# flexcompute/tidy3d

Hardware: AMD Instinct MI355X
Metric: Mcells/s on 512^3 Yee grid (higher is better)
Workload: dtype f32; 1 GPU; v0: vacuum, PEC walls, curl stencil only; 512^3 Yee cells, Ez point dipole (GaussianPulse 200 THz), random +-1e-3 initial fields; parallelism=z-slab x1, bytes_per_cell_step=72

## Files before the change

include/fdtd_hip.h:

```cpp
#ifndef FDTD_HIP_H
#define FDTD_HIP_H

#include <stddef.h>
#include <stdint.h>

#ifdef __cplusplus
extern "C" {
#endif

typedef struct FdtdSolver FdtdSolver;

enum { FDTD_BC_PEC = 0, FDTD_BC_PMC = 1, FDTD_BC_PERIODIC = 2, FDTD_BC_NEIGHBOR = 3 };
enum { FDTD_MON_TIME = 0, FDTD_MON_DFT = 1 };
enum { FDTD_VARIANT_AUTO = 0, FDTD_VARIANT_SIMPLE = 1, FDTD_VARIANT_ZMARCH = 2, FDTD_VARIANT_FUSED = 3 };
enum { FDTD_FLAG_TIME_KERNELS = 1 };

typedef struct FdtdConfig {
  int32_t nx, ny, nz;
  int32_t bc[6];
  int32_t device;
  int32_t variant;
  int32_t flags;
  int32_t z_chunk;
  float   ch;
  int32_t reserved[6];
} FdtdConfig;

typedef struct FdtdStats {
  int64_t steps_done;
  int32_t diverged;
  int32_t stopped_early;
  double  field_decay;
  double  run_ms;
  double  h_kernel_ms;
  double  e_kernel_ms;
  int64_t h_kernel_launches;
  int64_t e_kernel_launches;
  int64_t device_bytes;
  double  fused_kernel_ms;
  int64_t fused_kernel_launches;
  int32_t tile_rows;
  int32_t tile_zchunk;
  int32_t tile_order;
  int32_t placement;
  float   placement_ms_first;
  float   placement_ms_kept;
  int32_t stream_overlap;
  int32_t stream_retries;
  int32_t comm_ranks;
  int32_t comm_rank;
  int64_t two_step_pairs;
  int32_t tblock_planes;
  int32_t reserved0;
  int64_t graph_pairs;
  int64_t fused2_pairs;
  int64_t fused2_shape;
  int64_t shell_pairs;
  double  shell_kernel_ms;
  int64_t shell_kernel_launches;
  int64_t shell2_pairs;
  int32_t fused2_off_reason;
  int32_t struct_bytes;
  int64_t disp_pairs;
  int32_t single_step_reason;
  int32_t src_paged_pairs;
  double  seam_kernel_ms;
  int64_t seam_kernel_launches;
} FdtdStats;

enum { FDTD_F2_OFF_NONE = 0,
       FDTD_F2_OFF_DISABLED = 1,
       FDTD_F2_OFF_TOO_SMALL = 2,
       FDTD_F2_OFF_COMM = 3,
       FDTD_F2_OFF_PML = 4,
       FDTD_F2_OFF_ADE = 5,
       FDTD_F2_OFF_TFSF = 6,
       FDTD_F2_OFF_BOUNDARY = 7,
       FDTD_F2_OFF_H_SOURCE_ABSORBER = 8,
       FDTD_F2_OFF_SEAM_SOURCE = 9,
       FDTD_F2_OFF_SOURCES = 10,
       FDTD_F2_OFF_VARIANT = 11,
       FDTD_F2_OFF_SHELL = 12,
       FDTD_F2_OFF_MEMORY = 13 };

typedef int (*FdtdProgressFn)(int64_t step, double time, double field_decay, void* user);

const char* fdtd_last_error(const FdtdSolver* h);
int  fdtd_device_count(void);

int  fdtd_far_field(int device, int n_u, int n_v, const double* u, const double* v, const double* wu, const double* wv,
                    const double* currents, double w0, double k_re, double k_im, int n_dir, const double* r_u,
                    const double* r_v, const double* r_w, double* out);

int  fdtd_create(const FdtdConfig* cfg, FdtdSolver** out);
void fdtd_destroy(FdtdSolver* h);

int fdtd_set_steps(FdtdSolver* h, int axis, const float* inv_primal, const float* inv_dual, int n);

int fdtd_set_media(FdtdSolver* h, const float* ca, const float* cb, int n_media);
int fdtd_set_material(FdtdSolver* h, const uint8_t* mat, size_t bytes);
int fdtd_set_material16(FdtdSolver* h, const uint16_t* mat, size_t count);

int fdtd_set_pml(FdtdSolver* h, int axis, int n_lo, int n_hi,
                 const float* kinv_e, const float* b_e, const float* c_e,
                 const float* kinv_h, const float* b_h, const float* c_h, int n);

int fdtd_set_mirror_plus(FdtdSolver* h, int axis, int wall);

int fdtd_set_absorber(FdtdSolver* h, int axis, int n_lo, int n_hi, const float* fb, const float* fc, int n);

int fdtd_add_ade(FdtdSolver* h, int comp, int64_t n_cells, const uint32_t* cell_index,
                 int n_poles, const float* kap, const float* bet, float cc);

int fdtd_add_aniso(FdtdSolver* h, int comp, int64_t n_nodes, const uint32_t* cell_index, const uint32_t* nbr_index,
                   const float* w_new, const float* w_old);
int fdtd_add_aniso_bloch(FdtdSolver* h, int comp, int64_t n_nodes, const uint32_t* cell_index, const uint32_t* nbr_index,
                         const float* w_new, const float* w_old, const uint8_t* wrap);

int fdtd_add_point_source(FdtdSolver* h, int64_t n_points, const int32_t* comp,
                          const uint32_t* cell_index, const float* w_re, const float* w_im,
                          int64_t n_steps, const float* wave_e, const float* wave_h);

int fdtd_add_tfsf(FdtdSolver* h, int n_aux, const float* ae, const float* be,
                  const float* ah, const float* bh, int src_cell,
                  int64_t n_steps, const float* wave,
                  int64_t n_e, const int32_t* e_comp, const uint32_t* e_index, const float* e_w,
                  const int32_t* e_aux,
                  int64_t n_h, const int32_t* h_comp, const uint32_t* h_index, const float* h_w,
                  const int32_t* h_aux);

int fdtd_add_monitor(FdtdSolver* h, int kind, int n_comps, const int32_t* comps,
                     const int32_t lo[3], const int32_t hi[3],
                     int64_t n_rec, const int64_t* steps,
                     int nf, const float* phase_e, const float* phase_h);
int fdtd_get_monitor(FdtdSolver* h, int monitor_id, void* host, size_t bytes);

int fdtd_set_field(FdtdSolver* h, int comp, const float* host, size_t bytes);
int fdtd_get_field(FdtdSolver* h, int comp, float* host, size_t bytes);

int fdtd_set_shutoff(FdtdSolver* h, int every, double shutoff, int64_t ref_step);

int fdtd_comm_unique_id(char id[128]);
int fdtd_comm_init(FdtdSolver* h, const char id[128], int rank, int n_ranks);

int fdtd_run(FdtdSolver* h, int64_t n_steps, FdtdProgressFn progress, void* user);
int fdtd_run_bloch(FdtdSolver* h_re, FdtdSolver* h_im, int64_t n_steps, const double phase[3], const int n_real[3],
                   FdtdProgressFn progress, void* user);
int fdtd_get_stats(FdtdSolver* h, FdtdStats* out);
enum { FDTD_OPT_FLAGS = 0, FDTD_OPT_VARIANT = 1, FDTD_OPT_ZCHUNK = 2, FDTD_OPT_ROWS = 3, FDTD_OPT_XCD_REMAP = 4 ,
       FDTD_OPT_FUSED_LB = 5,
       FDTD_OPT_PML_FUSED = 6 ,
       FDTD_OPT_BND_PLANES = 7 ,
       FDTD_OPT_AUTOTUNE = 8 ,
       FDTD_OPT_PML_SPLIT = 9 ,
       FDTD_OPT_PLACEMENT_TRIES = 12,
       FDTD_OPT_MEM_HINTS = 11,
       FDTD_OPT_TBLOCK = 13,
       FDTD_OPT_EDGE_ZCHUNK = 14,
       FDTD_OPT_GRAPH = 15,
       FDTD_OPT_TWOSTEP = 16,
       FDTD_OPT_SHELL_PAIRS = 17,
       FDTD_OPT_STRIP = 18,
       FDTD_OPT_SHELL2 = 19,
       FDTD_OPT_SHELL2_SHAPE = 20,
       FDTD_OPT_DEBUG_SYNC = 21,
       FDTD_OPT_TILE_SPLIT = 22,
       FDTD_OPT_DISP = 23,
       FDTD_OPT_SRC_PAGED = 25,
       FDTD_OPT_WHATIF = 24,
       FDTD_OPT_SLAB_BOXES_FIRST = 26,
       FDTD_OPT_LDS_PAD = 10  };
int fdtd_set_option(FdtdSolver* h, int key, int value);
int fdtd_reset(FdtdSolver* h);

#ifdef __cplusplus
}
#endif
#endif
```

tidy3d_amd/csrc/fdtd_capi.hip:

```cpp
#include <hip/hip_runtime.h>
#include <rccl/rccl.h>

#include <array>
#include <cmath>
#include <cstdarg>
#include <cstdio>
#include <cstdlib>
#include <cstring>
#include <deque>
#include <map>
#include <string>
#include <utility>
#include <algorithm>
#include <vector>

#include "../../include/fdtd_hip.h"
#include "fdtd_kernels.hpp"
#include "fdtd_fused2.hpp"
#include "fdtd_strip.hpp"
#include "fdtd_shell2_host.hpp"
#include "fdtd_aniso.hpp"

using namespace fdtd;

// ... 165 lines not shown
  SrcPaged spg;
  std::map<std::array<int, 6>, int> box_paged;
  int spg_on = -1;
  int whatif = 0;
  int disp_on = -1;
  std::vector<AnisoGroup> aniso;
  std::vector<PointSrc> psrc;
  std::vector<Tfsf> tfsf;
  std::vector<Monitor> mons;
  hipStream_t stream = nullptr, comm_stream = nullptr;
  hipEvent_t ev0 = nullptr, ev1 = nullptr;
  std::vector<hipEvent_t> kev;
  std::vector<int> kev_kind;
  double* energy_dev = nullptr;
  int decay_every = 0;
  double shutoff = 0.0;
  long long decay_ref = 0;
  double energy_max = 0.0;
  long long step = 0;
  FdtdStats stats{};
  int zchunk = 2;
  int zchunk_f = 16;
  int last_zc = 0;
  int rows_f = 3;
  int xcd_remap = -1;
  int fused_lb = 0;
  int pml_fused = -1;
  int placement_tries = 6;
  int slab_boxes_first = 3;
  hipStream_t box_stream = nullptr;
  bool box_stream_tried = false;
  int box_stream_attempts = 0;
  hipEvent_t ev_box = nullptr, ev_box_in = nullptr;
  bool placement_done = false;
  float placement_ms[9] = {};
  int placement_tried = 0, placement_kept = 0;
  int mem_hints = 1;
  int lds_pad = 0;
  int pml_split = -1;
  int autotune = 0;
  bool tuned = false, user_geometry = false;
  int bnd_planes = 0;
  int rows = 4;
  PmlP* pml_blk[8][2][2] = {};
  PmlP* pml_blk2[2][2] = {};
  PmlP* pml_blk_hole[2][2][2] = {};
  bool pml_blk_hole_ok = false;
  bool pml_blk_ok[8] = {};
  bool pml_blk2_ok = false;
  int pml_parity = 0;
  int pml_e_parity = 0;
  ncclComm_t comm = nullptr;
  int rank = 0, n_ranks = 1;
  hipEvent_t ev_h_int = nullptr, ev_h_bnd = nullptr, ev_e_int = nullptr, ev_e_bnd = nullptr;
  int stream_overlap = 0, stream_retries = 0;
  bool streams_shared = false;
  int tblock = -1;
  int edge_zchunk = -1;
  int use_graph = -1;
  long long* step_dev = nullptr;
  long long step_dev_value = -1;
  bool step_dev_mode = false;
  long long step_dev_off = 0;
  long long graph_pairs = 0;
  int mirror_wall[3] = {-1, -1, -1};
  int graph_status = 0;
  long long two_step_pairs = 0;
  int tblock_used = 0;
  int twostep_w = -1, twostep_zc = 0;
  int twostep_w_used = 0, twostep_zc_used = 0;
  long long fused2_pairs = 0;
  int shell_on = -1;
  int strip_zc = 4;
  int strip_occ = 3;
  long long shell_pairs = 0;
  int shell2_on = -1;
  int shell2_qw = 0, shell2_ww = 8, shell2_zcw = 0;
  int shell2_ws = 6, shell2_zcs = 0;
  long long shell2_pairs = 0;
  int f2_off_reason = 0;
  int debug_sync = 0;
  hipEvent_t ev_shell_a = nullptr, ev_shell_b = nullptr;
  hipEvent_t ev_rec = nullptr;
  float* seam_buf = nullptr;
  float* inj_val = nullptr;
  float* cap_val = nullptr;
  float* dump_buf = nullptr;
  long long dump_cap = 0;
  std::deque<F2Table> f2_tables;
  size_t inj_sources = 0;
  float* src_tab = nullptr;
  long long src_tab_steps = 0, src_tab_nodes = 0;
  bool src_on_seam = false;
  bool src_h_on_seam = false;
  long long src_nodes = 0;
  int f2_dyn_reason = 0;
  long long src_h_nodes = 0;
  bool src_e_in_damp = false;
};

namespace {

int fail(FdtdSolver* h, const char* fmt, ...) {
  char buf[1024];
  va_list ap;
  va_start(ap, fmt);
  vsnprintf(buf, sizeof(buf), fmt, ap);
  va_end(ap);
  if (h) h->err = buf; else g_create_error = buf;
  return -1;
}

#define HIPCHK(h, call)                                                                   \
  do {                                                                                    \
    hipError_t e_ = (call);                                                               \
    if (e_ != hipSuccess)                                                                 \
      return fail(h, "%s failed: %s (%s:%d)", #call, hipGetErrorString(e_), __FILE__, __LINE__); \
  } while (0)

#define NCCLCHK(h, call)                                                                  \
  do {                                                                                    \
    ncclResult_t r_ = (call);                                                             \
    if (r_ != ncclSuccess)                                                                \
      return fail(h, "%s failed: %s (%s:%d)", #call, ncclGetErrorString(r_), __FILE__, __LINE__); \
  } while (0)

template <typename T>
int dev_alloc(FdtdSolver* h, T** out, size_t count, bool zero_fill = true) {
  void* p = nullptr;
  size_t bytes = count * sizeof(T);
  if (bytes == 0) bytes = sizeof(T);
  HIPCHK(h, hipMalloc(&p, bytes));
  if (zero_fill) {
    HIPCHK(h, hipMemset(p, 0, bytes));
    HIPCHK(h, hipStreamSynchronize(nullptr));
  }
  h->bufs.push_back({p, bytes});
  h->stats.device_bytes += (int64_t)bytes;
  *out = reinterpret_cast<T*>(p);
  return 0;
}

template <typename T>
int dev_upload(FdtdSolver* h, T** out, const T* host, size_t count) {
  if (dev_alloc(h, out, count, false)) return -1;
  if (count) HIPCHK(h, hipMemcpy(*out, host, count * sizeof(T), hipMemcpyHostToDevice));
  return 0;
}

#ifdef FDTD_PLACEMENT_PROBE
inline long env_long(const char* name, long dflt) {
  const char* e = std::getenv(name);
  return e ? std::atol(e) : dflt;
}
int alloc_field_set(FdtdSolver* h, float** base, size_t fcount, int set) {
  const int mode = (int)env_long("FDTD_FIELD_LAYOUT", 0);
  if (mode == 3 || mode == 4) {
    if (set == 1) return 0;
    const size_t s0 = (size_t)env_long("FDTD_FIELD_S0", 0) / 16 * 4;
    const size_t s1 = (size_t)env_long("FDTD_FIELD_S1", 0) / 16 * 4, s2 = (size_t)env_long("FDTD_FIELD_S2", 0) / 16 * 4;
    const size_t stride = fcount + s1;
    float* blk = nullptr;
    if (mode == 4) {
      static float* pool = nullptr;
      const size_t pool_floats = (size_t)env_long("FDTD_FIELD_POOL", 16L << 30) / 4;
      if (!pool) HIPCHK(h, hipMalloc((void**)&pool, pool_floats * 4));
      if (s0 + 12 * stride + s2 > pool_floats) return fail(h, "field pool too small");
// ... 556 lines not shown
  }
  std::stable_sort(ent.begin(), ent.end(), [](const std::array<int, 5>& x, const std::array<int, 5>& y) {
    return x[0] != y[0] ? x[0] < y[0] : (x[3] >= 8) < (y[3] >= 8);
  });
  std::vector<int> start((size_t)g.nz + 2, 0);
  std::vector<int4> e4(std::max<size_t>(1, ent.size()));
  for (size_t q = 0; q < ent.size(); ++q) {
    start[(size_t)ent[q][0] + 1]++;
    e4[q].x = ent[q][1]; e4[q].y = ent[q][2]; e4[q].z = ent[q][3]; e4[q].w = ent[q][4];
  }
  for (int k = 0; k <= g.nz; ++k) start[(size_t)k + 1] += start[(size_t)k];
  if (dev_upload(h, &tb.start, (const int*)start.data(), start.size()) ||
      dev_upload(h, &tb.ent, (const int4*)e4.data(), e4.size())) return nullptr;
  tb.dfts = plan.dfts; tb.dft_when = plan.dft_when;
  if (!plan.dfts.empty()) {
    std::vector<DumpBox> boxes;
    std::vector<std::vector<int>> per_plane((size_t)g.nz + 1);
    long long off = 0;
    for (size_t q = 0; q < plan.dfts.size(); ++q) {
      const Monitor& m = h->mons[(size_t)plan.dfts[q]];
      DumpBox bx{m.box.lo0, m.box.lo1, m.box.lo2, m.box.nx, m.box.ny, m.box.nz, {-1, -1, -1, -1, -1, -1}};
      const int when = plan.dft_when[q];
      for (int c : m.comps) if ((c >= 3 && (when & 1)) || (c < 3 && (when & 2))) { bx.off[c] = (int)off; off += m.cells; }
      tb.dft_off.push_back({bx.off[0], bx.off[1], bx.off[2], bx.off[3], bx.off[4], bx.off[5]});
      bool any = false;
      for (int c = 0; c < 6; ++c) any = any || bx.off[c] >= 0;
      if (!any) continue;
      for (int k = m.box.lo2; k < m.box.lo2 + m.box.nz; ++k) per_plane[(size_t)k].push_back((int)boxes.size());
      boxes.push_back(bx);
    }
    tb.dump_floats = off;
    if (!boxes.empty()) {
      std::vector<int> ds((size_t)g.nz + 2, 0), dl;
      for (int k = 0; k <= g.nz; ++k) { ds[(size_t)k] = (int)dl.size(); if (k < g.nz) for (int b : per_plane[(size_t)k]) dl.push_back(b); }
      ds[(size_t)g.nz + 1] = (int)dl.size();
      if (dl.empty()) dl.push_back(0);
      if (dev_upload(h, &tb.dstart, (const int*)ds.data(), ds.size()) || dev_upload(h, &tb.dlist, (const int*)dl.data(), dl.size()) ||
          dev_upload(h, &tb.dboxes, (const DumpBox*)boxes.data(), boxes.size())) return nullptr;
    }
  }
  h->f2_tables.push_back(tb);
  return &h->f2_tables.back();
}

const FdtdSolver::TileClasses* tile_classes(FdtdSolver* h, int W, int zc, const ClipP& box, int nbx, int nby, int nbz, bool disp = false, bool src = false) {
  const bool mats = h->mat4 && !h->roww_host.empty();
  if ((!mats && !src) || h->tile_split == 0) return nullptr;
  for (const auto& t : h->tile_cls)
    if (t.W == W && t.zc == zc && t.nbx == nbx && t.nby == nby && t.nbz == nbz && t.box.j0 == box.j0 && t.box.j1 == box.j1 &&
        t.box.k0 == box.k0 && t.box.k1 == box.k1 && t.disp == disp && t.src == src) return &t;
  const GridP& g = h->g;
  const int R = W - 3, nbx_all = (g.nx + 255) / 256;
  std::vector<unsigned char> cls((size_t)nbx * nby * nbz, 0);
  long long n_bg = 0;
  for (int tz = 0; tz < nbz; ++tz)
    for (int tx = 0; tx < nbx; ++tx)
      for (int ty = 0; ty < nby; ++ty) {
        const int k0 = box.k0 + tz * zc, k1 = std::min(k0 + zc, box.k1);
        const int j0 = box.j0 + ty * R;
        unsigned char c = 0;
        for (int k = std::max(k0 - 1, 0); mats && k <= std::min(k1, g.nz - 1) && !c; ++k)
          for (int j = std::max(j0 - 2, 0); j <= std::min(j0 + R, g.ny - 1); ++j)
            if (h->roww_host[((size_t)k * g.ny + j) * nbx_all + tx] != kBgWord) { c = 1; break; }
        if (disp && c)
          for (int k = std::max(k0 - 1, 0); k <= std::min(k1, g.nz - 1) && c < 2; ++k)
            for (int j = std::max(j0 - 2, 0); j <= std::min(j0 + R, g.ny - 1); ++j)
              if (h->disp.dseg_host[((size_t)k * g.ny + j) * nbx_all + tx] >= 0) { c = 2; break; }
        n_bg += !c;
        if (src) {
          bool found = false;
          for (int k = std::max(k0 - 1, 0); k <= std::min(k1, g.nz - 1) && !found; ++k)
            for (int j = std::max(j0 - 2, 0); j <= std::min(j0 + R, g.ny - 1); ++j)
              if (h->spg.sseg_host[((size_t)k * g.ny + j) * nbx_all + tx] >= 0) { found = true; break; }
          if (found) c |= 4;
        }
        cls[((size_t)tz * nbx + tx) * nby + ty] = c;
      }
  FdtdSolver::TileClasses e{W, zc, box, nbx, nby, nbz, nullptr, n_bg, (long long)cls.size(), disp, src};
  if (dev_upload(h, &e.dev, (const unsigned char*)cls.data(), cls.size())) return nullptr;
  h->tile_cls.push_back(e);
  return &h->tile_cls.back();
}

int launch_fused2(FdtdSolver* h, long long n, hipStream_t st, const F2Table* tb, bool* sources2_done, bool* damp2_done = nullptr,
                  const ClipP* clip = nullptr, bool use_disp = false, bool e2_clip = false, const SrcP& sr = SrcP{}) {
  const bool inject = tb->with_sources;
  const GridP& g = h->g;
  if (ensure_second_set(h)) return -1;
  int W = 16, zc = 32;
  const ClipP box = clip ? *clip : ClipP{0, g.nx, 0, g.ny, 0, g.nz};
  fused2_shape(h, &W, &zc, (clip && h->comm) ? clip : nullptr);
  if (clip && !h->comm && h->twostep_zc <= 0 && (long long)g.nx * g.ny * g.nz < (1LL << 28)) zc = std::min(zc, 16);
  zc = std::max(2, std::min(zc, box.k1 - box.k0));
  h->twostep_w_used = W; h->twostep_zc_used = zc;
  const int R = W - 3;
  const int nbx = (g.nx + 255) / 256, nby = (box.j1 - box.j0 + R - 1) / R;
  const int nbz = (box.k1 - box.k0 + zc - 1) / zc;
  const int n_seams = nbx - 1 + ((clip && h->cfg.bc[0] == FDTD_BC_PERIODIC) ? 1 : 0);
  if (!h->seam_buf && (nbx > 1 || h->cfg.bc[0] == FDTD_BC_PERIODIC) &&
      dev_alloc(h, &h->seam_buf, (size_t)nbx * kSeamArrays * (size_t)(g.nz + 2) * (size_t)g.ny)) return -1;
  if (!h->inj_val && dev_alloc(h, &h->inj_val, (size_t)kMaxInj)) return -1;
  if (!h->cap_val && dev_alloc(h, &h->cap_val, (size_t)kMaxCap)) return -1;
  InjP inj{};
  *sources2_done = false;
  {
    bool alive = false, alive2 = true;
    for (const PointSrc& s : h->psrc)
      if (inject && (s.n_e || s.n_h)) { alive = alive || n < s.n_steps; alive2 = alive2 && n + 1 < s.n_steps; }
    if (alive && h->src_tab && n + 1 < h->src_tab_steps) {
      inj.val = h->src_tab + n * h->src_tab_nodes;
      if (alive2) {
        inj.val2 = h->src_tab + (n + 1) * h->src_tab_nodes;
        if (!clip || e2_clip) { inj.e2_in_sweep = 1; *sources2_done = true; }
      }
    } else if (alive) {
      int off = 0;
      for (const PointSrc& s : h->psrc) {
        if (s.n_e) launch_inject_values(st, h->inj_val + off, s.wre_e, s.wim_e, s.wave_e, n, (int)s.n_e);
        off += (int)(s.n_e + s.n_h);
      }
      inj.val = h->inj_val;
    }
    inj.n = (alive || !tb->mons.empty()) ? 1 : 0;
    inj.start = tb->start; inj.ent = tb->ent; inj.cap = h->cap_val;
    if (tb->dstart) {
      if (tb->dump_floats > h->dump_cap) {
        if (dev_alloc(h, &h->dump_buf, (size_t)tb->dump_floats, false)) return -1;
        h->dump_cap = tb->dump_floats;
      }
      inj.dstart = tb->dstart; inj.dlist = tb->dlist; inj.dboxes = tb->dboxes; inj.dump = h->dump_buf;
      inj.n = 1;
    }
  }
  DampT dmp{};
  if (h->has_damp) {
    for (int a = 0; a < 3; ++a) { dmp.fb[a] = h->damp_fb[a]; dmp.fc[a] = h->damp_fc[a]; }
    bool post_sources = false;
    for (const PointSrc& s : h->psrc) post_sources = post_sources || (s.n_e && n + 1 < s.n_steps);
    dmp.e2 = (!post_sources || inj.e2_in_sweep || sr.sseg || !h->src_e_in_damp) ? 1 : 0;
    if (damp2_done) *damp2_done = dmp.e2 != 0;
  }
  const int total = nbx * nby * nbz;
  const int remap = h->xcd_remap < 0 ? 32 : h->xcd_remap;
  StepP sp = step_params(h);
  time_begin(h, 2, st);
  const MatP mp = mat_params(h);
  DispP dp{nullptr, nullptr, nullptr};
  if (use_disp) dp = DispP{h->disp.dseg, h->disp.cs, h->disp.e1};
  int opt = (h->mem_hints ? 1 : 0) | (h->mat4 ? 2 : 0) | ((tb->mons.empty() && (!tb->with_sources || h->src_h_nodes == 0) && !tb->dstart) ? 0 : 4) |
            (clip ? 16 : (h->has_damp ? 8 : 0)) | (use_disp ? 32 | 1 : 0);
  if (h->whatif > 0 && h->whatif <= 15 && h->whatif != 9 && opt == 1 && (W == 16 || h->whatif == 13 || h->whatif == 14)) opt |= h->whatif << 8;
  SrcP sr_used = sr;
  if (h->whatif == 9 && !sr.sseg && !(opt & 8) && (!(opt & 32) || (opt & 16))) {
    SrcPaged& S = h->spg;
    const size_t nseg = (size_t)g.nz * g.ny * ((g.nx + 255) / 256);
    if (!S.sseg && S.state != 1) {
      S.sseg_host.assign(nseg, -1);
      SrcT tab{};
      if (dev_upload(h, &S.sseg, (const int*)S.sseg_host.data(), nseg) || dev_upload(h, &S.tab, &tab, 1)) return -1;
    }
    if (S.sseg && S.state != 1) { sr_used.sseg = S.sseg; sr_used.t = S.tab; opt |= 64 | 4 | 1; }
  }
  if (sr.sseg) { opt |= 64 | 4 | 1; *sources2_done = true; h->spg.pairs++; }
  const int blocks = remap ? ((total + 7) / 8) * 8 : total;
  const FdtdSolver::TileClasses* tc = tile_classes(h, W, zc, box, nbx, nby, nbz, use_disp, sr_used.sseg != nullptr);
  const bool split = tc && (use_disp || sr_used.sseg || (tc->n_bg > 0 && (h->tile_split == 1 || 8 * tc->n_bg >= tc->n_all)));
  launch_fused2_step(st, W, opt, blocks, g, h->f, h->f2, sp, mp, zc, nbx, nby, nbz, remap, inj, h->seam_buf, dmp, box,
                     TileClassP{split ? tc->dev : nullptr}, dp, sr_used);
  time_end(h, st);
  if (n_seams > 0) {
    time_begin(h, 4, st);
    launch_seams(st, g, h->f2, sp, mp, h->seam_buf, n_seams, dmp, box, inj, sr);
    time_end(h, st);
  }
  if (use_disp) h->disp.pairs++;
  if (!clip) swap_sets(h);
  return 0;
}

struct ShellGeom { int o0[3], o1[3]; };
bool shell_geometry(const FdtdSolver* h, ShellGeom* G) {
  const int N[3] = {h->g.nx, h->g.ny, h->g.nz};
  for (int a = 0; a < 3; ++a) {
    const PmlAxisDev& P = h->pml[a];
    const int lo = P.ns > 0 ? P.lo : 0, hi0 = P.ns > 0 ? P.hi0 : N[a];
    int o0 = lo > 0 ? lo + 2 : 0, o1 = hi0 < N[a] ? hi0 - 1 : N[a];
    if (a > 0 && h->cfg.bc[2 * a] == FDTD_BC_PERIODIC) { o0 = 2; o1 = N[a] - 2; }
    if (a == 0) { o0 = (o0 + 3) / 4 * 4; o1 = o1 / 4 * 4; }
    if (o1 - o0 < (a == 0 ? 16 : 8)) return false;
    G->o0[a] = o0; G->o1[a] = o1;
  }
  return true;
}

void release_buf(FdtdSolver* h, void* p);
int ensure_third_set(FdtdSolver* h) {
  const GridP& g = h->g;
  if (h->f3.ex) return 0;
  const size_t fcount = (size_t)g.sxy * (g.nz + 2);
  if (!h->fbase3[0] && alloc_field_set(h, h->fbase3, fcount, 2)) {
    for (int c = 0; c < 6; ++c) { if (h->fbase3[c]) release_buf(h, h->fbase3[c]); h->fbase3[c] = nullptr; }
    return -1;
  }
  h->f3.ex = h->fbase3[0] + g.sxy; h->f3.ey = h->fbase3[1] + g.sxy; h->f3.ez = h->fbase3[2] + g.sxy;
  h->f3.hx = h->fbase3[3] + g.sxy; h->f3.hy = h->fbase3[4] + g.sxy; h->f3.hz = h->fbase3[5] + g.sxy;
  return 0;
}

void launch_strip(FdtdSolver* h, const FieldP& src, const FieldP& dst, const PmlP* pm, int ci0, int ci1, int j0, int j1,
                  int k0, int k1, hipStream_t st) {
  if (ci1 <= ci0 || j1 <= j0 || k1 <= k0) return;
  StripP sp;
  sp.q = std::min(kStripMaxQ, (ci1 - ci0) / 4);
  sp.xorg = ci0; sp.ci0 = ci0; sp.ci1 = ci1; sp.j0 = j0; sp.j1 = j1; sp.kbeg = k0; sp.kend = k1;
  sp.zchunk = h->strip_zc;
  const int slots = (64 / sp.q) * kStripWaves;
  sp.nbx = (ci1 - ci0 + 4 * sp.q - 1) / (4 * sp.q);
  sp.nby = (j1 - j0 + slots - 2) / (slots - 1);
  sp.nbz = (k1 - k0 + sp.zchunk - 1) / sp.zchunk;
  const int pmc = h->cfg.bc[4] == FDTD_BC_PMC;
  const dim3 grid((unsigned)(sp.nbx * sp.nby * sp.nbz)), block(64, kStripWaves);
  time_begin(h, 3, st);
  if (h->mat4 && h->strip_occ == 4) hipLaunchKernelGGL((strip_step_kernel<true, 4>), grid, block, 0, st, h->g, src, dst, step_params(h), mat_params(h), pm, sp, pmc);
  else if (h->mat4) hipLaunchKernelGGL((strip_step_kernel<true, 3>), grid, block, 0, st, h->g, src, dst, step_params(h), mat_params(h), pm, sp, pmc);
  else if (h->strip_occ == 4) hipLaunchKernelGGL((strip_step_kernel<false, 4>), grid, block, 0, st, h->g, src, dst, step_params(h), mat_params(h), pm, sp, pmc);
  else hipLaunchKernelGGL((strip_step_kernel<false, 3>), grid, block, 0, st, h->g, src, dst, step_params(h), mat_params(h), pm, sp, pmc);
  time_end(h, st);
}

struct ZPlan {
  int n = 0;
  int a[4] = {}, b[4] = {};
  bool ok = false;
};
bool zplan_build(const FdtdSolver* h, const ShellGeom& G, bool source_holes, ZPlan* P) {
  std::vector<std::pair<int, int>> holes;
  for (const AdeGroup& a : h->ade) if (a.n > 0) holes.push_back({a.k0 - 2, a.k1 + 2});
  if (source_holes) {
    for (const PointSrc& s : h->psrc) {
      if (s.n_e) holes.push_back({s.ke0 - 2, s.ke1 + 2});
      if (s.n_h) holes.push_back({s.kh0 - 2, s.kh1 + 2});
    }
    for (const Tfsf& t : h->tfsf) {
      if (t.e.n_targets) holes.push_back({t.e.k0 - 2, t.e.k1 + 2});
      if (t.h.n_targets) holes.push_back({t.h.k0 - 2, t.h.k1 + 2});
    }
  }
  std::sort(holes.begin(), holes.end());
  P->n = 0;
  int lo = G.o0[2];
  auto close = [&](int hi) {
    if (hi - lo >= 8) {
      if (P->n == 4) return false;
      P->a[P->n] = lo; P->b[P->n] = hi; P->n++;
    }
    return true;
  };
  for (const auto& hz : holes) {
    if (hz.second <= lo) continue;
    if (hz.first >= G.o1[2]) break;
// ... 1622 lines not shown
  return 0;
}
}

int fdtd_add_tfsf(FdtdSolver* h, int n_aux, const float* ae, const float* be, const float* ah, const float* bh,
                  int src_cell, int64_t n_steps, const float* wave, int64_t n_e, const int32_t* e_comp,
                  const uint32_t* e_index, const float* e_w, const int32_t* e_aux, int64_t n_h,
                  const int32_t* h_comp, const uint32_t* h_index, const float* h_w, const int32_t* h_aux) {
  if (!h) return -1;
  if (n_aux < 4 || src_cell < 1 || src_cell >= n_aux) return fail(h, "fdtd_add_tfsf: bad auxiliary grid");
  HIPCHK(h, hipSetDevice(h->cfg.device));
  Tfsf t{};
  t.n_aux = n_aux; t.src_cell = src_cell;
  t.n_steps = n_steps;
  if (dev_upload(h, &t.ae, ae, (size_t)n_aux + 1) || dev_upload(h, &t.be, be, (size_t)n_aux + 1) ||
      dev_upload(h, &t.ah, ah, (size_t)n_aux) || dev_upload(h, &t.bh, bh, (size_t)n_aux) ||
      dev_alloc(h, &t.e1, (size_t)n_aux + 1) || dev_alloc(h, &t.h1, (size_t)n_aux) ||
      dev_alloc(h, &t.e1c, (size_t)n_aux + 1) || dev_alloc(h, &t.h1c, (size_t)n_aux) ||
      dev_upload(h, &t.wave, wave, (size_t)n_steps))
    return -1;
  if (build_tfsf_list(h, t.e, n_e, e_comp, e_index, e_w, e_aux, n_aux - 1) ||
      build_tfsf_list(h, t.h, n_h, h_comp, h_index, h_w, h_aux, n_aux))
    return -1;
  h->tfsf.push_back(t);
  return 0;
}

int fdtd_add_monitor(FdtdSolver* h, int kind, int n_comps, const int32_t* comps, const int32_t lo[3],
                     const int32_t hi[3], int64_t n_rec, const int64_t* steps, int nf, const float* phase_e,
                     const float* phase_h) {
  if (!h) return -1;
  if (kind != FDTD_MON_TIME && kind != FDTD_MON_DFT) return fail(h, "fdtd_add_monitor: bad kind %d", kind);
  const int N[3] = {h->g.nx, h->g.ny, h->g.nz};
  for (int a = 0; a < 3; ++a)
    if (lo[a] < 0 || hi[a] > N[a] || hi[a] <= lo[a]) return fail(h, "fdtd_add_monitor: box [%d,%d) outside axis %d of %d cells", lo[a], hi[a], a, N[a]);
  if (n_comps < 1 || n_comps > 6) return fail(h, "fdtd_add_monitor: n_comps must be 1..6");
  if (kind == FDTD_MON_DFT && nf < 1) return fail(h, "fdtd_add_monitor: a DFT monitor needs frequencies");
  HIPCHK(h, hipSetDevice(h->cfg.device));
  Monitor m;
  m.kind = kind;
  m.comps.assign(comps, comps + n_comps);
  for (int c : m.comps) if (c < 0 || c > 5) return fail(h, "fdtd_add_monitor: bad component %d", c);
  m.box.lo0 = lo[0]; m.box.lo1 = lo[1]; m.box.lo2 = lo[2];
  m.box.nx = hi[0] - lo[0]; m.box.ny = hi[1] - lo[1]; m.box.nz = hi[2] - lo[2];
  m.cells = (long long)m.box.nx * m.box.ny * m.box.nz;
  m.steps.assign(steps, steps + n_rec);
  for (size_t i = 1; i < m.steps.size(); ++i)
    if (m.steps[i] <= m.steps[i - 1]) return fail(h, "fdtd_add_monitor: steps must be strictly increasing");
  m.nf = nf;
  if (kind == FDTD_MON_TIME) {
    m.data_bytes = (size_t)n_rec * n_comps * m.cells * sizeof(float);
    float* d = nullptr;
    if (dev_alloc(h, &d, (size_t)n_rec * n_comps * m.cells)) return -1;
    m.data = d;
  } else {
    m.data_bytes = (size_t)nf * n_comps * m.cells * sizeof(float2);
    float2* d = nullptr;
    if (dev_alloc(h, &d, (size_t)nf * n_comps * m.cells)) return -1;
    m.data = d;
    if (dev_upload(h, &m.phase_e, reinterpret_cast<const float2*>(phase_e), (size_t)n_rec * nf) ||
        dev_upload(h, &m.phase_h, reinterpret_cast<const float2*>(phase_h), (size_t)n_rec * nf))
      return -1;
  }
  h->mons.push_back(m);
  return (int)h->mons.size() - 1;
}

int fdtd_get_monitor(FdtdSolver* h, int id, void* host, size_t bytes) {
  if (!h) return -1;
  if (id < 0 || id >= (int)h->mons.size()) return fail(h, "fdtd_get_monitor: bad id %d", id);
  Monitor& m = h->mons[id];
  if (bytes != m.data_bytes) return fail(h, "fdtd_get_monitor: expected %zu bytes, got %zu", m.data_bytes, bytes);
  HIPCHK(h, hipSetDevice(h->cfg.device));
  HIPCHK(h, hipStreamSynchronize(h->stream));
  HIPCHK(h, hipMemcpy(host, m.data, bytes, hipMemcpyDeviceToHost));
  return 0;
}

int fdtd_set_field(FdtdSolver* h, int comp, const float* host, size_t bytes) {
  if (!h) return -1;
  if (comp < 0 || comp > 5) return fail(h, "fdtd_set_field: bad component");
  if (bytes != (size_t)n_cells(h) * 4) return fail(h, "fdtd_set_field: expected %zu bytes", (size_t)n_cells(h) * 4);
  HIPCHK(h, hipSetDevice(h->cfg.device));
  HIPCHK(h, hipMemcpy(field_ptr(h, comp), host, bytes, hipMemcpyHostToDevice));
  for (AdeGroup& a : h->ade)
    if (a.comp == comp) {
      hipLaunchKernelGGL(ade_gather_kernel, dim3(nblk(a.n)), dim3(256), 0, h->stream, (const float*)field_ptr(h, comp),
                         (const uint32_t*)a.cell, a.e_old, a.n);
      HIPCHK(h, hipStreamSynchronize(h->stream));
    }
  if (h->comm == nullptr) { fill_ghost_h(h, h->stream); fill_ghost_e(h, h->stream); fill_ghost_fused(h, h->stream); HIPCHK(h, hipStreamSynchronize(h->stream)); }
  else if (comp == 0 || comp == 1 || comp == 3 || comp == 4) {
    HIPCHK(h, hipStreamSynchronize(h->stream));
    if (exchange(h, comp < 3, h->comm_stream)) return -1;
    HIPCHK(h, hipStreamSynchronize(h->comm_stream));
  }
  return 0;
}

int fdtd_get_field(FdtdSolver* h, int comp, float* host, size_t bytes) {
  if (!h) return -1;
  if (comp < 0 || comp > 5) return fail(h, "fdtd_get_field: bad component");
  if (bytes != (size_t)n_cells(h) * 4) return fail(h, "fdtd_get_field: expected %zu bytes", (size_t)n_cells(h) * 4);
  HIPCHK(h, hipSetDevice(h->cfg.device));
  HIPCHK(h, hipStreamSynchronize(h->stream));
  HIPCHK(h, hipMemcpy(host, field_ptr(h, comp), bytes, hipMemcpyDeviceToHost));
  return 0;
}

int fdtd_set_shutoff(FdtdSolver* h, int every, double shutoff, int64_t ref_step) {
  if (!h) return -1;
  h->decay_every = every; h->shutoff = shutoff; h->decay_ref = ref_step;
  return 0;
}

int fdtd_comm_unique_id(char id[128]) {
  ncclUniqueId u;
  if (ncclGetUniqueId(&u) != ncclSuccess) return fail(nullptr, "ncclGetUniqueId failed");
  std::memcpy(id, &u, 128);
  return 0;
}

int fdtd_comm_init(FdtdSolver* h, const char id[128], int rank, int n_ranks) {
  if (!h) return -1;
  if (rank < 0 || rank >= n_ranks) return fail(h, "fdtd_comm_init: bad rank %d of %d", rank, n_ranks);
  HIPCHK(h, hipSetDevice(h->cfg.device));
  ncclUniqueId u;
  std::memcpy(&u, id, 128);
  NCCLCHK(h, ncclCommInitRank(&h->comm, n_ranks, u, rank));
  h->rank = rank; h->n_ranks = n_ranks;
  int cnt = 0, ur = -1;
  NCCLCHK(h, ncclCommCount(h->comm, &cnt));
  NCCLCHK(h, ncclCommUserRank(h->comm, &ur));
  h->stats.comm_ranks = cnt; h->stats.comm_rank = ur;
  return 0;
}

int fdtd_reset(FdtdSolver* h) {
  if (!h) return -1;
  HIPCHK(h, hipSetDevice(h->cfg.device));
  HIPCHK(h, hipStreamSynchronize(h->stream));
  for (int c = 0; c < 6; ++c) HIPCHK(h, hipMemset(h->fbase[c], 0, h->field_bytes));
  for (int c = 0; c < 6; ++c) if (h->fbase2[c]) HIPCHK(h, hipMemset(h->fbase2[c], 0, h->field_bytes));
  for (int c = 0; c < 6; ++c) if (h->fbase3[c]) HIPCHK(h, hipMemset(h->fbase3[c], 0, h->field_bytes));
  for (int a = 0; a < 3; ++a) {
    PmlAxisDev& P = h->pml[a];
    if (P.n == 0) continue;
    for (int s = 0; s < 2; ++s) {
      if (P.psi_e[s]) HIPCHK(h, hipMemset(P.psi_e[s], 0, P.psi_count * 4));
      if (P.psi_h[s]) HIPCHK(h, hipMemset(P.psi_h[s], 0, (P.psi_count + P.psi_plane) * 4));
      if (P.psi_h2[s]) HIPCHK(h, hipMemset(P.psi_h2[s], 0, (P.psi_count + P.psi_plane) * 4));
      if (P.psi_e2[s]) HIPCHK(h, hipMemset(P.psi_e2[s], 0, P.psi_count * 4));
      if (P.psi_et[s]) HIPCHK(h, hipMemset(P.psi_et[s], 0, P.psi_count * 4));
      if (P.psi_ht[s]) HIPCHK(h, hipMemset(P.psi_ht[s], 0, (P.psi_count + P.psi_plane) * 4));
    }
  }
  for (AdeGroup& a : h->ade) {
    HIPCHK(h, hipMemset(a.e_old, 0, (size_t)a.n * 4));
    HIPCHK(h, hipMemset(a.q, 0, (size_t)a.n * a.p.n_poles * 8));
  }
  if (h->disp.state == 1) HIPCHK(h, hipMemset(h->disp.cs, 0, (size_t)h->disp.n_blocks * 3 * 256 * sizeof(float)));
  for (Tfsf& t : h->tfsf) {
    HIPCHK(h, hipMemset(t.e1, 0, ((size_t)t.n_aux + 1) * 4));
    HIPCHK(h, hipMemset(t.h1, 0, (size_t)t.n_aux * 4));
  }
  for (Monitor& m : h->mons) { HIPCHK(h, hipMemset(m.data, 0, m.data_bytes)); m.next = 0; }
  h->step = 0; h->energy_max = 0.0;
  h->stats.steps_done = 0; h->stats.diverged = 0; h->stats.stopped_early = 0; h->stats.field_decay = 1.0;
  return 0;
}

}
namespace {
struct GraphRec { const float* set; int parity; hipGraphExec_t exec; };
struct Run {
  FdtdSolver* h;
  int64_t n_steps;
  FdtdProgressFn progress;
  void* user;
  bool multi = false, nb_lo = false, nb_hi = false;
  int nz = 0;
  hipStream_t st = nullptr, cs = nullptr;
  bool fused_ok = false, fused = false, fused_multi = false;
  int b_lo = 0, b_hi = 0;
  bool primed = false;
  int pml_in_m = 0;
  bool psi_ghosts = false;
  int tb_req = 0;
  bool tb_two_streams = false, tb_ok = false;
  std::vector<hipEvent_t> tb_ev;
  bool split_now = false, graph_ok = false;
  std::vector<GraphRec> graphs;
  bool f2_ok = false, f2s_ok = false, s2_ok = false, s2_deep = false, f2m_ok = false;
  bool s2_disp = false;
  bool pair_disp = false;
  bool spg_ok = false;
  bool pair_spg = false;
  bool f2mc_ok = false, f2mc_deep = false;
  ShellGeom sg{}, sgm{};
  ZPlan zp_base, zp_src;
  ZPlan zp_s2, zp_s2h;
  F2Plan f2_plan;
  int64_t done = 0;
  long long n = 0;
  bool rec = false, src_alive = false, pair = false, use_s2 = false;
  int src_why = 0;
  const ZPlan* zp = nullptr;

  void sync_point() { if (h->debug_sync) (void)hipDeviceSynchronize(); }
  int setup() {
    multi = h->comm != nullptr;
    nb_lo = h->cfg.bc[4] == FDTD_BC_NEIGHBOR, nb_hi = h->cfg.bc[5] == FDTD_BC_NEIGHBOR;
    if ((nb_lo || nb_hi) && !multi) return fail(h, "fdtd_run: neighbour faces need fdtd_comm_init");
    if (multi && !h->aniso.empty()) return fail(h, "fdtd_run: fully anisotropic media are not available on z-slabs");
    if (multi && h->mirror_wall[2] >= 0 && (nb_hi || h->mirror_wall[2] != h->g.nz - 2 || h->g.nz < 6))
      return fail(h, "fdtd_run: a PMC plus face along z needs the last z-slab to hold the wall and at least 6 planes");
    nz = h->g.nz;
    if ((multi || any_pml(h) || h->tblock > 4096) && probe_stream_overlap(h)) return -1;
    st = h->stream, cs = h->comm_stream;
    for (hipEvent_t e : h->kev) hipEventDestroy(e);
    h->kev.clear(); h->kev_kind.clear();
    h->stats.stopped_early = 0;
    HIPCHK(h, hipEventRecord(h->ev0, st));
    if (multi && (nb_lo || nb_hi) && nz < 2) return fail(h, "fdtd_run: a z-slab needs at least 2 planes");
// ... 240 lines not shown
  int setup_pairs() {
    if (fused && !tb_ok && !h->ade.empty() && disp_setup(h)) return -1;
    h->disp.pairs = 0;
    s2_disp = false;
    spg_ok = false;
    h->spg.pairs = 0;
    if (fused && !tb_ok && !multi && (!h->tfsf.empty() || !h->psrc.empty())) {
      if (fused2_sources(h)) return -1;
      bool needs = !h->tfsf.empty() || h->src_nodes > kMaxInj || h->src_h_on_seam || (h->src_h_nodes > 0 && !h->src_tab);
      if (!needs) {
        long long len = -1;
        for (const PointSrc& s : h->psrc) if (s.n_e || s.n_h) { if (len >= 0 && s.n_steps != len) needs = true; len = s.n_steps; }
      }
      if (needs && spg_setup(h)) return -1;
      spg_ok = needs && h->spg.state == 1 && !(h->has_damp && h->spg.any_h);
    }
    f2_ok = fused && !tb_ok && fused2_eligible(h);
    sg = ShellGeom{};
    f2s_ok = false;
    h->f2_off_reason = !fused ? FDTD_F2_OFF_VARIANT : (tb_ok ? FDTD_F2_OFF_DISABLED : 0);
    if (fused && !tb_ok && !f2_ok) {
      const bool shell = any_pml(h) || any_periodic(h) || !h->ade.empty();
      h->f2_off_reason = shell ? shell_why_not(h, &sg, &zp_base, &zp_src) : fused2_why_not(h);
      f2s_ok = shell && h->f2_off_reason == 0;
    }
    s2_ok = false, s2_deep = false;
    if (fused && !tb_ok && !f2_ok && any_pml(h)) {
      ShellGeom g2{};
      const int why2 = shell2_why_not(h, &g2);
      if (why2 == 0) {
        const int why_r4 = h->f2_off_reason;
        s2_ok = true; sg = g2;
        s2_deep = shell2_sources_deep(h, sg);
        h->f2_off_reason = 0;
        zp_s2 = ZPlan{};
        s2_disp = !h->ade.empty() && h->disp.state == 1 && h->cfg.bc[2] != FDTD_BC_PERIODIC && h->shell2_on != 2 && h->shell2_on != 3;
        if (h->ade.empty() || s2_disp) { zp_s2.n = 1; zp_s2.a[0] = sg.o0[2]; zp_s2.b[0] = sg.o1[2]; zp_s2.ok = true; }
        else if (zplan_build(h, sg, false, &zp_s2) && zp_s2.a[0] == sg.o0[2] && zp_s2.b[zp_s2.n - 1] == sg.o1[2]) zp_s2.ok = true;
        if (!zp_s2.ok) { s2_ok = false; s2_disp = false; h->f2_off_reason = why_r4; }
        zp_s2h = ZPlan{};
        if (h->shell2_on != 2 && h->shell2_on != 3 && zplan_build(h, sg, true, &zp_s2h) && zp_s2h.n > 1 && zp_s2h.a[0] == sg.o0[2] &&
            zp_s2h.b[zp_s2h.n - 1] == sg.o1[2]) zp_s2h.ok = true;
      }
    }
    h->f2_dyn_reason = 0;
    if (f2_ok || f2s_ok || s2_ok) {
      if (fused2_sources(h)) return -1;
    }
    if (f2s_ok && ensure_third_set(h)) {
      (void)hipGetLastError();
      h->err.clear();
      f2s_ok = false;
      h->f2_off_reason = FDTD_F2_OFF_MEMORY;
    }
    if ((f2s_ok || s2_ok) && probe_stream_overlap(h)) return -1;
    f2m_ok = fused_multi && !any_pml(h) && !h->has_damp && h->shell_on != 0 && nz >= 8 && fused2_why_not(h, true) == 0;
    if (fused_multi) h->f2_off_reason = f2m_ok ? 0 : (any_pml(h) || h->has_damp ? FDTD_F2_OFF_COMM : (fused2_why_not(h, true) ? fused2_why_not(h, true) : FDTD_F2_OFF_COMM));
    if (f2m_ok) {
      if (fused2_sources(h)) return -1;
      if (ensure_third_set(h)) { (void)hipGetLastError(); h->err.clear(); f2m_ok = false; h->f2_off_reason = FDTD_F2_OFF_MEMORY; }
    }
    f2mc_ok = false;
    if (fused_multi && any_pml(h) && pml_in_m != 0 && pml_in_m == pml_in_sweep_mask(h) && !h->has_damp && h->shell_on != 0 &&
        h->shell2_on != 0 && h->shell2_on != 2 && h->shell2_on != 3 &&
        h->ade.empty() && !any_periodic(h) && (long long)h->g.sxy * 4 < (1LL << 32)) {
      int why = fused2_why_not(h, true, true);
      if (!why && !shell_geometry(h, &sgm)) why = FDTD_F2_OFF_PML;
      if (!why) {
        const PmlAxisDev& pz = h->pml[2];
        if (nb_lo) sgm.o0[2] = std::max(sgm.o0[2], 2);
        if (nb_hi) sgm.o1[2] = std::min(sgm.o1[2], nz - 2);
        if (sgm.o1[2] - sgm.o0[2] < 8 || (pz.ns > 0 && ((nb_lo && pz.lo > 0) || (nb_hi && pz.hi0 < nz)))) why = FDTD_F2_OFF_TOO_SMALL;
      }
      if (!why && (fused2_sources(h) || ensure_third_set(h) || ensure_pml_blocks2(h) || ensure_pml_blocks_hole(h))) {
        (void)hipGetLastError();
        h->err.clear();
        why = FDTD_F2_OFF_MEMORY;
      }
      f2mc_ok = why == 0;
      f2mc_deep = f2mc_ok && shell2_sources_deep(h, sgm);
      h->f2_off_reason = why;
    }
    h->fused2_pairs = 0;
    h->shell_pairs = 0;
    h->shell2_pairs = 0;
    done = 0;
    return 0;
  }
  int shell_pair(long long n, const F2Table* tb, const ZPlan& zp) {
    hipStream_t cs = (h->shell_on == 2) ? st : h->comm_stream;
    const int pml_in = 7 & pml_in_sweep_mask(h);
    if (ensure_second_set(h) || ensure_third_set(h) || ensure_pml_blocks(h, pml_in)) return -1;
    if (!h->ev_shell_a) {
      HIPCHK(h, hipEventCreateWithFlags(&h->ev_shell_a, hipEventDisableTiming));
      HIPCHK(h, hipEventCreateWithFlags(&h->ev_shell_b, hipEventDisableTiming));
    }
    const int N[3] = {h->g.nx, h->g.ny, nz};
    int in0[3], in1[3];
    for (int a = 0; a < 3; ++a) {
      in0[a] = sg.o0[a] > 0 ? sg.o0[a] + (a == 0 ? 4 : 1) : 0;
      in1[a] = sg.o1[a] < N[a] ? sg.o1[a] - (a == 0 ? 4 : 1) : N[a];
    }
    launch_sources(h, false, n, 0, nz, st);
    advance_tfsf_aux(h, false, n, st);
    if (h->cfg.bc[4] == FDTD_BC_PERIODIC) fill_ghost_h(h, st);
    HIPCHK(h, hipEventRecord(h->ev_shell_a, st));
    HIPCHK(h, hipStreamWaitEvent(cs, h->ev_shell_a, 0));
    const FieldP A = h->f, B = h->f2, T = h->f3;
    const int par = h->pml_parity;
    bool s2 = false;
    for (int i = 0; i < zp.n; ++i) {
      const ClipP clip{sg.o0[0], sg.o1[0], sg.o0[1], sg.o1[1], zp.a[i], zp.b[i]};
      if (launch_fused2(h, n, st, tb, &s2, nullptr, &clip)) return -1;
    }
    if (launch_shell_step(h, A, T, par, in0, in1, pml_in, cs, zp, 1)) return -1;
    launch_sources(h, true, n, 0, nz, cs, false, &T);
    launch_ade(h, 0, nz, cs, &T);
    advance_tfsf_aux(h, true, n, cs);
    launch_sources(h, false, n + 1, 0, nz, cs, false, &T);
    advance_tfsf_aux(h, false, n + 1, cs);
    fill_ghost_fused(h, cs, &T);
    if (launch_shell_step(h, T, B, par ^ 1, sg.o0, sg.o1, pml_in, cs, zp, 0)) return -1;
    HIPCHK(h, hipEventRecord(h->ev_shell_b, cs));
    HIPCHK(h, hipStreamWaitEvent(st, h->ev_shell_b, 0));
    swap_sets(h);
    pair_record(h, tb, n, st);
    if (rec_at(n + 1)) record_monitors(h, n + 1, true, st);
    launch_sources(h, true, n + 1, 0, nz, st);
    launch_ade(h, 0, nz, st);
    advance_tfsf_aux(h, true, n + 1, st);
    fill_ghost_fused(h, st);
    return 0;
  }
  int shell2_pair(long long n, const F2Table* tb, const ZPlan& zp) {
    hipStream_t cs = (h->shell_on == 2) ? st : h->comm_stream;
    const bool holes = zp.n > 1;
    const bool per_y = h->cfg.bc[2] == FDTD_BC_PERIODIC;
    if (ensure_second_set(h) || ensure_pml_blocks2(h)) return -1;
    if ((holes || per_y) && (ensure_third_set(h) || ensure_pml_blocks_hole(h))) return -1;
    if (!h->ev_shell_a) {
      HIPCHK(h, hipEventCreateWithFlags(&h->ev_shell_a, hipEventDisableTiming));
      HIPCHK(h, hipEventCreateWithFlags(&h->ev_shell_b, hipEventDisableTiming));
    }
    launch_sources(h, false, n, 0, nz, st);
    if (pair_spg) spg_fill(h, n, st);
    else advance_tfsf_aux(h, false, n, st);
    const SrcP sr = pair_spg ? spg_params(h) : SrcP{};
    HIPCHK(h, hipEventRecord(h->ev_shell_a, st));
    HIPCHK(h, hipStreamWaitEvent(cs, h->ev_shell_a, 0));
    const FieldP A = h->f, B = h->f2, T = h->f3;
    const int hp = h->pml_parity, ep = h->pml_e_parity;
    bool s2 = false;
    Shell2Box boxes[kShell2MaxBoxes];
    int nb = 0;
    for (int i = 0; i < zp.n; ++i) {
      const ClipP clip{sg.o0[0], sg.o1[0], sg.o0[1], sg.o1[1], zp.a[i], zp.b[i]};
      if (launch_fused2(h, n, st, tb, &s2, nullptr, &clip, pair_disp, zp.n == 1 && s2_deep, sr)) return -1;
      ShellGeom gi = sg;
      gi.o0[2] = zp.a[i]; gi.o1[2] = zp.b[i];
      Shell2Box bi[kShell2MaxBoxes];
      const int ni = shell2_boxes(h, gi, bi, i == 0 ? 0 : zp.a[i], i == zp.n - 1 ? nz : zp.b[i]);
      for (int q = 0; q < ni && nb < kShell2MaxBoxes; ++q) boxes[nb++] = bi[q];
    }
    bool src_due = false;
    for (const PointSrc& sr : h->psrc) src_due = src_due || (sr.n_e && n + 1 < sr.n_steps);
    const bool ade2_early = pair_disp && (s2 || !src_due) && disp_inside(h, sg.o0, sg.o1, 2);
    if (ade2_early) launch_ade2(h, st, &B);
    launch_shell2_boxes(h, boxes, nb, h->pml_blk2[hp][ep], cs, tb, pair_disp, sr);
    if (holes || per_y) {
      const int pml_in = 7 & pml_in_sweep_mask(h);
      ShellSets s1{A, T, hp, 0, 0, h->pml_blk_hole[0][hp][ep]}, s2h{T, B, hp, 0, 0, h->pml_blk_hole[1][hp][ep]};
      auto wrap_rows = [&](const ShellSets& base, int grow) {
        const int R = h->rows_f, ny = h->g.ny, nby_all = (ny + R - 1) / R;
        const int in0 = 2 + grow, in1 = ny - 2 - grow;
        const int ty_a = std::min(nby_all, (in0 + R - 1) / R), ty_c = std::max(ty_a, in1 / R);
        ShellSets sh = base;
        sh.ex_j0 = in0; sh.ex_j1 = in1;
        for (int i = 0; i < zp.n; ++i) {
          const int lo = i == 0 ? 0 : zp.a[i], hi = i == zp.n - 1 ? nz : zp.b[i];
          if (launch_fused_range(h, lo, hi, cs, pml_in, 0, 0, ty_a + (nby_all - ty_c), ty_a, ty_c - ty_a, true, &sh)) return -1;
        }
        return 0;
      };
      for (int i = 0; i + 1 < zp.n; ++i)
        if (launch_fused_range(h, zp.b[i] - 1, zp.a[i + 1] + 1, cs, pml_in, 0, 0, -1, 0, 0, true, &s1)) return -1;
      if (per_y && wrap_rows(s1, 1)) return -1;
      if (holes) {
        launch_sources(h, true, n, 0, nz, cs, false, &T);
        launch_ade(h, 0, nz, cs, &T);
        advance_tfsf_aux(h, true, n, cs);
        launch_sources(h, false, n + 1, 0, nz, cs, false, &T);
        advance_tfsf_aux(h, false, n + 1, cs);
      }
      for (int i = 0; i + 1 < zp.n; ++i)
        if (launch_fused_range(h, zp.b[i], zp.a[i + 1], cs, pml_in, 0, 0, -1, 0, 0, true, &s2h)) return -1;
      if (per_y && wrap_rows(s2h, 0)) return -1;
    }
    HIPCHK(h, hipEventRecord(h->ev_shell_b, cs));
    HIPCHK(h, hipStreamWaitEvent(st, h->ev_shell_b, 0));
    swap_sets(h);
    swap_psi_h(h, 7);
    swap_psi_e(h);
    pair_record(h, tb, n, st);
    if (rec_at(n + 1)) record_monitors(h, n + 1, true, st);
    if (!holes && !pair_spg) {
      advance_tfsf_aux(h, true, n, st);
      advance_tfsf_aux(h, false, n + 1, st);
    }
    if (!s2) launch_sources(h, true, n + 1, 0, nz, st);
    if (!pair_disp) launch_ade(h, 0, nz, st);
    else if (!ade2_early) launch_ade2(h, st);
    if (!pair_spg) advance_tfsf_aux(h, true, n + 1, st);
    fill_ghost_fused(h, st);
    return 0;
  }
  bool plan_clear_of_holes(const F2Plan& pl, const ZPlan& zp) {
    auto inside = [&](const Monitor& m, bool segment) {
      for (int i = 0; i < zp.n; ++i) {
        const int lo = (segment && i == 0) ? 0 : zp.a[i], hi = (segment && i == zp.n - 1) ? nz : zp.b[i];
        if (m.box.lo2 >= lo && m.box.lo2 + m.box.nz <= hi) return true;
      }
      return false;
    };
    for (int q : pl.mons) if (!inside(h->mons[(size_t)q], false)) return false;
    for (int q : pl.dfts) if (!inside(h->mons[(size_t)q], true)) return false;
    if (h->cfg.bc[2] == FDTD_BC_PERIODIC)
      for (int q : pl.dfts) {
        const Monitor& m = h->mons[(size_t)q];
        if (m.box.lo1 < 2 || m.box.lo1 + m.box.ny > h->g.ny - 2) return false;
      }
    return true;
  }
  bool plan_in_bulk(const F2Plan& pl, const ZPlan& zp) {
    auto inside = [&](const Monitor& m) {
      for (int i = 0; i < zp.n; ++i) if (m.box.lo2 >= zp.a[i] && m.box.lo2 + m.box.nz <= zp.b[i]) return true;
      return false;
    };
    for (int q : pl.mons) if (!inside(h->mons[(size_t)q])) return false;
    for (int q : pl.dfts) if (!inside(h->mons[(size_t)q])) return false;
    return true;
  }
  int begin_step() {
    n = h->step;
    rec = !fused_multi && rec_at(n);
    if (rec && multi) {
      HIPCHK(h, hipStreamWaitEvent(st, h->ev_e_bnd, 0));
      HIPCHK(h, hipStreamWaitEvent(st, h->ev_h_bnd, 0));
    }
    src_alive = false;
    src_why = 0;
    zp = &zp_base;
    pair = fused && (f2_ok || f2s_ok || s2_ok) && done + 2 <= n_steps && !(h->decay_every > 0 && ((n + 1) % h->decay_every) == 0);
    use_s2 = false;
    if (pair) {
      src_why = fused2_sources_why_not(h, n, &src_alive);
      pair_spg = false;
      if (src_why != 0 && spg_ok && (src_why == FDTD_F2_OFF_TFSF || src_why == FDTD_F2_OFF_SOURCES || src_why == FDTD_F2_OFF_SEAM_SOURCE)) {
        const bool s2_form = s2_ok && zp_s2.ok && zp_s2.n == 1 && h->cfg.bc[2] != FDTD_BC_PERIODIC;
        if (s2_form || f2_ok) { pair_spg = true; src_why = 0; src_alive = false; }
      }
      use_s2 = s2_ok && src_why == 0 && (!src_alive || s2_deep || pair_spg);
      if (use_s2) zp = &zp_s2;
      else if (s2_ok && zp_s2h.ok && (src_why != 0 || src_alive)) {
        use_s2 = true; src_why = 0; src_alive = false; zp = &zp_s2h;
      }
      if (!use_s2 && !f2_ok && !f2s_ok) { if (src_why) h->f2_dyn_reason = src_why; pair = false; }
    }
    if (pair && use_s2) {
      pair = fused2_plan(h, n, &f2_plan, sg.o0, sg.o1, true) && plan_clear_of_holes(f2_plan, *zp);
      if (!pair && f2s_ok) { pair = true; use_s2 = false; zp = &zp_base; src_why = fused2_sources_why_not(h, n, &src_alive); }
    }
    if (pair && !use_s2) {
      if (src_why && f2s_ok && zp_src.ok) { src_why = 0; src_alive = false; zp = &zp_src; }
      if (src_why) h->f2_dyn_reason = src_why;
      pair = src_why == 0 && fused2_plan(h, n, &f2_plan, f2s_ok ? sg.o0 : nullptr, f2s_ok ? sg.o1 : nullptr) &&
             (!f2s_ok || plan_in_bulk(f2_plan, *zp));
    }
    pair_disp = pair && !h->ade.empty() && h->disp.state == 1 && (use_s2 ? (s2_disp && zp == &zp_s2) : !f2s_ok);
    pair_spg = pair_spg && pair && (use_s2 ? zp == &zp_s2 : (f2_ok && !f2s_ok));
    if (rec) record_monitors(h, n, false, st, (pair && !h_terms_in_front(h)) ? &f2_plan : nullptr);
    if (rec && multi) {
      if (!h->ev_rec) HIPCHK(h, hipEventCreateWithFlags(&h->ev_rec, hipEventDisableTiming));
      HIPCHK(h, hipEventRecord(h->ev_rec, st));
      HIPCHK(h, hipStreamWaitEvent(cs, h->ev_rec, 0));
    }
    return 0;
  }
  int slab_shell2_pair(const F2Table* tb) {
    const int bl = nb_lo ? 2 : 0, bh = nb_hi ? 2 : 0;
    const FieldP A = h->f, B = h->f2, T = h->f3;
    const int hp = h->pml_parity, ep = h->pml_e_parity;
    ShellSets s1{A, T, hp, 0, 0, h->pml_blk_hole[0][hp][ep]}, s2h{T, B, hp, 0, 0, h->pml_blk_hole[1][hp][ep]};
    HIPCHK(h, hipStreamWaitEvent(cs, h->ev_e_int, 0));
    HIPCHK(h, hipStreamWaitEvent(st, h->ev_e_bnd, 0));
    const ClipP clip{sgm.o0[0], sgm.o1[0], sgm.o0[1], sgm.o1[1], sgm.o0[2], sgm.o1[2]};
    bool s2done = false;
    Shell2Box boxes[kShell2MaxBoxes];
    const int nb = shell2_boxes(h, sgm, boxes, bl, nz - bh);
    bool third = (h->slab_boxes_first == 2 || (h->slab_boxes_first == 3 && nz >= 96)) && nb > 0 && !h->streams_shared && !h->debug_sync;
    if (third && !h->box_stream_tried && make_box_stream(h)) return -1;
    third = third && h->box_stream != nullptr;
    if (third) {
      HIPCHK(h, hipEventRecord(h->ev_box_in, st));
      HIPCHK(h, hipStreamWaitEvent(h->box_stream, h->ev_box_in, 0));
      HIPCHK(h, hipStreamWaitEvent(h->box_stream, h->ev_e_bnd, 0));
      launch_shell2_boxes(h, boxes, nb, h->pml_blk2[hp][ep], h->box_stream, tb);
      HIPCHK(h, hipEventRecord(h->ev_box, h->box_stream));
    } else if (h->slab_boxes_first) launch_shell2_boxes(h, boxes, nb, h->pml_blk2[hp][ep], st, tb);
    if (launch_fused2(h, n, st, tb, &s2done, nullptr, &clip)) return -1;
    if (launch_fused_range(h, 0, bl ? bl + 1 : 0, cs, pml_in_m, bh ? nz - bh - 1 : nz, nz, -1, 0, 0, true, &s1)) return -1;
    HIPCHK(h, hipEventRecord(h->ev_h_bnd, cs));
    if (bl) { launch_sources(h, true, n, 0, bl + 1, cs, false, &T); launch_sources(h, false, n + 1, 0, bl + 1, cs, false, &T); }
    if (bh) { launch_sources(h, true, n, nz - bh - 1, nz, cs, false, &T); launch_sources(h, false, n + 1, nz - bh - 1, nz, cs, false, &T); }
    if (exchange_fused_all(h, cs, psi_ghosts, &T, 1)) return -1;
    if (launch_fused_range(h, 0, bl, cs, pml_in_m, nz - bh, nz, -1, 0, 0, true, &s2h)) return -1;
    if (bl) { launch_sources(h, true, n + 1, 0, bl, cs, false, &B); launch_sources(h, false, n + 2, 0, bl, cs, false, &B); }
    if (bh) { launch_sources(h, true, n + 1, nz - bh, nz, cs, false, &B); launch_sources(h, false, n + 2, nz - bh, nz, cs, false, &B); }
    HIPCHK(h, hipEventRecord(h->ev_e_bnd, cs));
    if (exchange_fused_all(h, cs, psi_ghosts, &B, 2)) return -1;
    if (!h->slab_boxes_first) launch_shell2_boxes(h, boxes, nb, h->pml_blk2[hp][ep], st, tb);
    if (third) HIPCHK(h, hipStreamWaitEvent(st, h->ev_box, 0));
    swap_sets(h);
    swap_psi_h(h, 7);
    swap_psi_e(h);
    launch_sources(h, true, n + 1, bl, nz - bh, st);
    launch_sources(h, false, n + 2, bl, nz - bh, st);
    HIPCHK(h, hipEventRecord(h->ev_e_int, st));
// ... 27 lines not shown
      bool s2done = false;
      if (launch_fused2(h, n, st, tb, &s2done, nullptr, &clip)) return -1;
      if (launch_fused_range(h, 0, bl ? bl + 1 : 0, cs, 0, bh ? nz - bh - 1 : nz, nz, -1, 0, 0, false, &s1)) return -1;
      HIPCHK(h, hipEventRecord(h->ev_h_bnd, cs));
      if (bl) { launch_sources(h, true, n, 0, bl + 1, cs, false, &T); launch_sources(h, false, n + 1, 0, bl + 1, cs, false, &T); }
      if (bh) { launch_sources(h, true, n, nz - bh - 1, nz, cs, false, &T); launch_sources(h, false, n + 1, nz - bh - 1, nz, cs, false, &T); }
      if (exchange_fused_all(h, cs, false, &T)) return -1;
      if (launch_fused_range(h, 0, bl, cs, 0, nz - bh, nz, -1, 0, 0, false, &s2)) return -1;
      if (bl) { launch_sources(h, true, n + 1, 0, bl, cs, false, &B); launch_sources(h, false, n + 2, 0, bl, cs, false, &B); }
      if (bh) { launch_sources(h, true, n + 1, nz - bh, nz, cs, false, &B); launch_sources(h, false, n + 2, nz - bh, nz, cs, false, &B); }
      HIPCHK(h, hipEventRecord(h->ev_e_bnd, cs));
      if (exchange_fused_all(h, cs, false, &B)) return -1;
      swap_sets(h);
      launch_sources(h, true, n + 1, bl, nz - bh, st);
      launch_sources(h, false, n + 2, bl, nz - bh, st);
      HIPCHK(h, hipEventRecord(h->ev_e_int, st));
      h->fused2_pairs++;
      h->step = n + 2;
      return 1;
    }
    const bool decay_step = h->decay_every > 0 && ((n + 1) % h->decay_every) == 0;
    const bool last = (done + 1 == n_steps) || decay_step;
    HIPCHK(h, hipStreamWaitEvent(cs, h->ev_e_int, 0));
    const int pml_b = pml_in_m & 3;
    if (b_lo > 0 && b_hi > 0) { if (launch_fused_range(h, 0, b_lo, cs, pml_b, nz - b_hi, nz)) return -1; }
    else if (b_lo > 0) { if (launch_fused_range(h, 0, b_lo, cs, pml_b)) return -1; }
    else if (b_hi > 0) { if (launch_fused_range(h, nz - b_hi, nz, cs, pml_b)) return -1; }
    HIPCHK(h, hipEventRecord(h->ev_h_bnd, cs));
    HIPCHK(h, hipStreamWaitEvent(st, h->ev_e_bnd, 0));
    if ((pml_in_m & 6) == 0) {
      if (launch_fused_range(h, b_lo, nz - b_hi, st, pml_in_m)) return -1;
    } else {
      const int R = h->rows_f, nby_all = (h->g.ny + R - 1) / R, ki = b_lo, ke = nz - b_hi;
      const PmlAxisDev &py = h->pml[1], &pz = h->pml[2];
      const bool in_y = (pml_in_m & 2) && py.ns > 0, in_z = (pml_in_m & 4) && pz.ns > 0;
      const int za = std::min(ke, std::max(ki, (in_z && pz.lo > 0) ? std::min(nz, pz.lo + 1) : 0));
      const int zc = std::max(za, std::min(ke, (in_z && pz.hi0 < nz) ? pz.hi0 : nz));
      const int ty_a = (in_y && py.lo > 0) ? std::min(nby_all, py.lo / R + 1) : 0;
      const int ty_c = (in_y && py.hi0 < h->g.ny) ? std::max(ty_a, py.hi0 / R) : nby_all;
      if ((za > ki || zc < ke) && launch_fused_range(h, ki, za, st, pml_in_m, zc, ke, -1, 0, 0, true)) return -1;
      if (launch_fused_range(h, za, zc, st, pml_in_m & 3, 0, 0, ty_a + (nby_all - ty_c), ty_a, ty_c - ty_a, true)) return -1;
      if (launch_fused_range(h, za, zc, st, pml_in_m & 1, 0, 0, ty_c - ty_a, 0, ty_a)) return -1;
    }
    swap_sets(h);
    swap_psi_h(h, pml_in_m);
    const bool rec_post = rec_at(n);
    if (rec_post || last || rec_at(n + 1)) {
      HIPCHK(h, hipStreamWaitEvent(st, h->ev_h_bnd, 0));
      if (rec_post) record_monitors(h, n, true, st);
      e_post(n, 0, nz, st, false);
      advance_tfsf_aux(h, true, n, st, false);
      advance_tfsf_aux(h, true, n, st, true);
      primed = false;
      if (!last && prime(n + 1)) return -1;
      if (last) {
        HIPCHK(h, hipEventRecord(h->ev_e_int, st));
        HIPCHK(h, hipStreamWaitEvent(cs, h->ev_e_int, 0));
        HIPCHK(h, hipEventRecord(h->ev_e_bnd, cs));
      }
    } else {
      e_post(n, 0, b_lo, cs, true);
      e_post(n, nz - b_hi, nz, cs, true);
      advance_tfsf_aux(h, true, n, cs, true);
      h_pre(n + 1, 0, b_lo, cs, true);
      h_pre(n + 1, nz - b_hi, nz, cs, true);
      advance_tfsf_aux(h, false, n + 1, cs, true);
      HIPCHK(h, hipEventRecord(h->ev_e_bnd, cs));
      if (exchange_fused_all(h, cs, psi_ghosts)) return -1;
      e_post(n, b_lo, nz - b_hi, st, false);
      advance_tfsf_aux(h, true, n, st, false);
      h_pre(n + 1, b_lo, nz - b_hi, st, false);
      advance_tfsf_aux(h, false, n + 1, st, false);
      HIPCHK(h, hipEventRecord(h->ev_e_int, st));
    }
    h->step = n + 1;
    return 0;
  }
  int plain_pair() {
    const F2Table* tb = fused2_table(h, f2_plan, src_alive);
    if (!tb) return -1;
    bool sources2_done = false, damp2_done = true;
    launch_sources(h, false, n, 0, nz, st);
    if (pair_spg) spg_fill(h, n, st);
    if (launch_fused2(h, n, st, tb, &sources2_done, &damp2_done, nullptr, pair_disp, false, pair_spg ? spg_params(h) : SrcP{})) return -1;
    pair_record(h, tb, n, st);
    if (rec_at(n + 1)) record_monitors(h, n + 1, true, st);
    if (!sources2_done) launch_sources(h, true, n + 1, 0, nz, st);
    if (h->has_damp && !damp2_done) launch_damp(h, true, 0, nz, st);
    if (pair_disp) launch_ade2(h, st);
    fill_ghost_fused(h, st);
    return 0;
  }
  int two_pass_step() {
    const int h_top = (multi && nb_hi) ? nz - 1 : nz;
    const bool mirrors = h->mirror_wall[0] >= 0 || h->mirror_wall[1] >= 0 || h->mirror_wall[2] >= 0;
    if (multi && mirrors) {
      HIPCHK(h, hipStreamWaitEvent(st, h->ev_e_bnd, 0));
      fill_mirror(h, st, 0, nz);
      if (!h->ev_rec) HIPCHK(h, hipEventCreateWithFlags(&h->ev_rec, hipEventDisableTiming));
      HIPCHK(h, hipEventRecord(h->ev_rec, st));
      HIPCHK(h, hipStreamWaitEvent(cs, h->ev_rec, 0));
    }
    if (multi && nb_hi) {
      HIPCHK(h, hipStreamWaitEvent(cs, h->ev_e_int, 0));
      launch_damp(h, false, h_top, nz, cs);
      launch_sources(h, false, n, h_top, nz, cs);
      launch_pml(h, false, h_top, nz, cs);
      launch_h_main(h, h_top, nz, cs);
      HIPCHK(h, hipEventRecord(h->ev_h_bnd, cs));
    }
    if (multi) HIPCHK(h, hipStreamWaitEvent(st, h->ev_e_bnd, 0));
    if (!multi) fill_mirror(h, st, 0, nz);
    launch_damp(h, false, 0, h_top, st);
    launch_sources(h, false, n, 0, h_top, st);
    launch_pml(h, false, 0, h_top, st);
    launch_h_main(h, 0, h_top, st);
    advance_tfsf_aux(h, false, n, st);
    if (multi) {
      HIPCHK(h, hipEventRecord(h->ev_h_int, st));
      if (!nb_hi) HIPCHK(h, hipStreamWaitEvent(cs, h->ev_h_int, 0));
      HIPCHK(h, hipStreamWaitEvent(cs, h->ev_e_int, 0));
      if (exchange(h, false, cs)) return -1;
    }
    if (!multi || !nb_lo) fill_ghost_h(h, st);
    if (rec) {
      if (multi) HIPCHK(h, hipStreamWaitEvent(st, h->ev_h_bnd, 0));
      record_monitors(h, n, true, st);
    }
    const int e_bot = (multi && nb_lo) ? 1 : 0;
    if (multi && nb_lo) {
      HIPCHK(h, hipStreamWaitEvent(cs, h->ev_h_int, 0));
      launch_e_main(h, 0, e_bot, cs);
      launch_pml(h, true, 0, e_bot, cs);
      launch_sources(h, true, n, 0, e_bot, cs);
      launch_damp(h, true, 0, e_bot, cs);
      launch_ade(h, 0, e_bot, cs);
      HIPCHK(h, hipEventRecord(h->ev_e_bnd, cs));
    }
    if (multi && nb_hi) HIPCHK(h, hipStreamWaitEvent(st, h->ev_h_bnd, 0));
    aniso_save(h, st);
    launch_e_main(h, e_bot, nz, st);
    launch_pml(h, true, e_bot, nz, st);
    launch_sources(h, true, n, e_bot, nz, st);
    aniso_apply(h, st);
    launch_damp(h, true, e_bot, nz, st);
    launch_ade(h, e_bot, nz, st);
    advance_tfsf_aux(h, true, n, st);
    if (multi) {
      HIPCHK(h, hipEventRecord(h->ev_e_int, st));
      if (!nb_lo) HIPCHK(h, hipStreamWaitEvent(cs, h->ev_e_int, 0));
      HIPCHK(h, hipStreamWaitEvent(cs, h->ev_h_int, 0));
      if (exchange(h, true, cs)) return -1;
    }
    if (!multi || !nb_hi) fill_ghost_e(h, st);
    h->step = n + 1;
    return 0;
  }
  int decay_check() {
  if (h->decay_every > 0 && (h->step % h->decay_every) == 0) {
    if (multi) HIPCHK(h, hipStreamWaitEvent(st, h->ev_e_bnd, 0));
    double en = 0.0;
    if (eval_energy(h, st, &en)) return -1;
    if (multi) {
      double* tmp = h->energy_dev;
      HIPCHK(h, hipMemcpyAsync(tmp, &en, sizeof(double), hipMemcpyHostToDevice, cs));
      NCCLCHK(h, ncclAllReduce(tmp, tmp, 1, ncclDouble, ncclSum, h->comm, cs));
      HIPCHK(h, hipMemcpyAsync(&en, tmp, sizeof(double), hipMemcpyDeviceToHost, cs));
      HIPCHK(h, hipStreamSynchronize(cs));
    }
    if (!std::isfinite(en)) {
      h->stats.diverged = 1;
      return 1;
    }
    if (en > h->energy_max) h->energy_max = en;
    h->stats.field_decay = h->energy_max > 0 ? en / h->energy_max : 1.0;
    if (progress && progress(h->step, 0.0, h->stats.field_decay, user)) return 1;
    if (h->shutoff > 0 && h->step > h->decay_ref && h->stats.field_decay < h->shutoff) {
      h->stats.stopped_early = 1;
      return 1;
    }
  }
    return 0;
  }
  int finish() {
    if (multi) {
      HIPCHK(h, hipStreamWaitEvent(st, h->ev_e_bnd, 0));
      HIPCHK(h, hipStreamWaitEvent(st, h->ev_h_bnd, 0));
    }
    HIPCHK(h, hipEventRecord(h->ev1, st));
    HIPCHK(h, hipStreamSynchronize(st));
    HIPCHK(h, hipStreamSynchronize(cs));
    for (hipEvent_t e : tb_ev) hipEventDestroy(e);
    for (const GraphRec& r : graphs) hipGraphExecDestroy(r.exec);
    HIPCHK(h, hipGetLastError());
    float ms = 0.f;
    HIPCHK(h, hipEventElapsedTime(&ms, h->ev0, h->ev1));
    h->stats.run_ms = ms;
    h->stats.steps_done = h->step;
    h->stats.h_kernel_ms = h->stats.e_kernel_ms = h->stats.fused_kernel_ms = h->stats.shell_kernel_ms = h->stats.seam_kernel_ms = 0.0;
    h->stats.h_kernel_launches = h->stats.e_kernel_launches = h->stats.fused_kernel_launches = h->stats.shell_kernel_launches = h->stats.seam_kernel_launches = 0;
    for (size_t i = 0; i < h->kev_kind.size(); ++i) {
      float t = 0.f;
      if (hipEventElapsedTime(&t, h->kev[2 * i], h->kev[2 * i + 1]) != hipSuccess) continue;
      if (h->kev_kind[i] == 0) { h->stats.h_kernel_ms += t; h->stats.h_kernel_launches++; }
      else if (h->kev_kind[i] == 1) { h->stats.e_kernel_ms += t; h->stats.e_kernel_launches++; }
      else if (h->kev_kind[i] == 3) { h->stats.shell_kernel_ms += t; h->stats.shell_kernel_launches++; }
      else if (h->kev_kind[i] == 4) { h->stats.seam_kernel_ms += t; h->stats.seam_kernel_launches++; }
      else { h->stats.fused_kernel_ms += t; h->stats.fused_kernel_launches++; }
    }
    return 0;
  }
  int loop() {
    for (; done < n_steps; ++done) {
      if (begin_step()) return -1;
      if (fused_multi) {
        const int rc = slab_rank_step();
        if (rc < 0) return -1;
        if (rc > 0) { ++done; continue; }
      } else if (fused && tb_ok && done + 2 <= n_steps && !rec && !rec_at(n + 1) &&
                 !(h->decay_every > 0 && ((n + 1) % h->decay_every) == 0)) {
        if (tb_pair(n)) return -1;
        h->step = n + 2;
        ++done;
      } else if (pair && use_s2) {
        const F2Table* tb = fused2_table(h, f2_plan, src_alive);
        if (!tb) return -1;
        if (shell2_pair(n, tb, *zp)) return -1;
        h->fused2_pairs++;
        h->shell_pairs++;
        h->shell2_pairs++;
        h->step = n + 2;
        ++done;
      } else if (pair && f2s_ok) {
        const F2Table* tb = fused2_table(h, f2_plan, src_alive);
        if (!tb) return -1;
        if (shell_pair(n, tb, *zp)) return -1;
        h->fused2_pairs++;
        h->shell_pairs++;
        h->step = n + 2;
        ++done;
      } else if (pair) {
        if (plain_pair()) return -1;
        h->fused2_pairs++;
        h->step = n + 2;
        ++done;
      } else if (fused && graph_ok && done + 2 <= n_steps && !rec && !rec_at(n + 1) &&
                 !(h->decay_every > 0 && ((n + 1) % h->decay_every) == 0) && sources_alive(n + 1)) {
        const int grc = graph_pair(n);
        if (grc < 0) return -1;
        if (grc == 0) {
          h->step = n + 2;
          ++done;
        } else {
          if (fused_one(n, rec)) return -1;
          h->step = n + 1;
        }
      } else if (fused) {
        if (fused_one(n, rec)) return -1;
        h->step = n + 1;
      } else {
        if (two_pass_step()) return -1;
      }
      sync_point();
      const int dc = decay_check();
      if (dc < 0) return -1;
      if (dc > 0) { ++done; break; }
    }
    return 0;
  }
};
}
extern "C" {

int fdtd_run(FdtdSolver* h, int64_t n_steps, FdtdProgressFn progress, void* user) {
  if (!h) return -1;
  HIPCHK(h, hipSetDevice(h->cfg.device));
  Run r{h, n_steps, progress, user};
  if (r.setup() || r.setup_schedules() || r.setup_pairs()) return -1;
  if (r.loop()) return -1;
  return r.finish();
}
int fdtd_run_bloch(FdtdSolver* hr, FdtdSolver* hi, int64_t n_steps, const double phase[3], const int n_real[3],
                   FdtdProgressFn progress, void* user) {
  if (!hr || !hi) return -1;
  if (hi->comm) return fail(hr, "fdtd_run_bloch: the communicator of a z-slab belongs to the first (real-part) handle");
  const bool aniso = !hr->aniso.empty();
  if (hi->aniso.size() != hr->aniso.size())
    return fail(hr, "fdtd_run_bloch: the two solvers must carry the same fully anisotropic lists");
  for (size_t k = 0; k < hr->aniso.size(); ++k)
    if (hi->aniso[k].comp != hr->aniso[k].comp || hi->aniso[k].n != hr->aniso[k].n)
      return fail(hr, "fdtd_run_bloch: the two solvers must carry the same fully anisotropic lists");
  for (int a = 0; a < 3; ++a)
    if (hr->mirror_wall[a] >= 0 || hi->mirror_wall[a] >= 0) return fail(hr, "fdtd_run_bloch: PMC on a plus face is not available together with Bloch boundaries");
  const bool multi = hr->comm != nullptr;
  const bool nb_lo = hr->cfg.bc[4] == FDTD_BC_NEIGHBOR, nb_hi = hr->cfg.bc[5] == FDTD_BC_NEIGHBOR;
  if ((nb_lo || nb_hi) && !multi) return fail(hr, "fdtd_run_bloch: neighbour faces need fdtd_comm_init on the first handle");
  if (multi && aniso) return fail(hr, "fdtd_run_bloch: fully anisotropic media are not available on z-slabs");
  if (hi->cfg.bc[4] != hr->cfg.bc[4] || hi->cfg.bc[5] != hr->cfg.bc[5])
    return fail(hr, "fdtd_run_bloch: the two solvers must have the same z faces");
  if (hr->g.nx != hi->g.nx || hr->g.ny != hi->g.ny || hr->g.nz != hi->g.nz || hr->cfg.device != hi->cfg.device ||
      hr->mons.size() != hi->mons.size() || hr->step != hi->step)
    return fail(hr, "fdtd_run_bloch: the two solvers must describe the same simulation");
  const GridP& g = hr->g;
  const int nz = g.nz;
  const int N[3] = {g.nx, g.ny, nz};
  for (int a = 0; a < 2; ++a)
    if (n_real[a] < 0 || (n_real[a] > 0 && n_real[a] + 2 > N[a]))
      return fail(hr, "fdtd_run_bloch: axis %d has %d cells, cannot hold %d real cells + 2 ghost cells", a, N[a], n_real[a]);
  HIPCHK(hr, hipSetDevice(hr->cfg.device));
  hipStream_t st = hr->stream;
  HIPCHK(hr, hipStreamSynchronize(hi->stream));
  FdtdSolver* both[2] = {hr, hi};
  for (FdtdSolver* h : both) {
    for (hipEvent_t e : h->kev) hipEventDestroy(e);
    h->kev.clear(); h->kev_kind.clear();
    h->stats.stopped_early = 0;
  }
  HIPCHK(hr, hipEventRecord(hr->ev0, st));
  const bool per_z = hr->cfg.bc[4] == FDTD_BC_PERIODIC;
  const bool fused = !multi && !hr->mat4b && (g.nx % 4 == 0) && hr->rows_f <= 15 &&
                     (hr->cfg.variant == FDTD_VARIANT_FUSED || hr->cfg.variant == FDTD_VARIANT_AUTO);
  if (fused) for (FdtdSolver* h : both) if (ensure_second_set(h)) return -1;
  if (fused && !hr->tuned && !hr->user_geometry && !hi->user_geometry &&
      (n_cells(hr) >= (1LL << 20) || hr->autotune == 2)) {
    const long long wgs = (long long)((g.nx + 255) / 256) * ((g.ny + hr->rows_f - 1) / hr->rows_f) *
                          ((nz + hr->zchunk_f - 1) / hr->zchunk_f);
    if (wgs < 768 || hr->autotune) {
      if (autotune_fused(hr, st)) return -1;
      hi->rows_f = hr->rows_f; hi->zchunk_f = hr->zchunk_f; hi->tuned = true;
    }
  }
  float cph[3], sph[3];
  for (int a = 0; a < 3; ++a) { cph[a] = (float)std::cos(phase[a]); sph[a] = (float)std::sin(phase[a]); }
  AnisoPhaseTab wrap_tab{};
  if (aniso) {
    const double ph[3] = {n_real[0] > 0 ? phase[0] : 0.0, n_real[1] > 0 ? phase[1] : 0.0, per_z ? phase[2] : 0.0};
    for (int c = 0; c < kWrapCodes; ++c) {
      double p = 0.0;
      for (int a = 0; a < 3; ++a) {
        const int w = (c >> (2 * a)) & 3;
        p += w == 1 ? ph[a] : (w == 2 ? -ph[a] : 0.0);
      }
      wrap_tab.r[c] = make_float2((float)std::cos(p), (float)std::sin(p));
    }
  }
  auto e_tail = [&](long long n) {
    if (!aniso) {
      for (FdtdSolver* h : both) {
        launch_pml(h, true, 0, nz, st);
        launch_sources(h, true, n, 0, nz, st);
        launch_damp(h, true, 0, nz, st);
        launch_ade(h, 0, nz, st);
      }
      return;
    }
    for (FdtdSolver* h : both) {
      launch_pml(h, true, 0, nz, st);
      launch_sources(h, true, n, 0, nz, st);
    }
    aniso_apply_bloch(hr, hi, wrap_tab, st);
    for (FdtdSolver* h : both) {
      launch_damp(h, true, 0, nz, st);
// ... 81 lines not shown
      if (!per_z && !nb_hi) for (FdtdSolver* h : both) fill_ghost_e(h, st);
    }
    hr->step = hi->step = n + 1;
    if (hr->decay_every > 0 && (hr->step % hr->decay_every) == 0) {
      double en = 0.0;
      for (FdtdSolver* h : both) {
        double part = 0.0;
        if (eval_energy(h, st, &part)) { hr->err = h->err; return -1; }
        en += part;
      }
      if (multi) {
        double* tmp = hr->energy_dev;
        HIPCHK(hr, hipMemcpyAsync(tmp, &en, sizeof(double), hipMemcpyHostToDevice, st));
        NCCLCHK(hr, ncclAllReduce(tmp, tmp, 1, ncclDouble, ncclSum, hr->comm, st));
        HIPCHK(hr, hipMemcpyAsync(&en, tmp, sizeof(double), hipMemcpyDeviceToHost, st));
        HIPCHK(hr, hipStreamSynchronize(st));
      }
      if (!std::isfinite(en)) {
        hr->stats.diverged = hi->stats.diverged = 1;
        ++done;
        break;
      }
      if (en > hr->energy_max) hr->energy_max = hi->energy_max = en;
      hr->stats.field_decay = hi->stats.field_decay = hr->energy_max > 0 ? en / hr->energy_max : 1.0;
      if (progress && progress(hr->step, 0.0, hr->stats.field_decay, user)) { ++done; break; }
      if (hr->shutoff > 0 && hr->step > hr->decay_ref && hr->stats.field_decay < hr->shutoff) {
        hr->stats.stopped_early = hi->stats.stopped_early = 1;
        ++done;
        break;
      }
    }
  }
  fill_xy();
  HIPCHK(hr, hipEventRecord(hr->ev1, st));
  HIPCHK(hr, hipStreamSynchronize(st));
  HIPCHK(hr, hipGetLastError());
  float ms = 0.f;
  HIPCHK(hr, hipEventElapsedTime(&ms, hr->ev0, hr->ev1));
  for (FdtdSolver* h : both) {
    h->stats.run_ms = ms;
    h->stats.steps_done = h->step;
    h->stats.h_kernel_ms = h->stats.e_kernel_ms = h->stats.fused_kernel_ms = 0.0;
    h->stats.h_kernel_launches = h->stats.e_kernel_launches = h->stats.fused_kernel_launches = 0;
  }
  return 0;
}

int fdtd_set_option(FdtdSolver* h, int key, int value) {
  if (!h) return -1;
  switch (key) {
    case FDTD_OPT_FLAGS: h->cfg.flags = value; return 0;
    case FDTD_OPT_VARIANT: h->cfg.variant = value; return 0;
    case FDTD_OPT_ZCHUNK: if (value < 1) break; h->zchunk = value; h->zchunk_f = value; h->user_geometry = true; return 0;
    case FDTD_OPT_ROWS: if (value < 1 || value > 15) break; h->rows = value > 8 ? 8 : value; h->rows_f = value; h->user_geometry = true; return 0;
    case FDTD_OPT_XCD_REMAP: if (value > 1024) break; h->xcd_remap = value < 0 ? -1 : value; return 0;
    case FDTD_OPT_PML_FUSED: h->pml_fused = value < 0 ? -1 : (value & 7); for (bool& ok : h->pml_blk_ok) ok = false; h->pml_blk2_ok = false; h->pml_blk_hole_ok = false; return 0;
    case FDTD_OPT_BND_PLANES: h->bnd_planes = value > 0 ? value : 0; return 0;
    case FDTD_OPT_AUTOTUNE: h->autotune = value < 0 ? 0 : (value > 2 ? 1 : value); if (value) h->tuned = false; return 0;
    case FDTD_OPT_MEM_HINTS: h->mem_hints = value != 0; return 0;
    case FDTD_OPT_PLACEMENT_TRIES: if (value < 0 || (value % 100) > 8) break; h->placement_tries = value; h->placement_done = false; return 0;
    case FDTD_OPT_LDS_PAD: if (value < 0 || value > 120000) break; h->lds_pad = value; return 0;
    case FDTD_OPT_TBLOCK: h->tblock = value < 0 ? -1 : value; return 0;
    case FDTD_OPT_EDGE_ZCHUNK: h->edge_zchunk = value < 0 ? -1 : value; return 0;
    case FDTD_OPT_GRAPH: h->use_graph = value < 0 ? -1 : (value != 0); return 0;
    case FDTD_OPT_TWOSTEP: {
      if (value <= 0) { h->twostep_w = value < 0 ? -1 : 0; h->twostep_zc = 0; return 0; }
      const int w = value % 64, zc = (value / 64) % 1024;
      if (w < 4 || w > 16) return fail(h, "FDTD_OPT_TWOSTEP: %d waves per workgroup (4 ... 16)", w);
      h->twostep_w = w;
      h->twostep_zc = zc;
      return 0;
    }
    case FDTD_OPT_PML_SPLIT: h->pml_split = value < 0 ? -1 : (value != 0); return 0;
    case FDTD_OPT_SHELL_PAIRS: h->shell_on = value < 0 ? -1 : value; return 0;
    case FDTD_OPT_STRIP: if (value % 64 < 1 || (value / 64 != 3 && value / 64 != 4)) break; h->strip_zc = value % 64; h->strip_occ = value / 64; return 0;
    case FDTD_OPT_SHELL2: h->shell2_on = value < 0 ? -1 : (value > 3 ? 1 : value); return 0;
    case FDTD_OPT_DEBUG_SYNC: h->debug_sync = value != 0; return 0;
    case FDTD_OPT_TILE_SPLIT: h->tile_split = value < 0 ? -1 : (value != 0); return 0;
    case FDTD_OPT_SRC_PAGED:
      h->spg_on = value < 0 ? -1 : (value != 0);
      if (h->spg.state == -1 && value != 0) h->spg.state = 0;
      return 0;
    case FDTD_OPT_SLAB_BOXES_FIRST: if (value < 0 || value > 3) break; h->slab_boxes_first = value; return 0;
    case FDTD_OPT_WHATIF: if (value < 0 || value > 15) break; h->whatif = value; return 0;
    case FDTD_OPT_DISP:
      if (h->disp.state == 1 && value == 0) break;
      h->disp_on = value < 0 ? -1 : (value != 0);
      if (h->disp.state == -1 && value != 0) h->disp.state = 0;
      return 0;
    case FDTD_OPT_SHELL2_SHAPE: {
      if (value <= 0) { h->shell2_qw = 0; h->shell2_ww = 8; h->shell2_zcw = 0; h->shell2_ws = 6; h->shell2_zcs = 0; return 0; }
      const int qw = value % 128, ww = (value >> 7) % 8 + ((value >> 7) % 8 == 0 ? 8 : 0), zcw = (value >> 10) % 128;
      const int ws = (value >> 17) % 16, zcs = (value >> 21) % 128;
      if ((qw != 0 && qw < 3) || qw > 64 || ws > 8) break;
      h->shell2_qw = qw; h->shell2_ww = ww; h->shell2_zcw = zcw;
      h->shell2_ws = ws > 0 ? ws : 6; h->shell2_zcs = zcs;
      return 0;
    }
    case FDTD_OPT_FUSED_LB: if (value != 0 && value != 256 && value != 512 && value != 1024) break; h->fused_lb = value; return 0;
    default: break;
  }
  return fail(h, "fdtd_set_option: bad key/value %d/%d", key, value);
}

int fdtd_get_stats(FdtdSolver* h, FdtdStats* out) {
  if (!h || !out) return -1;
  *out = h->stats;
  out->tile_rows = h->rows_f;
  out->tile_zchunk = h->last_zc > 0 ? h->last_zc : h->zchunk_f;
  out->tile_order = h->xcd_remap < 0 ? kTileRun : h->xcd_remap;
  out->placement = (h->placement_tried << 8) | h->placement_kept;
  out->placement_ms_first = h->placement_ms[0];
  out->placement_ms_kept = h->placement_ms[h->placement_kept];
  out->stream_overlap = h->stream_overlap;
  out->stream_retries = h->stream_retries;
  out->two_step_pairs = h->two_step_pairs;
  out->tblock_planes = h->tblock_used;
  out->graph_pairs = h->graph_pairs;
  out->reserved0 = h->graph_status;
  out->fused2_pairs = h->fused2_pairs;
  out->fused2_shape = h->fused2_pairs ? (h->twostep_w_used | (h->twostep_zc_used << 6)) : 0;
  out->shell_pairs = h->shell_pairs;
  out->shell2_pairs = h->shell2_pairs;
  out->fused2_off_reason = h->fused2_pairs ? 0 : (h->f2_off_reason ? h->f2_off_reason : h->f2_dyn_reason);
  out->disp_pairs = h->disp.pairs;
  out->single_step_reason = h->f2_dyn_reason;
  out->src_paged_pairs = (int32_t)std::min<long long>(h->spg.pairs, 0x7fffffff);
  out->struct_bytes = (int32_t)sizeof(FdtdStats);
  return 0;
}

}
```

tidy3d_amd/csrc/fdtd_fused2.hip:

```cpp
#include <hip/hip_runtime.h>
#undef __global__
#if defined(__HIPCC__)
#define __global__ static __attribute__((global))
#else
#define __global__ static
#endif
#include "fdtd_kernels2.hpp"

namespace fdtd {

void launch_inject_values(hipStream_t st, float* val, const float* w_re, const float* w_im, const float2* wave,
                          long long step, int n) {
  hipLaunchKernelGGL(inject_values_kernel, dim3(1), dim3(256), 0, st, val, w_re, w_im, wave, step, n);
}

void launch_fused2_step(hipStream_t st, int waves, int opt, int grid_blocks, const GridP& g, const FieldP& a,
                        const FieldP& b, const StepP& s, const MatP& m, int zchunk, int nbx, int nby, int nbz,
                        int xcd_remap, const InjP& inj, float* seam, const DampT& dmp, const ClipP& clip, const TileClassP& tcl, const DispP& dp, const SrcP& sr) {
  if (opt & 64) {
    launch_fused2_step_src(st, waves, opt, grid_blocks, g, a, b, s, m, zchunk, nbx, nby, nbz, xcd_remap, inj, seam, dmp, clip, tcl, dp, sr);
    return;
  }
  if (opt >> 8) {
    launch_fused2_step_whatif(st, waves, opt, grid_blocks, g, a, b, s, m, zchunk, nbx, nby, nbz, xcd_remap, inj, seam, dmp, clip);
    return;
  }
  if (opt & 32) {
    launch_fused2_step_disp(st, waves, opt, grid_blocks, g, a, b, s, m, zchunk, nbx, nby, nbz, xcd_remap, inj, seam, dmp, clip, tcl, dp);
    return;
  }
  if (opt & 16) {
    launch_fused2_step_clip(st, waves, opt, grid_blocks, g, a, b, s, m, zchunk, nbx, nby, nbz, xcd_remap, inj, seam, dmp, clip, tcl);
    return;
  }
  const dim3 grid(grid_blocks, 1, 1), block(64, waves, 1);
#define FDTD_F2_O(LBV, OV)                                                                                             \
  hipLaunchKernelGGL((fused2_step_kernel<LBV, OV>), grid, block, fused2_lds_bytes(LBV, OV, waves), st, g, a, b, s, m, zchunk, nbx, nby, nbz,     \
                     xcd_remap, inj, seam, dmp, clip, tcl, dp, sr)
#define FDTD_F2(LBV)                                                                                                   \
  do {                                                                                                                 \
    switch (opt & 15) {                                                                                                \
      case 0: FDTD_F2_O(LBV, 0); break; case 1: FDTD_F2_O(LBV, 1); break; case 2: FDTD_F2_O(LBV, 2); break;            \
      case 3: FDTD_F2_O(LBV, 3); break; case 4: FDTD_F2_O(LBV, 4); break; case 5: FDTD_F2_O(LBV, 5); break;            \
      case 6: FDTD_F2_O(LBV, 6); break; case 7: FDTD_F2_O(LBV, 7); break; case 8: FDTD_F2_O(LBV, 8); break;            \
      case 9: FDTD_F2_O(LBV, 9); break; case 10: FDTD_F2_O(LBV, 10); break; case 11: FDTD_F2_O(LBV, 11); break;        \
      case 12: FDTD_F2_O(LBV, 12); break; case 13: FDTD_F2_O(LBV, 13); break; case 14: FDTD_F2_O(LBV, 14); break;      \
      default: FDTD_F2_O(LBV, 15); break;                                                                              \
    }                                                                                                                  \
  } while (0)
  if (waves <= 8) FDTD_F2(512);
  else if (waves <= 12) FDTD_F2(768);
  else FDTD_F2(1024);
#undef FDTD_F2
#undef FDTD_F2_O
}

void launch_inject_table(hipStream_t st, float* tab, long long stride, long long off, const float* w_re, const float* w_im,
                         const float2* wave, long long n_steps, int n) {
  const unsigned blocks = (unsigned)((n_steps * n + 255) / 256);
  hipLaunchKernelGGL(inject_table_kernel, dim3(blocks), dim3(256), 0, st, tab, stride, off, w_re, w_im, wave, n_steps, n);
}

void launch_pair_record(hipStream_t st, const PairRecP& r, long long max_cells, const GridP& g, const FieldP& a, const FieldP& b,
                        const float* cap) {
  const dim3 grid((unsigned)((max_cells + 255) / 256), (unsigned)(r.n_mon * 6));
  hipLaunchKernelGGL(pair_record_kernel, grid, dim3(256), 0, st, r, g, a, b, cap);
}

void launch_dft_record_dump(hipStream_t st, const DftDumpP& r, const float* dump, float2* acc, long long cells, long long fstride,
                            const float2* phase, int nf) {
  const dim3 grid((unsigned)((cells + 255) / 256), (unsigned)r.n);
  hipLaunchKernelGGL(dft_record_dump_kernel, grid, dim3(256), 0, st, r, dump, acc, cells, fstride, phase, nf);
}

void launch_seams(hipStream_t st, const GridP& g, const FieldP& b, const StepP& s, const MatP& m, const float* seam,
                  int n_seams, const DampT& dmp, const ClipP& clip, const InjP& inj, const SrcP& sr) {
  const long long nt = (long long)n_seams * (clip.j1 - clip.j0) * (clip.k1 - clip.k0);
  if (nt <= 0) return;
  const unsigned blocks = (unsigned)((nt + 255) / 256);
  hipLaunchKernelGGL(seam_kernel, dim3(blocks), dim3(256), 0, st, g, b, s, m, seam, n_seams, dmp, clip, inj, sr);
}

}
```

tidy3d_amd/csrc/fdtd_fused2.hpp:

```cpp
#pragma once
#include "fdtd_kernels.hpp"

namespace fdtd {

constexpr int kMaxInj = 256;
struct InjP {
  int n;
  const int* start;
  const int4* ent;
  const float* val;
  const float* val2;
  int e2_in_sweep;
  float* cap;
  const int* dstart;
  const int* dlist;
  const struct DumpBox* dboxes;
  float* dump;
};
struct DumpBox {
  int lo0, lo1, lo2, nx, ny, nz;
  int off[6];
};
constexpr int kMaxDumps = 8;
struct DampT {
  const float* fb[3];
  const float* fc[3];
  int e2;
};
struct ClipP { int i0, i1, j0, j1, k0, k1; };
struct TileClassP { const unsigned char* cls; };
struct DispP {
  const int* dseg;
  const float* cs;
  float* e1;
};
struct SrcT {
  const float* e1;
  const float* h2;
  const float* e2;
  int use_h2, use_e2;
  const float* e1b;
  const float* h2b;
  const float* e2b;
};
struct SrcP {
  const int* sseg = nullptr;
  const SrcT* t = nullptr;
};
#if !defined(FDTD_NO_EXJ)
#define FDTD_NO_EXJ 0
#endif
constexpr bool fused2_exj(int lb, int opt) { return !FDTD_NO_EXJ && (opt & 8) == 0 && !(lb == 512 && (opt & 2) != 0); }
constexpr int fused2_xch_arrays(int lb, int opt) { return fused2_exj(lb, opt) ? 9 : 8; }
constexpr size_t fused2_lds_bytes(int lb, int opt, int waves) {
  return ((size_t)fused2_xch_arrays(lb, opt) * waves * 64 + ((opt & 8) ? 2 * 64 : 0)) * sizeof(float4) + ((opt & 2) ? (size_t)kMaxMedia * sizeof(float2) : 0);
}
static_assert(fused2_lds_bytes(1024, 1 | 2 | 4 | 16 | 32 | 64, 16) <= 160 * 1024 && fused2_lds_bytes(1024, 2 | 8, 16) <= 160 * 1024 &&
              2 * fused2_lds_bytes(512, 1, 8) <= 160 * 1024 && 2 * fused2_lds_bytes(512, 2 | 8, 8) <= 160 * 1024,
              "fused2_step_kernel: LDS of a workgroup (two per CU for eight waves)");
constexpr int kMaxCap = 1024;
constexpr int kSeamArrays = 13;

void launch_inject_values(hipStream_t st, float* val, const float* w_re, const float* w_im, const float2* wave,
                          long long step, int n);
void launch_fused2_step(hipStream_t st, int waves, int opt, int grid_blocks, const GridP& g, const FieldP& a,
                        const FieldP& b, const StepP& s, const MatP& m, int zchunk, int nbx, int nby, int nbz,
                        int xcd_remap, const InjP& inj, float* seam, const DampT& dmp, const ClipP& clip, const TileClassP& tcl = TileClassP{nullptr},
                        const DispP& dp = DispP{nullptr, nullptr, nullptr}, const SrcP& sr = SrcP{});
void launch_fused2_step_src(hipStream_t st, int waves, int opt, int grid_blocks, const GridP& g, const FieldP& a,
                            const FieldP& b, const StepP& s, const MatP& m, int zchunk, int nbx, int nby, int nbz,
                            int xcd_remap, const InjP& inj, float* seam, const DampT& dmp, const ClipP& clip, const TileClassP& tcl, const DispP& dp, const SrcP& sr);
void launch_fused2_step_whatif(hipStream_t st, int waves, int opt, int grid_blocks, const GridP& g, const FieldP& a,
                               const FieldP& b, const StepP& s, const MatP& m, int zchunk, int nbx, int nby, int nbz,
                               int xcd_remap, const InjP& inj, float* seam, const DampT& dmp, const ClipP& clip);
void launch_fused2_step_disp(hipStream_t st, int waves, int opt, int grid_blocks, const GridP& g, const FieldP& a,
                             const FieldP& b, const StepP& s, const MatP& m, int zchunk, int nbx, int nby, int nbz,
                             int xcd_remap, const InjP& inj, float* seam, const DampT& dmp, const ClipP& clip, const TileClassP& tcl, const DispP& dp);
void launch_fused2_step_clip(hipStream_t st, int waves, int opt, int grid_blocks, const GridP& g, const FieldP& a,
                             const FieldP& b, const StepP& s, const MatP& m, int zchunk, int nbx, int nby, int nbz,
                             int xcd_remap, const InjP& inj, float* seam, const DampT& dmp, const ClipP& clip, const TileClassP& tcl = TileClassP{nullptr});
void launch_inject_table(hipStream_t st, float* tab, long long stride, long long off, const float* w_re, const float* w_im,
                         const float2* wave, long long n_steps, int n);
constexpr int kPairMons = 4;
struct PairRecP {
  int n_mon;
  int pre_done;
  BoxP box[kPairMons];
  int nc[kPairMons];
  int comp[kPairMons][6];
  int cap_off[kPairMons];
  float* out_n[kPairMons];
  float* out_m[kPairMons];
};
void launch_pair_record(hipStream_t st, const PairRecP& r, long long max_cells, const GridP& g, const FieldP& a, const FieldP& b,
                        const float* cap);
struct DftDumpP { int n; int slot[3]; int off[3]; };
void launch_dft_record_dump(hipStream_t st, const DftDumpP& r, const float* dump, float2* acc, long long cells, long long fstride,
                            const float2* phase, int nf);
void launch_seams(hipStream_t st, const GridP& g, const FieldP& b, const StepP& s, const MatP& m, const float* seam,
                  int n_seams, const DampT& dmp, const ClipP& clip, const InjP& inj, const SrcP& sr = SrcP{});

}
```

tidy3d_amd/csrc/fdtd_fused2w.hip:

```cpp
#include <hip/hip_runtime.h>
#undef __global__
#if defined(__HIPCC__)
#define __global__ static __attribute__((global))
#else
#define __global__ static
#endif
#include "fdtd_kernels2.hpp"

namespace fdtd {

void launch_fused2_step_whatif(hipStream_t st, int waves, int opt, int grid_blocks, const GridP& g, const FieldP& a,
                               const FieldP& b, const StepP& s, const MatP& m, int zchunk, int nbx, int nby, int nbz,
                               int xcd_remap, const InjP& inj, float* seam, const DampT& dmp, const ClipP& clip) {
  const dim3 grid(grid_blocks, 1, 1), block(64, waves, 1);
  const int wv = opt >> 8;
  const size_t shmem = ((size_t)(wv == 13 ? 9 : ((wv >= 10 && wv <= 12) ? 6 + (wv == 11 ? 2 : 3) : 8)) * waves * 64) * sizeof(float4);
  const TileClassP tcl{nullptr};
  const DispP dp{nullptr, nullptr, nullptr};
#define FDTD_F2_W(WV)                                                                                                  \
  case WV: hipLaunchKernelGGL((fused2_step_kernel<1024, 1 | (WV << 8)>), grid, block, shmem, st, g, a, b, s, m, zchunk, nbx, nby,  \
                              nbz, xcd_remap, inj, seam, dmp, clip, tcl, dp, SrcP{}); break
  switch (opt >> 8) {
    FDTD_F2_W(1); FDTD_F2_W(2); FDTD_F2_W(3); FDTD_F2_W(4); FDTD_F2_W(5); FDTD_F2_W(6); FDTD_F2_W(7); FDTD_F2_W(8);
    FDTD_F2_W(10); FDTD_F2_W(11); FDTD_F2_W(12); FDTD_F2_W(13); FDTD_F2_W(14); FDTD_F2_W(15);
    default: break;
  }
#undef FDTD_F2_W
}

}
```

tidy3d_amd/csrc/fdtd_kernels2.hpp:

```cpp
#pragma once
#include "fdtd_fused2.hpp"

namespace fdtd {

__global__ __launch_bounds__(256) void pair_record_kernel(PairRecP r, GridP g, FieldP a, FieldP b, const float* cap) {
  const int mi = blockIdx.y / 6, ic = blockIdx.y % 6;
  if (mi >= r.n_mon || ic >= r.nc[mi]) return;
  const BoxP bx = r.box[mi];
  const long long cells = (long long)bx.nx * bx.ny * bx.nz;
  const long long t = (long long)blockIdx.x * blockDim.x + threadIdx.x;
  if (t >= cells) return;
  const int c = r.comp[mi][ic];
  const int lx = (int)(t % bx.nx), ly = (int)((t / bx.nx) % bx.ny), lz = (int)(t / ((long long)bx.nx * bx.ny));
  const long long p = (long long)(bx.lo2 + lz) * g.sxy + (long long)(bx.lo1 + ly) * g.nx + bx.lo0 + lx;
  const long long idx = (long long)ic * cells + t;
  const float* fa = c == 0 ? a.ex : (c == 1 ? a.ey : (c == 2 ? a.ez : (c == 3 ? a.hx : (c == 4 ? a.hy : a.hz))));
  const float* fb = c == 0 ? b.ex : (c == 1 ? b.ey : (c == 2 ? b.ez : (c == 3 ? b.hx : (c == 4 ? b.hy : b.hz))));
  const float mid = cap[r.cap_off[mi] + idx];
  float* on = r.out_n[mi];
  float* om = r.out_m[mi];
  if (c < 3) {
    if (on && !r.pre_done) on[idx] = 1.0f * fa[p];
    if (om) om[idx] = 1.0f * mid;
  } else {
    if (on) { float o = on[idx]; if (!r.pre_done) o = o + 0.5f * fa[p]; o = o + 0.5f * mid; on[idx] = o; }
    if (om) { float o = om[idx]; o = o + 0.5f * mid; o = o + 0.5f * fb[p]; om[idx] = o; }
  }
}

__global__ __launch_bounds__(256) void dft_record_dump_kernel(DftDumpP r, const float* dump, float2* acc, long long cells,
                                                              long long fstride, const float2* phase, int nf) {
  const int q = blockIdx.y;
  const long long t = (long long)blockIdx.x * blockDim.x + threadIdx.x;
  if (t >= cells || q >= r.n) return;
  const float v = dump[r.off[q] + t];
  float2* a0 = acc + (long long)r.slot[q] * cells;
  for (int k = 0; k < nf; ++k) {
    const float2 ph = phase[k];
    float2 a = a0[(long long)k * fstride + t];
    a.x += v * ph.x;
    a.y += v * ph.y;
    a0[(long long)k * fstride + t] = a;
  }
}

__global__ __launch_bounds__(256) void inject_table_kernel(float* tab, long long stride, long long off, const float* w_re,
                                                           const float* w_im, const float2* wave, long long n_steps, int n) {
  const long long g = (long long)blockIdx.x * blockDim.x + threadIdx.x;
  if (g >= n_steps * n) return;
  const long long step = g / n;
  const int t = (int)(g % n);
  const float2 a = wave[step];
  tab[step * stride + off + t] = w_re[t] * a.x - w_im[t] * a.y;
}

__global__ __launch_bounds__(256) void inject_values_kernel(float* val, const float* w_re, const float* w_im,
                                                            const float2* wave, long long step, int n) {
  const int t = threadIdx.x;
  if (t >= n) return;
  const float2 a = wave[step];
  val[t] = w_re[t] * a.x - w_im[t] * a.y;
}

__device__ __forceinline__ long long seam_at(const GridP& g, int seam, int arr, int j, int k) {
  return (((long long)seam * kSeamArrays + arr) * (g.nz + 2) + (k + 1)) * g.ny + j;
}

__device__ __forceinline__ float lane_next(float v) {
#if defined(__HIP_DEVICE_COMPILE__)
  const int x = __builtin_bit_cast(int, v);
  return __builtin_bit_cast(float, __builtin_amdgcn_update_dpp(x, x, 0x130, 0xf, 0xf, false));
#else
  return __shfl_down(v, 1);
#endif
}
__device__ __forceinline__ float lane_prev(float v) {
#if defined(__HIP_DEVICE_COMPILE__)
  const int x = __builtin_bit_cast(int, v);
  return __builtin_bit_cast(float, __builtin_amdgcn_update_dpp(x, x, 0x138, 0xf, 0xf, false));
#else
  return __shfl_up(v, 1);
#endif
}

__device__ __forceinline__ void lds_dma16(const float* base, unsigned off, float4* dst, int lane) {
#if defined(__HIP_DEVICE_COMPILE__)
  const unsigned lds_addr = __builtin_amdgcn_readfirstlane((unsigned)(size_t)dst);
  unsigned keep;
  asm volatile("s_mov_b32 %0, m0\n\ts_mov_b32 m0, %2\n\ts_nop 0\n\tglobal_load_lds_dwordx4 %1, %3\n\ts_mov_b32 m0, %0"
               : "=&s"(keep) : "v"(off), "s"(lds_addr), "s"(base) : "memory");
#else
  dst[lane] = *reinterpret_cast<const float4*>(reinterpret_cast<const char*>(base) + off);
#endif
}
__device__ __forceinline__ void lds_dma_wait() {
#if defined(__HIP_DEVICE_COMPILE__)
  asm volatile("s_waitcnt vmcnt(0)" ::: "memory");
#endif
}
__device__ __forceinline__ void lds_dma_fence() {
#if defined(__HIP_DEVICE_COMPILE__)
  asm volatile("s_waitcnt lgkmcnt(0)" ::: "memory");
#endif
}

__device__ __forceinline__ int opaque_lane(int v) {
#if defined(__HIP_DEVICE_COMPILE__)
  asm volatile("" : "+v"(v));
#endif
  return v;
}

__device__ __forceinline__ int lane_value(int v, int l) {
#if defined(__HIP_DEVICE_COMPILE__)
  return __builtin_amdgcn_readlane(v, l);
#else
  return __shfl(v, l);
#endif
}

template <int LB, int OPT>
__device__ __forceinline__ void fused2_step_tile(const GridP& g, const FieldP& a, const FieldP& b, const StepP& s, const MatP& m,
                                                 int zchunk, int nbx, int nby, int nbz, const InjP& inj,
                                                 float* __restrict__ seam, const DampT& dmp, const ClipP& clip, int t,
                                                 const DispP& dp, const SrcP& sr) {
  constexpr int V = 4;
  constexpr bool SRC = (OPT & 64) != 0;
  constexpr bool NT = (OPT & 1) != 0, MAT = (OPT & 2) != 0, MON = (OPT & 4) != 0;
  constexpr bool DISP = (OPT & 32) != 0;
  constexpr int WHATIF = (OPT >> 8) & 15;
  constexpr int PF = (WHATIF >= 10 && WHATIF <= 12) ? WHATIF : 0;
  constexpr bool EZL = WHATIF == 15;
  constexpr bool EXJ = (WHATIF == 0 && (OPT & 4096) == 0) || WHATIF == 13 || EZL;
  constexpr bool E1S = PF != 0 || EZL;
  constexpr int XE = E1S ? 6 : 8, XZ = 7;
  [[maybe_unused]] constexpr int NPF = PF == 11 ? 2 : (PF ? 3 : 0);
  constexpr int NXCH = E1S ? 6 : 8;
  static_assert((!PF && !EZL) || (OPT & 0xfe) == 0, "prefetch instantiations: the vacuum sweep only");
  constexpr bool DAMP = (OPT & 8) != 0;
  constexpr bool CLIP = (OPT & 16) != 0;
  const bool per_x = CLIP && g.bcx0 == BC_PERIODIC;
  const int tile_y = t % nby;
  const int tile_x = (t / nby) % nbx;
  const int tile_z = t / (nby * nbx);
  HIP_DYNAMIC_SHARED(float4, xch)
  const int tx = threadIdx.x;
  const int ty = __builtin_amdgcn_readfirstlane((int)threadIdx.y);
  const int W = blockDim.y, R = W - 3;
  const int slot = W * 64;
  const int me = ty * 64 + tx;
  {
    const float4 z4 = {0.f, 0.f, 0.f, 0.f};
#pragma unroll
    for (int q = 0; q < NXCH; ++q) xch[q * slot + me] = z4;
  }
  [[maybe_unused]] float4* xdm = xch + (EXJ ? 9 : 8) * slot;
  [[maybe_unused]] float2* lut_s = reinterpret_cast<float2*>(xdm + (DAMP ? 2 * 64 : 0));
  if constexpr (MAT) {
    for (int q = me; q < m.n_media; q += slot) lut_s[q] = m.lut[q];
  }
  if constexpr (DAMP) {
    if (ty == 0) {
      const int ii = (tile_x * 64 + tx) * V;
      float4 b4 = {1.f, 1.f, 1.f, 1.f}, c4 = {1.f, 1.f, 1.f, 1.f};
      if (ii < g.nx) { b4 = *reinterpret_cast<const float4*>(dmp.fb[0] + ii); c4 = *reinterpret_cast<const float4*>(dmp.fc[0] + ii); }
      xdm[tx] = b4; xdm[64 + tx] = c4;
    }
  }
  __syncthreads();
  const float ca = m.ca1, cb = m.cb1;
  const int k0 = (CLIP ? clip.k0 : 0) + tile_z * zchunk;
  const int k1 = min(k0 + zchunk, CLIP ? clip.k1 : g.nz);
  const int kA = k0 > 0 ? k0 - 1 : 0;
  int j = (CLIP ? clip.j0 : 0) + tile_y * R + ty - 2;
  const bool row_ok = (j >= 0) && (j < g.ny);
  if (!row_ok) {
    if constexpr (WHATIF != 6 && WHATIF != 7 && WHATIF != 8)
      for (int k = kA; k <= k1; ++k) { __syncthreads(); if constexpr (WHATIF != 2) __syncthreads(); }
    return;
  }
  const int i0 = (tile_x * 64 + tx) * V;
  const unsigned ux = (unsigned)i0;
  const unsigned ub = ux * 4u;
  const unsigned ubc = (i0 < g.nx) ? ub : 0u;
  const bool act = (i0 < g.nx);
  const bool do_e1 = ty >= 1;
  const bool do_h2 = ty >= 1 && ty <= W - 2;
  const bool own = ty >= 2 && ty <= W - 2 && (!CLIP || j < clip.j1);
  const float ch = g.ch;
  const bool last_x = (i0 + V >= g.nx);
  const bool first_x = (i0 == 0);
  const bool use_jp = (j + 1 < g.ny);
  const long long rowb = (long long)j * g.nx;
  const long long rowpb = use_jp ? rowb + g.nx : 0;
  const bool xh = act && (tx == 0) && (!first_x || per_x);
  const int im = first_x ? (per_x ? g.nx - 1 : 0) : i0 - 1;
  const bool pmc_x0 = g.bcx0 == BC_PMC, pmc_y0 = g.bcy0 == BC_PMC, pmc_z0 = !g.pec_z0;
  const bool wall_y = (j == 0) && !pmc_y0;

  [[maybe_unused]] float byv = 1.f, cyv = 1.f, bxm = 1.f, cxm = 1.f, bz_m = 1.f, cz_m = 1.f;
  if constexpr (DAMP) { byv = dmp.fb[1][j]; cyv = dmp.fc[1][j]; }
  float ipx[V], idx[V];
  zero<V>(ipx); zero<V>(idx);
  float ipx_m = 0.f;
  if (act) {
    ldv<V>(ipx, at(uni(s.ipx), ub));
    ldv<V>(idx, at(uni(s.idx), ub));
    ipx_m = s.ipx[im];
    if constexpr (DAMP) { bxm = dmp.fb[0][im]; cxm = dmp.fc[0][im]; }
  }
  const float ipy = s.ipy[j], idy = s.idy[j];

  float exk[V], eyk[V];
  float h1x[V], h1y[V], h1z[V];
  float e1x[V], e1y[V], e1z[V];
  float h2xm[V], h2ym[V];
  zero<V>(h1x); zero<V>(h1y); zero<V>(h1z); zero<V>(e1x); zero<V>(e1y); zero<V>(e1z); zero<V>(h2xm); zero<V>(h2ym);
  float exk_m = 0.f;
  float ipz_m = 0.f, idz_m = 0.f;
  int qm0 = 0, qm1 = 0;
  [[maybe_unused]] uint32_t rw_m = kBgWord;
  [[maybe_unused]] int ss_m = -1;
  {
    const long long p0 = (long long)kA * g.sxy + rowb;
    ldf<V, true>(exk, uni(a.ex + p0), ubc);
    ldf<V, true>(eyk, uni(a.ey + p0), ubc);
    if (xh) exk_m = a.ex[p0 + im];
  }
  if (kA > 0 && do_e1) {
    const long long pb = (long long)(kA - 1) * g.sxy + rowb;
    float ezm[V], ezj[V], exm[V], eym[V], ho[V], hoy[V];
    zero<V>(ezj);
    ldf<V, true>(ezm, uni(a.ez + pb), ubc);
    ldf<V, true>(exm, uni(a.ex + pb), ubc);
    ldf<V, true>(eym, uni(a.ey + pb), ubc);
    if (use_jp) ldf<V, true>(ezj, uni(a.ez + (long long)(kA - 1) * g.sxy + rowpb), ubc);
    float ezx = lane_next(ezm[0]);
    if (act && (tx == 63 || last_x)) ezx = last_x ? (per_x ? a.ez[pb] : 0.f) : a.ez[pb + ux + V];
    const float ipz = s.ipz[kA - 1];
    ldf<V, true>(ho, uni(a.hx + pb), ubc);
    ldf<V, true>(hoy, uni(a.hy + pb), ubc);
    if constexpr (DAMP) {
      const float czp = dmp.fc[2][kA - 1];
      const float4 b4 = xdm[tx], c4 = xdm[64 + tx];
      const float bx[V] = {b4.x, b4.y, b4.z, b4.w}, cx[V] = {c4.x, c4.y, c4.z, c4.w};
#pragma unroll
      for (int e = 0; e < V; ++e) { ho[e] *= bx[e] * cyv * czp; hoy[e] *= cx[e] * byv * czp; }
    }
#pragma unroll
    for (int e = 0; e < V; ++e) h1x[e] = upd_h(ho[e], ch, ezj[e] - ezm[e], ipy, eyk[e] - eym[e], ipz);
#pragma unroll
    for (int e = 0; e < V; ++e) {
      const float ez_ip = (e + 1 < V) ? ezm[(e + 1) % V] : ezx;
      h1y[e] = upd_h(hoy[e], ch, exk[e] - exm[e], ipz, ez_ip - ezm[e], ipx[e]);
    }
  }
  int cur = 0;
  const long long seam_arr = (long long)(g.nz + 2) * g.ny;
  const long long seam_row = seam_at(g, tile_x, 0, j, 0);
  struct Ld {
    float exn[V], eyn[V], ezk[V], exj[V], ezj[V], hxn[V], hyn[V], hzn[V];
    float eyx_g, ezx_g;
    float exn_m, ez_mm, ey_mm, ex_jm, hy_o, hz_o;
  };
  [[maybe_unused]] float4* pfb = xch + NXCH * slot;
  [[maybe_unused]] auto pf_issue = [&](int k) __attribute__((always_inline)) {
    if constexpr (PF != 0) {
      const long long pb = (long long)k * g.sxy + rowb;
      const long long up = (k < g.nz) ? g.sxy : 0;
      lds_dma_fence();
      if constexpr (PF == 10) {
        lds_dma16(uni(a.hx + pb), ubc, pfb + 0 * slot + ty * 64, tx);
        lds_dma16(uni(a.hy + pb), ubc, pfb + 1 * slot + ty * 64, tx);
        lds_dma16(uni(a.hz + pb), ubc, pfb + 2 * slot + ty * 64, tx);
      } else if constexpr (PF == 11) {
        lds_dma16(uni(a.ey + pb + up), ubc, pfb + 0 * slot + ty * 64, tx);
        lds_dma16(uni(a.hy + pb), ubc, pfb + 1 * slot + ty * 64, tx);
      } else {
        lds_dma16(uni(a.ex + pb + up), ubc, pfb + 0 * slot + ty * 64, tx);
        lds_dma16(uni(a.ey + pb + up), ubc, pfb + 1 * slot + ty * 64, tx);
        lds_dma16(uni(a.ez + pb), ubc, pfb + 2 * slot + ty * 64, tx);
      }
    }
  };
  [[maybe_unused]] auto pf_take = [&](int q, float (&o)[V]) __attribute__((always_inline)) {
    const float4 t4 = pfb[q * slot + me];
    o[0] = t4.x; o[1] = t4.y; o[2] = t4.z; o[3] = t4.w;
  };
  auto issue = [&](int k, Ld& L) __attribute__((always_inline)) {
    if constexpr (WHATIF == 3) {
      if (ty < 2 || ty == W - 1) {
        zero<V>(L.exn); zero<V>(L.eyn); zero<V>(L.ezk); zero<V>(L.exj); zero<V>(L.ezj); zero<V>(L.hxn); zero<V>(L.hyn); zero<V>(L.hzn);
        L.eyx_g = L.ezx_g = L.exn_m = L.ez_mm = L.ey_mm = L.ex_jm = L.hy_o = L.hz_o = 0.f;
        return;
      }
    }
    const int txo = (MAT || DAMP) ? tx : opaque_lane(tx);
    const int i0o = (tile_x * 64 + txo) * V;
    const bool act = i0o < g.nx, last_x = i0o + V >= g.nx, first_x = i0o == 0;
    const bool xh = act && txo == 0 && (!first_x || per_x);
    [[maybe_unused]] const bool wall_x0 = first_x && !pmc_x0 && !per_x;
    const long long pb = WHATIF == 4 ? (long long)(k & 1) * g.sxy : (long long)k * g.sxy + rowb;
    const long long pjb = WHATIF == 4 ? (long long)(k & 1) * g.sxy + g.nx : (long long)k * g.sxy + rowpb;
    const long long up = WHATIF == 4 ? 0 : ((k < g.nz) ? g.sxy : 0);
    if constexpr (PF != 12) ldf<V, true>(L.exn, uni(a.ex + pb + up), ubc);
    if constexpr (WHATIF == 1) zero<V>(L.eyn);
    else if constexpr (PF != 11 && PF != 12) ldf<V, true>(L.eyn, uni(a.ey + pb + up), ubc);
    if constexpr (EZL) {
      if (k == kA) ldf<V, true>(L.ezk, uni(a.ez + pb), ubc);
      else { const float4 t4 = xch[XZ * slot + me]; L.ezk[0] = t4.x; L.ezk[1] = t4.y; L.ezk[2] = t4.z; L.ezk[3] = t4.w; }
    } else if constexpr (PF != 12) ldf<V, true>(L.ezk, uni(a.ez + pb), ubc);
    if (use_jp) {
      if constexpr (EXJ) {
        if (ty == W - 1 || k == kA) ldf<V, true>(L.exj, uni(a.ex + pjb), ubc);
        else { const float4 t4 = xch[XE * slot + me + 64]; L.exj[0] = t4.x; L.exj[1] = t4.y; L.exj[2] = t4.z; L.exj[3] = t4.w; }
      } else {
        ldf<V, true>(L.exj, uni(a.ex + pjb), ubc);
      }
      if constexpr (EZL) {
        if (ty == W - 1 || k == kA) ldf<V, true>(L.ezj, uni(a.ez + pjb), ubc);
        else { const float4 t4 = xch[XZ * slot + me + 64]; L.ezj[0] = t4.x; L.ezj[1] = t4.y; L.ezj[2] = t4.z; L.ezj[3] = t4.w; }
      } else {
        ldf<V, true>(L.ezj, uni(a.ez + pjb), ubc);
      }
    } else {
      zero<V>(L.exj); zero<V>(L.ezj);
    }
    if constexpr (PF != 10) ldf<V, true>(L.hxn, uni(a.hx + pb), ubc);
    if constexpr (WHATIF == 1) zero<V>(L.hyn);
    else if constexpr (PF != 10 && PF != 11) ldf<V, true>(L.hyn, uni(a.hy + pb), ubc);
    if constexpr (PF != 10) ldf<V, true>(L.hzn, uni(a.hz + pb), ubc);
    L.eyx_g = 0.f; L.ezx_g = 0.f;
    if (act && txo == 63 && !last_x) { L.eyx_g = a.ey[pb + ux + V]; L.ezx_g = a.ez[pb + ux + V]; }
    if (per_x && act && last_x) { L.eyx_g = a.ey[pb]; L.ezx_g = a.ez[pb]; }
    L.exn_m = 0.f; L.ez_mm = 0.f; L.ey_mm = 0.f; L.ex_jm = 0.f; L.hy_o = 0.f; L.hz_o = 0.f;
    if (xh && do_e1) {
      const long long pm = pb + im;
      L.exn_m = a.ex[pm + up];
      L.ez_mm = a.ez[pm]; L.ey_mm = a.ey[pm];
      L.ex_jm = use_jp ? a.ex[pjb + im] : 0.f;
      L.hy_o = a.hy[pm]; L.hz_o = a.hz[pm];
    }
    if constexpr (PF != 0) {
      lds_dma_wait();
      if constexpr (PF == 10) { pf_take(0, L.hxn); pf_take(1, L.hyn); pf_take(2, L.hzn); }
      else if constexpr (PF == 11) { pf_take(0, L.eyn); pf_take(1, L.hyn); }
      else { pf_take(0, L.exn); pf_take(1, L.eyn); pf_take(2, L.ezk); }
    }
  };
  Ld LA, LB2;
  auto body = [&](int k, Ld& L) __attribute__((always_inline)) {
    const int txo = (MAT || DAMP) ? tx : opaque_lane(tx);
    const int i0o = (tile_x * 64 + txo) * V;
    const bool act = i0o < g.nx, last_x = i0o + V >= g.nx, first_x = i0o == 0;
    const bool xh = act && txo == 0 && (!first_x || per_x);
    [[maybe_unused]] const bool wall_x0 = first_x && !pmc_x0 && !per_x;
    const bool seam_l = (txo == 63 && !last_x) || (per_x && last_x), seam_r = txo == 0 && (tile_x > 0 || per_x);
    const long long seam_back = (tile_x > 0 ? -1 : (long long)(nbx - 1)) * kSeamArrays * seam_arr;
    const long long pb = (long long)k * g.sxy + rowb;
    const float ipz = s.ipz[k], idz = s.idz[k];
    [[maybe_unused]] float bzk = 1.f, czk = 1.f;
    if constexpr (DAMP) { bzk = dmp.fb[2][min(k, g.nz - 1)]; czk = dmp.fc[2][min(k, g.nz - 1)]; }
    int q0 = 0, q1 = 0;
    if (inj.n > 0) { q0 = inj.start[k]; q1 = inj.start[k + 1]; }
    [[maybe_unused]] int d0 = 0, d1 = 0;
    if constexpr (MON) { if (inj.dstart) { d0 = inj.dstart[k]; d1 = inj.dstart[k + 1]; } }
    float hy_m = 0.f, hz_m = 0.f;
    float (&exn)[V] = L.exn, (&eyn)[V] = L.eyn, (&ezk)[V] = L.ezk, (&exj)[V] = L.exj, (&ezj)[V] = L.ezj;
    float (&hxn)[V] = L.hxn, (&hyn)[V] = L.hyn, (&hzn)[V] = L.hzn;
    [[maybe_unused]] uint32_t rw = kBgWord;
    if constexpr (MAT) {
      if (do_e1) rw = m.roww[((long long)min(k, g.nz - 1) * g.ny + j) * nbx + tile_x];
    }
    [[maybe_unused]] int ss = -1;
    if constexpr (SRC) {
      if (do_e1 && k < g.nz) ss = sr.sseg[((long long)k * g.ny + j) * nbx + tile_x];
    }
    [[maybe_unused]] int ds = -1;
    if constexpr (DISP) {
      if (do_e1 && k < g.nz) ds = dp.dseg[((long long)k * g.ny + j) * nbx + tile_x];
    }
    if constexpr (WHATIF == 7) {
      issue(k, L);
      if (own && k > k0 && act) {
        const long long po = pb - g.sxy + i0;
        float o0[V], o1[V], o2[V];
#pragma unroll
        for (int e = 0; e < V; ++e) { o0[e] = L.exn[e] + L.exj[e]; o1[e] = L.ezk[e] + L.ezj[e]; o2[e] = L.eyn[e]; }
        stv_h<V, NT>(b.ex + po, o0); stv_h<V, NT>(b.ey + po, o2); stv_h<V, NT>(b.ez + po, o1);
        stv_h<V, NT>(b.hx + po, L.hxn); stv_h<V, NT>(b.hy + po, L.hyn); stv_h<V, NT>(b.hz + po, L.hzn);
      }
      return;
    }
    {
      issue(k, L);
      float eyx = lane_next(eyk[0]);
      float ezx = lane_next(ezk[0]);
      if (act && (txo == 63 || last_x)) {
        if (!last_x || per_x) { eyx = L.eyx_g; ezx = L.ezx_g; }
        else { eyx = 0.f; ezx = 0.f; }
      }
      if constexpr (DAMP) {
        {
          const float4 b4 = xdm[tx];
          const float bx[V] = {b4.x, b4.y, b4.z, b4.w};
#pragma unroll
          for (int e = 0; e < V; ++e) hxn[e] *= bx[e] * cyv * czk;
        }
        {
          const float4 c4 = xdm[64 + tx];
          const float cx[V] = {c4.x, c4.y, c4.z, c4.w};
#pragma unroll
          for (int e = 0; e < V; ++e) { hyn[e] *= cx[e] * byv * czk; hzn[e] *= cx[e] * cyv * bzk; }
        }
        L.hy_o *= cxm * byv * czk;
        L.hz_o *= cxm * cyv * bzk;
      }
#pragma unroll
      for (int e = 0; e < V; ++e) {
        const float ey_ip = (e + 1 < V) ? eyk[(e + 1) % V] : eyx;
        const float ez_ip = (e + 1 < V) ? ezk[(e + 1) % V] : ezx;
        hxn[e] = upd_h(hxn[e], ch, ezj[e] - ezk[e], ipy, eyn[e] - eyk[e], ipz);
        hyn[e] = upd_h(hyn[e], ch, exn[e] - exk[e], ipz, ez_ip - ezk[e], ipx[e]);
        hzn[e] = upd_h(hzn[e], ch, ey_ip - eyk[e], ipx[e], exj[e] - exk[e], ipy);
// ... 112 lines not shown
            } else if (MON && en.z >= (DISP ? 11 : 8) && own && k >= k0 && k < k1) {
              const int c = en.z - 8;
#pragma unroll
              for (int e = 0; e < V; ++e) {
                if (d == e) {
                  float mid = c == 0 ? e1xn[e] : (c == 1 ? e1yn[e] : (c == 2 ? e1zn[e] : (c == 3 ? hxn[e] : (c == 4 ? hyn[e] : hzn[e]))));
                  if constexpr (DAMP) {
                    const float4 b4 = xdm[tx], c4 = xdm[64 + tx];
                    const float bx[V] = {b4.x, b4.y, b4.z, b4.w}, cx[V] = {c4.x, c4.y, c4.z, c4.w};
                    if (c == 0) mid *= cx[e] * byv * bzk; else if (c == 1) mid *= bx[e] * cyv * bzk; else if (c == 2) mid *= bx[e] * byv * czk;
                  }
                  inj.cap[en.w] = mid;
                }
              }
            }
          }
        }
        if constexpr (DAMP) {
          {
            const float4 c4 = xdm[64 + tx];
            const float cx[V] = {c4.x, c4.y, c4.z, c4.w};
#pragma unroll
            for (int e = 0; e < V; ++e) e1xn[e] *= cx[e] * byv * bzk;
          }
          {
            const float4 b4 = xdm[tx];
            const float bx[V] = {b4.x, b4.y, b4.z, b4.w};
#pragma unroll
            for (int e = 0; e < V; ++e) { e1yn[e] *= bx[e] * cyv * bzk; e1zn[e] *= bx[e] * byv * czk; }
          }
        }
        if constexpr (DISP) {
          if (ds >= 0 && act) {
            const long long qb = ((long long)ds * 3) * 256 + tx * V;
            float cx[V], cy[V], cz[V];
            ldv<V>(cx, dp.cs + qb); ldv<V>(cy, dp.cs + qb + 256); ldv<V>(cz, dp.cs + qb + 512);
#pragma unroll
            for (int e = 0; e < V; ++e) { e1xn[e] = e1xn[e] - cx[e]; e1yn[e] = e1yn[e] - cy[e]; e1zn[e] = e1zn[e] - cz[e]; }
            if (own && k >= k0 && k < k1 && (!CLIP || (i0o >= clip.i0 && i0o < clip.i1))) {
              stv<V>(dp.e1 + qb, e1xn); stv<V>(dp.e1 + qb + 256, e1yn); stv<V>(dp.e1 + qb + 512, e1zn);
            }
          }
          if constexpr (MON) {
            if (own && k >= k0 && k < k1) {
              for (int qb = q0; qb < q1; qb += 64) {
                int4 ev = {0, -1, 0, 0};
                if (qb + tx < q1) ev = inj.ent[qb + tx];
                unsigned long long hit = __ballot(ev.y == j && ev.z >= 8 && ev.z < 11);
                while (hit) {
                  const int l = __ffsll(hit) - 1;
                  hit &= hit - 1;
                  const int d = lane_value(ev.x, l) - i0, c = lane_value(ev.z, l) - 8, w = lane_value(ev.w, l);
#pragma unroll
                  for (int e = 0; e < V; ++e)
                    if (d == e) inj.cap[w] = c == 0 ? e1xn[e] : (c == 1 ? e1yn[e] : e1zn[e]);
                }
              }
            }
          }
        }
        if constexpr (MON) {
          if (own && k >= k0 && k < k1) {
            for (int q = d0; q < d1; ++q) {
              const DumpBox bx = inj.dboxes[inj.dlist[q]];
              const int ly = j - bx.lo1, lz = k - bx.lo2;
              if (ly >= 0 && ly < bx.ny) {
                const long long rowo = ((long long)lz * bx.ny + ly) * bx.nx;
#pragma unroll
                for (int e = 0; e < V; ++e) {
                  const int lx = i0o + e - bx.lo0;
                  if (lx >= 0 && lx < bx.nx && act && (!CLIP || (i0o + e >= clip.i0 && i0o + e < clip.i1))) {
                    if (bx.off[0] >= 0) inj.dump[bx.off[0] + rowo + lx] = e1xn[e];
                    if (bx.off[1] >= 0) inj.dump[bx.off[1] + rowo + lx] = e1yn[e];
                    if (bx.off[2] >= 0) inj.dump[bx.off[2] + rowo + lx] = e1zn[e];
                    if (bx.off[3] >= 0) inj.dump[bx.off[3] + rowo + lx] = hxn[e];
                    if (bx.off[4] >= 0) inj.dump[bx.off[4] + rowo + lx] = hyn[e];
                    if (bx.off[5] >= 0) inj.dump[bx.off[5] + rowo + lx] = hzn[e];
                  }
                }
              }
            }
          }
        }
        if ((CLIP || (own && k >= k0 && k < k1)) && act) {
          float* sp = seam + seam_row + (long long)k * g.ny;
          if (seam_l) {
            sp[0] = hyn[V - 1];
            sp[seam_arr] = hzn[V - 1];
            sp[2 * seam_arr] = e1xn[V - 1];
            sp[3 * seam_arr] = e1yn[V - 1];
            sp[4 * seam_arr] = e1zn[V - 1];
          }
          if (seam_r) {
            sp[5 * seam_arr + seam_back] = e1yn[0];
            sp[6 * seam_arr + seam_back] = e1zn[0];
          }
        }
      }
    }
    float h2x[V], h2y[V], h2z[V];
    unspecified<V>(h2x); unspecified<V>(h2y); unspecified<V>(h2z);
    if (do_h2 && k > kA) {
      if constexpr (DAMP) {
        {
          const float4 b4 = xdm[tx];
          const float bx[V] = {b4.x, b4.y, b4.z, b4.w};
#pragma unroll
          for (int e = 0; e < V; ++e) h1x[e] *= bx[e] * cyv * cz_m;
        }
        {
          const float4 c4 = xdm[64 + tx];
          const float cx[V] = {c4.x, c4.y, c4.z, c4.w};
#pragma unroll
          for (int e = 0; e < V; ++e) { h1y[e] *= cx[e] * byv * cz_m; h1z[e] *= cx[e] * cyv * bz_m; }
        }
      }
      if constexpr (SRC) {
        if (ss_m >= 0 && act && sr.t->use_h2) {
          const long long qs = ((long long)ss_m * 3) * 256 + tx * V;
          float tx_[V], ty_[V], tz_[V];
          ldv<V>(tx_, sr.t->h2 + qs); ldv<V>(ty_, sr.t->h2 + qs + 256); ldv<V>(tz_, sr.t->h2 + qs + 512);
#pragma unroll
          for (int e = 0; e < V; ++e) { h1x[e] = h1x[e] + tx_[e]; h1y[e] = h1y[e] + ty_[e]; h1z[e] = h1z[e] + tz_[e]; }
          if (sr.t->h2b) {
            ldv<V>(tx_, sr.t->h2b + qs); ldv<V>(ty_, sr.t->h2b + qs + 256); ldv<V>(tz_, sr.t->h2b + qs + 512);
#pragma unroll
            for (int e = 0; e < V; ++e) { h1x[e] = h1x[e] + tx_[e]; h1y[e] = h1y[e] + ty_[e]; h1z[e] = h1z[e] + tz_[e]; }
          }
        }
      }
      if constexpr (MON) {
        if (inj.val2) {
          for (int qb = qm0; qb < qm1; qb += 64) {
            int4 ev = {0, -1, 8, 0};
            if (qb + tx < qm1) ev = inj.ent[qb + tx];
            unsigned long long hit = __ballot(ev.y == j && ev.z >= 3 && ev.z < 8);
            while (hit) {
              const int l = __ffsll(hit) - 1;
              hit &= hit - 1;
              const int d = lane_value(ev.x, l) - i0o, code = lane_value(ev.z, l);
              const float v = inj.val2[lane_value(ev.w, l)];
#pragma unroll
              for (int e = 0; e < V; ++e) {
                const bool mine = d == e;
                h1x[e] = (mine && code == 3) ? h1x[e] + v : h1x[e];
                h1y[e] = (mine && code == 4) ? h1y[e] + v : h1y[e];
                h1z[e] = (mine && code == 5) ? h1z[e] + v : h1z[e];
              }
            }
          }
        }
      }
      float eyx = lane_next(e1y[0]);
      float ezx = lane_next(e1z[0]);
      if (txo == 63 || last_x) { eyx = 0.f; ezx = 0.f; }
      float4 t0, t1;
      if constexpr (WHATIF == 6) {
        t0 = make_float4(e1x[0], e1x[1], e1x[2], e1x[3]); t1 = make_float4(e1z[0], e1z[1], e1z[2], e1z[3]);
      } else {
        t0 = xch[(4 + (E1S ? 0 : (cur ^ 1) * 2) + 0) * slot + me + 64];
        t1 = xch[(4 + (E1S ? 0 : (cur ^ 1) * 2) + 1) * slot + me + 64];
      }
      const float exj1[V] = {t0.x, t0.y, t0.z, t0.w}, ezj1[V] = {t1.x, t1.y, t1.z, t1.w};
#pragma unroll
      for (int e = 0; e < V; ++e) {
        const float ey_ip = (e + 1 < V) ? e1y[(e + 1) % V] : eyx;
        const float ez_ip = (e + 1 < V) ? e1z[(e + 1) % V] : ezx;
// ... 77 lines not shown
      const bool wall_z = (k - 1 == 0) && !pmc_z0;
      float ex[V], ey[V], ez[V];
      auto s4 = [&](auto coef) __attribute__((always_inline)) {
#pragma unroll
        for (int e = 0; e < V; ++e) {
          const float hy_im = (e > 0) ? h2y[(e + V - 1) % V] : hyx;
          const float hz_im = (e > 0) ? h2z[(e + V - 1) % V] : hzx;
          float nex = upd_e(e1x[e], coef(0, e).x, coef(0, e).y, h2z[e] - hzj[e], idy, h2y[e] - h2ym[e], idz_m);
          float ney = upd_e(e1y[e], coef(1, e).x, coef(1, e).y, h2x[e] - h2xm[e], idz_m, h2z[e] - hz_im, idx[e]);
          float nez = upd_e(e1z[e], coef(2, e).x, coef(2, e).y, h2y[e] - hy_im, idx[e], h2x[e] - hxj[e], idy);
          const bool wx = wall_x0 && (e == 0);
          if (wall_y || wall_z) nex = 0.f;
          if (wx || wall_z) ney = 0.f;
          if (wx || wall_y) nez = 0.f;
          ex[e] = nex; ey[e] = ney; ez[e] = nez;
        }
      };
      if constexpr (MAT) {
        if (rw_m != kMixedWord) {
          const float2 c0 = lut_s[rw_m & 1023u], c1 = lut_s[(rw_m >> 10) & 1023u], c2 = lut_s[(rw_m >> 20) & 1023u];
          s4([&](int c, int) { return c == 0 ? c0 : (c == 1 ? c1 : c2); });
        } else {
          uint32_t mw_m[V] = {kBgWord, kBgWord, kBgWord, kBgWord};
          if (act) ldm<V>(mw_m, at(uni(m.m4 + pb - g.sxy), ub));
          s4([&](int c, int e) { return lut_s[(mw_m[e] >> (10 * c)) & 1023u]; });
        }
      } else {
        const float2 c1 = make_float2(ca, cb);
        s4([&](int, int) { return c1; });
      }
      if constexpr (SRC) {
        if (ss_m >= 0 && act && sr.t->use_e2) {
          const long long qs = ((long long)ss_m * 3) * 256 + tx * V;
          float tx_[V], ty_[V], tz_[V];
          ldv<V>(tx_, sr.t->e2 + qs); ldv<V>(ty_, sr.t->e2 + qs + 256); ldv<V>(tz_, sr.t->e2 + qs + 512);
#pragma unroll
          for (int e = 0; e < V; ++e) { ex[e] = ex[e] + tx_[e]; ey[e] = ey[e] + ty_[e]; ez[e] = ez[e] + tz_[e]; }
          if (sr.t->e2b) {
            ldv<V>(tx_, sr.t->e2b + qs); ldv<V>(ty_, sr.t->e2b + qs + 256); ldv<V>(tz_, sr.t->e2b + qs + 512);
#pragma unroll
            for (int e = 0; e < V; ++e) { ex[e] = ex[e] + tx_[e]; ey[e] = ey[e] + ty_[e]; ez[e] = ez[e] + tz_[e]; }
          }
        }
      }
      if (inj.val2 && inj.e2_in_sweep) {
        for (int qb = qm0; qb < qm1; qb += 64) {
          int4 ev = {0, -1, 8, 0};
          if (qb + tx < qm1) ev = inj.ent[qb + tx];
          unsigned long long hit = __ballot(ev.y == j && ev.z < 3);
          while (hit) {
            const int l = __ffsll(hit) - 1;
            hit &= hit - 1;
            const int d = lane_value(ev.x, l) - i0, code = lane_value(ev.z, l);
            const float v = inj.val2[lane_value(ev.w, l)];
#pragma unroll
            for (int e = 0; e < V; ++e) {
              if (d == e) {
                if (code == 0) ex[e] += v;
                else if (code == 1) ey[e] += v;
                else ez[e] += v;
              }
            }
          }
        }
      }
      if constexpr (DAMP) {
        if (dmp.e2) {
          {
            const float4 c4 = xdm[64 + tx];
            const float cx[V] = {c4.x, c4.y, c4.z, c4.w};
#pragma unroll
            for (int e = 0; e < V; ++e) ex[e] *= cx[e] * byv * bz_m;
          }
          {
            const float4 b4 = xdm[tx];
            const float bx[V] = {b4.x, b4.y, b4.z, b4.w};
#pragma unroll
            for (int e = 0; e < V; ++e) { ey[e] *= bx[e] * cyv * bz_m; ez[e] *= bx[e] * byv * cz_m; }
          }
        }
      }
      if (act && (!CLIP || (i0o >= clip.i0 && i0o < clip.i1))) {
        float* sq = seam + seam_row + (long long)(k - 1) * g.ny;
        if (!CLIP && txo == 63 && !last_x) {
          sq[7 * seam_arr] = h2x[V - 1];
          sq[8 * seam_arr] = h2y[V - 2];
          sq[9 * seam_arr] = h2z[V - 2];
        }
        if (!CLIP && txo == 0 && tile_x > 0) {
          sq[10 * seam_arr - kSeamArrays * seam_arr] = h2x[0];
          sq[11 * seam_arr - kSeamArrays * seam_arr] = h2y[0];
          sq[12 * seam_arr - kSeamArrays * seam_arr] = h2z[0];
        }
        const long long po = pb - g.sxy + i0;
        if (WHATIF != 5 || ex[0] == 3.0e38f) {
          stv_h<V, NT>(b.hx + po, h2x);
          stv_h<V, NT>(b.hy + po, h2y);
          stv_h<V, NT>(b.hz + po, h2z);
          stv_h<V, NT>(b.ex + po, ex);
          stv_h<V, NT>(b.ey + po, ey);
          stv_h<V, NT>(b.ez + po, ez);
        }
      }
    }
#pragma unroll
    for (int e = 0; e < V; ++e) {
      h2xm[e] = h2x[e]; h2ym[e] = h2y[e];
      h1x[e] = hxn[e]; h1y[e] = hyn[e]; h1z[e] = hzn[e];
      e1x[e] = e1xn[e]; e1y[e] = e1yn[e]; e1z[e] = e1zn[e];
      exk[e] = exn[e]; eyk[e] = eyn[e];
    }
    exk_m = L.exn_m;
    ipz_m = ipz; idz_m = idz;
    qm0 = q0; qm1 = q1;
    if constexpr (DAMP) { bz_m = bzk; cz_m = czk; }
    if constexpr (MAT) rw_m = rw;
    if constexpr (SRC) ss_m = ss;
    cur ^= 1;
  };
  if constexpr (PF != 0) pf_issue(kA);
  for (int k = kA; k <= k1; k += 2) {
    body(k, LA);
    if (k + 1 <= k1) body(k + 1, LB2);
  }
}

template <int LB, int OPT>
__device__ __forceinline__ void fused2_tile_by_class(const GridP& g, const FieldP& a, const FieldP& b, const StepP& s, const MatP& m,
                                                     int zchunk, int nbx, int nby, int nbz, const InjP& inj, float* __restrict__ seam,
                                                     const DampT& dmp, const ClipP& clip, int t, const DispP& dp, const SrcP& sr, const TileClassP& tcl) {
  if constexpr ((OPT & 2) != 0) {
    if (tcl.cls) {
      const int cl = tcl.cls[t] & 3;
      if (cl == 0) {
        fused2_step_tile<LB, (OPT & ~(2 | 32))>(g, a, b, s, m, zchunk, nbx, nby, nbz, inj, seam, dmp, clip, t, dp, sr);
        return;
      }
      if constexpr ((OPT & 32) != 0) {
        if (cl == 1) {
          fused2_step_tile<LB, (OPT & ~32)>(g, a, b, s, m, zchunk, nbx, nby, nbz, inj, seam, dmp, clip, t, dp, sr);
          return;
        }
      }
    }
  }
  fused2_step_tile<LB, OPT>(g, a, b, s, m, zchunk, nbx, nby, nbz, inj, seam, dmp, clip, t, dp, sr);
}

template <int LB, int OPT>
__global__ __launch_bounds__(LB, (LB == 512 ? 4 : 1)) void fused2_step_kernel(GridP g, FieldP a, FieldP b, StepP s, MatP m,
                                                         int zchunk, int nbx, int nby, int nbz, int xcd_remap,
                                                         InjP inj, float* __restrict__ seam, DampT dmp, ClipP clip, TileClassP tcl, DispP dp, SrcP sr) {
  const int total = nbx * nby * nbz;
  int t = blockIdx.x;
  if (xcd_remap == 1) {
    const int per = (total + 7) >> 3;
    t = (t & 7) * per + (t >> 3);
    if (t >= total) return;
  } else if (xcd_remap > 1) {
    const int G = xcd_remap, full = total / (8 * G) * (8 * G);
    if (t < full) {
      const int x = t & 7, mloc = t >> 3;
      t = ((mloc / G) * 8 + x) * G + mloc % G;
    }
    if (t >= total) return;
  }
  constexpr int OPTK = OPT | (fused2_exj(LB, OPT) ? 0 : 4096);
  if constexpr ((OPT & 64) != 0) {
    if (tcl.cls && !(tcl.cls[t] & 4)) {
      fused2_tile_by_class<LB, (OPTK & ~64)>(g, a, b, s, m, zchunk, nbx, nby, nbz, inj, seam, dmp, clip, t, dp, sr, tcl);
      return;
    }
  }
  fused2_tile_by_class<LB, OPTK>(g, a, b, s, m, zchunk, nbx, nby, nbz, inj, seam, dmp, clip, t, dp, sr, tcl);
}

__global__ __launch_bounds__(256) void seam_kernel(GridP g, FieldP b, StepP s, MatP m,
                                                   const float* __restrict__ seam, int n_seams, DampT dmp, ClipP clip, InjP inj, SrcP sr) {
  const long long t = (long long)blockIdx.x * blockDim.x + threadIdx.x;
  const int nj = clip.j1 - clip.j0;
  const long long per = (long long)nj * (clip.k1 - clip.k0);
  if (t >= per * n_seams) return;
  const int sm = (int)(t / per);
  const int k = clip.k0 + (int)((t % per) / nj), j = clip.j0 + (int)(t % nj);
  const bool wrap = g.bcx0 == BC_PERIODIC && sm == n_seams - 1;
  const int c = wrap ? g.nx : (sm + 1) * 256;
  const int cc = wrap ? 0 : c;
  const bool wl = c - 1 >= clip.i0 && c - 1 < clip.i1, wr = cc >= clip.i0 && cc < clip.i1;
  if (!wl && !wr) return;
  const float ch = g.ch;
  const float ipx = s.ipx[c - 1];
  auto A = [&](int a, int jj, int kk) { return seam[seam_at(g, sm, a, jj, kk)]; };
  auto h2 = [&](int jj, int kk, float& hy, float& hz) {
    const float e1x = A(2, jj, kk), e1y = A(3, jj, kk), e1z = A(4, jj, kk);
    const float e1x_jp = (jj + 1 < g.ny) ? A(2, jj + 1, kk) : 0.f;
    float h1y = A(0, jj, kk), h1z = A(1, jj, kk);
    if (dmp.fb[0]) {
      const float cxv = dmp.fc[0][c - 1];
      h1y *= cxv * dmp.fb[1][jj] * dmp.fc[2][kk];
      h1z *= cxv * dmp.fc[1][jj] * dmp.fb[2][kk];
    }
    if (sr.sseg && sr.t->use_h2) {
      const int blk = sr.sseg[((long long)kk * g.ny + jj) * ((g.nx + 255) >> 8) + ((c - 1) >> 8)];
      if (blk >= 0) {
        const long long qs = ((long long)blk * 3) * 256 + ((c - 1) & 255);
        h1y = h1y + sr.t->h2[qs + 256];
        h1z = h1z + sr.t->h2[qs + 512];
        if (sr.t->h2b) { h1y = h1y + sr.t->h2b[qs + 256]; h1z = h1z + sr.t->h2b[qs + 512]; }
      }
    }
    hy = upd_h(h1y, ch, A(2, jj, kk + 1) - e1x, s.ipz[kk], A(6, jj, kk) - e1z, ipx);
    hz = upd_h(h1z, ch, A(5, jj, kk) - e1y, ipx, e1x_jp - e1x, s.ipy[jj]);
  };
  float hy_m, hz_m;
  h2(j, k, hy_m, hz_m);
  const bool pmc_y0 = g.bcy0 == BC_PMC, pmc_z0 = !g.pec_z0;
  const bool wall_y = (j == 0) && !pmc_y0, wall_z = (k == 0) && !pmc_z0;
  const bool mir_y = (j == 0) && pmc_y0, mir_z = (k == 0) && pmc_z0;
  const long long pr = (long long)k * g.sxy + (long long)j * g.nx;
  const long long p = pr + cc, pl = pr + c - 1;
  if (wl) { b.hy[pl] = hy_m; b.hz[pl] = hz_m; }
  const float idy = s.idy[j], idz = s.idz[k], idx_m = s.idx[c - 1], idx_c = s.idx[cc];
  const float hx_m = A(7, j, k), hy_mm = A(8, j, k), hz_mm = A(9, j, k);
  const float hx_c = A(10, j, k), hy_c = A(11, j, k), hz_c = A(12, j, k);
  auto coef = [&](long long cell, int c) {
    return m.m4 ? m.lut[(m.m4[cell] >> (10 * c)) & 1023u] : make_float2(m.ca1, m.cb1);
  };
  float ex_m = 0.f, ey_m = 0.f, ez_m = 0.f, ey_c = 0.f, ez_c = 0.f;
  float hy_k = 0.f, hz_j = 0.f, dum;
  if (mir_z) hy_k = -hy_m; else if (!wall_z) h2(j, k - 1, hy_k, dum);
  if (mir_y) hz_j = -hz_m; else if (!wall_y) h2(j - 1, k, dum, hz_j);
  const float hxm_k = wall_z ? 0.f : (mir_z ? -hx_m : A(7, j, k - 1)), hxc_k = wall_z ? 0.f : (mir_z ? -hx_c : A(10, j, k - 1));
  const float hxm_j = wall_y ? 0.f : (mir_y ? -hx_m : A(7, j - 1, k)), hxc_j = wall_y ? 0.f : (mir_y ? -hx_c : A(10, j - 1, k));
  if (!wall_y && !wall_z) { const float2 q = coef(pl, 0); ex_m = upd_e(A(2, j, k), q.x, q.y, hz_m - hz_j, idy, hy_m - hy_k, idz); }
  if (!wall_z) {
    const float2 qm = coef(pl, 1), qc = coef(p, 1);
    ey_m = upd_e(A(3, j, k), qm.x, qm.y, hx_m - hxm_k, idz, hz_m - hz_mm, idx_m);
    ey_c = upd_e(A(5, j, k), qc.x, qc.y, hx_c - hxc_k, idz, hz_c - hz_m, idx_c);
  }
  if (!wall_y) {
    const float2 qm = coef(pl, 2), qc = coef(p, 2);
    ez_m = upd_e(A(4, j, k), qm.x, qm.y, hy_m - hy_mm, idx_m, hx_m - hxm_j, idy);
    ez_c = upd_e(A(6, j, k), qc.x, qc.y, hy_c - hy_m, idx_c, hx_c - hxc_j, idy);
  }
  if (sr.sseg && sr.t->use_e2) {
    const int nbxg = (g.nx + 255) >> 8;
    const int bl = sr.sseg[((long long)k * g.ny + j) * nbxg + ((c - 1) >> 8)], br = sr.sseg[((long long)k * g.ny + j) * nbxg + (cc >> 8)];
    if (bl >= 0) {
      const long long qs = ((long long)bl * 3) * 256 + ((c - 1) & 255);
      ex_m = ex_m + sr.t->e2[qs]; ey_m = ey_m + sr.t->e2[qs + 256]; ez_m = ez_m + sr.t->e2[qs + 512];
      if (sr.t->e2b) { ex_m = ex_m + sr.t->e2b[qs]; ey_m = ey_m + sr.t->e2b[qs + 256]; ez_m = ez_m + sr.t->e2b[qs + 512]; }
    }
    if (br >= 0) {
      const long long qs = ((long long)br * 3) * 256 + (cc & 255);
      ey_c = ey_c + sr.t->e2[qs + 256]; ez_c = ez_c + sr.t->e2[qs + 512];
      if (sr.t->e2b) { ey_c = ey_c + sr.t->e2b[qs + 256]; ez_c = ez_c + sr.t->e2b[qs + 512]; }
    }
  }
  if (inj.val2 && inj.e2_in_sweep) {
    const int q0 = inj.start[k], q1 = inj.start[k + 1];
    for (int q = q0; q < q1; ++q) {
      const int4 en = inj.ent[q];
      if (en.y != j || en.z >= 3) continue;
      const float v = inj.val2[en.w];
      if (en.x == c - 1) { if (en.z == 0) ex_m += v; else if (en.z == 1) ey_m += v; else ez_m += v; }
      else if (en.x == cc) { if (en.z == 1) ey_c += v; else if (en.z == 2) ez_c += v; }
    }
  }
  if (dmp.fb[0] && dmp.e2) {
    const float bxm = dmp.fb[0][c - 1], cxm = dmp.fc[0][c - 1], bxc = dmp.fb[0][cc];
    const float byv = dmp.fb[1][j], cyv = dmp.fc[1][j], bzv = dmp.fb[2][k], czv = dmp.fc[2][k];
    ex_m *= cxm * byv * bzv; ey_m *= bxm * cyv * bzv; ez_m *= bxm * byv * czv;
    ey_c *= bxc * cyv * bzv; ez_c *= bxc * byv * czv;
  }
  if (wl) { b.ex[pl] = ex_m; b.ey[pl] = ey_m; b.ez[pl] = ez_m; }
  if (wr) { b.ey[p] = ey_c; b.ez[p] = ez_c; }
}

}
```

tidy3d_amd/engine.py:

```python
from __future__ import annotations

import ctypes as C
from typing import Callable, Dict, List, Optional, Tuple

import numpy as np

from . import lib as L
from .coeffs import damping_tables, h_coeff, inv_steps, material_table, pml_axis
from .exceptions import SetupError, SolverLibraryError
from .spec import BC_PERIODIC, MonitorSpec, SolverSpec


def _f32(a) -> np.ndarray:
    return np.ascontiguousarray(np.asarray(a, dtype=np.float32))


def _ptr(a: np.ndarray):
    return a.ctypes.data_as(C.c_void_p)


def _cplx_f32(a) -> np.ndarray:
    a = np.asarray(a, dtype=np.complex128)
    out = np.empty(a.shape + (2,), dtype=np.float32)
    out[..., 0] = a.real
# ... 463 lines not shown
            wre, wim = _f32(s.w_re[keep]), _f32(s.w_im[keep])
            we, wh = _cplx_f32(s.wave_e), _cplx_f32(s.wave_h)
            self._chk(d.fdtd_add_point_source(h, len(cell), _ptr(comp), _ptr(cell), _ptr(wre),
                                              _ptr(wim), len(s.wave_e), _ptr(we), _ptr(wh)),
                      "fdtd_add_point_source")
        for t in spec.tfsf:
            def loc(ijk, *arrs):
                k = ijk[:, 2]
                keep = (k >= z0) & (k < z1)
                ij = ijk[keep]
                cell = ((ij[:, 2] - z0).astype(np.int64) * sxy + ij[:, 1].astype(np.int64) * nx
                        + ij[:, 0]).astype(np.uint32)
                return [cell] + [np.ascontiguousarray(a[keep]) for a in arrs]
            ecell, ecomp, ew, eaux = loc(t.e_corr_ijk, t.e_corr_comp.astype(np.int32),
                                         t.e_corr_w.astype(np.float32), t.e_corr_aux.astype(np.int32))
            hcell, hcomp, hw, haux = loc(t.h_corr_ijk, t.h_corr_comp.astype(np.int32),
                                         t.h_corr_w.astype(np.float32), t.h_corr_aux.astype(np.int32))
            ae, be, ah, bh, wave = _f32(t.ae), _f32(t.be), _f32(t.ah), _f32(t.bh), _f32(t.wave)
            self._chk(d.fdtd_add_tfsf(h, t.n_aux, _ptr(ae), _ptr(be), _ptr(ah), _ptr(bh),
                                      int(t.src_cell), len(wave),
                                      _ptr(wave), len(ecell), _ptr(ecomp), _ptr(ecell), _ptr(ew),
                                      _ptr(eaux), len(hcell), _ptr(hcomp), _ptr(hcell), _ptr(hw),
                                      _ptr(haux)), "fdtd_add_tfsf")
        self.mon_ids: List[Tuple[MonitorSpec, int, Tuple[int, int]]] = []
        for m in spec.monitors:
            lo2, hi2 = max(m.lo[2], z0), min(m.hi[2], z1)
            if hi2 <= lo2:
                self.mon_ids.append((m, -1, (0, 0)))
                continue
            comps = np.asarray(m.comps, dtype=np.int32)
            lo = np.asarray([m.lo[0], m.lo[1], lo2 - z0], dtype=np.int32)
            hi = np.asarray([m.hi[0], m.hi[1], hi2 - z0], dtype=np.int32)
            steps = np.ascontiguousarray(m.steps, dtype=np.int64)
            if m.kind == "dft":
                pe, ph = _cplx_f32(m.phase_e), _cplx_f32(m.phase_h)
                mid = d.fdtd_add_monitor(h, L.MON_DFT, len(comps), _ptr(comps), _ptr(lo), _ptr(hi),
                                         len(steps), _ptr(steps), len(m.freqs), _ptr(pe), _ptr(ph))
            else:
                mid = d.fdtd_add_monitor(h, L.MON_TIME, len(comps), _ptr(comps), _ptr(lo), _ptr(hi),
                                         len(steps), _ptr(steps), 0, None, None)
            self._chk(mid, "fdtd_add_monitor")
            self.mon_ids.append((m, mid, (lo2, hi2)))
        self._chk(d.fdtd_set_shutoff(h, int(spec.decay_every), float(spec.shutoff),
                                     int(spec.decay_ref_step)), "fdtd_set_shutoff")

    def unique_id(self) -> bytes:
        buf = C.create_string_buffer(128)
        self.lib.check(self.lib.dll.fdtd_comm_unique_id(buf), None, "fdtd_comm_unique_id")
        return buf.raw

    def comm_init(self, uid: bytes):
        buf = C.create_string_buffer(uid, 128)
        self._chk(self.lib.dll.fdtd_comm_init(self.handle, buf, self.rank, self.n_ranks),
                  "fdtd_comm_init")

    def run(self, n_steps: Optional[int] = None,
            progress: Optional[Callable[[int, float, float], bool]] = None) -> L.FdtdStats:
        n_steps = self.spec.n_steps if n_steps is None else n_steps
        dt = self.spec.dt

        def _cb(step, _t, decay, _user):
            try:
                return 1 if (progress and progress(int(step), step * dt, float(decay))) else 0
            except KeyboardInterrupt:
                return 1
        cb = L.PROGRESS_FN(_cb) if progress else C.cast(None, L.PROGRESS_FN)
        if self.twin is not None:
            ph = (C.c_double * 3)(*[float(v) for v in self.spec.bloch])
            nr = (C.c_int * 3)(*[int(v) for v in self.n_real])
            self._chk(self.lib.dll.fdtd_run_bloch(self.handle, self.twin.handle, int(n_steps), ph, nr, cb, None),
                      "fdtd_run_bloch")
        else:
            self._chk(self.lib.dll.fdtd_run(self.handle, int(n_steps), cb, None), "fdtd_run")
        return self.stats()

    def stats(self) -> L.FdtdStats:
        st = L.FdtdStats()
        self._chk(self.lib.dll.fdtd_get_stats(self.handle, C.byref(st)), "fdtd_get_stats")
        if int(st.struct_bytes) != C.sizeof(L.FdtdStats):
            raise SolverLibraryError(f"'{self.lib.path}' fills an FdtdStats of {int(st.struct_bytes)} bytes, this binding expects "
                                     f"{C.sizeof(L.FdtdStats)}: rebuild the library (python -m tidy3d_amd.build)")
        return st

    def set_option(self, key: int, value: int):
        self._chk(self.lib.dll.fdtd_set_option(self.handle, key, value), "fdtd_set_option")

    def reset(self):
        self._chk(self.lib.dll.fdtd_reset(self.handle), "fdtd_reset")
        if self.twin is not None:
            self.twin.reset()

    def _dev_comp(self, comp: int) -> int:
        return (comp % 3 - self.axis_shift) % 3 + 3 * (comp // 3)

    def get_field(self, comp: int) -> np.ndarray:
        dc = self._dev_comp(comp)
        a = self._get_field_real(dc)
        if self.twin is not None:
            a = a + 1j * self.twin._get_field_real(dc)
        return unpermute_array(a, self.axis_shift)

    def _get_field_real(self, comp: int) -> np.ndarray:
        nx, ny, _ = self.spec.shape
        out = np.empty((self.nzl, ny, self.nxp), dtype=np.float32)
        self._chk(self.lib.dll.fdtd_get_field(self.handle, comp, _ptr(out), out.nbytes),
                  "fdtd_get_field")
        if any(self.ghost):
            gx, gy = self.ghost[0], self.ghost[1]
            ux, uy = self.user_shape[0], self.user_shape[1]
            return np.ascontiguousarray(out[:, gy:gy + uy, gx:gx + ux])
        return np.ascontiguousarray(out[..., :nx]) if self.pad_x else out

    def set_field(self, comp: int, arr: np.ndarray):
        if self.axis_shift:
            sig = [(a + self.axis_shift) % 3 for a in range(3)]
            arr = np.transpose(np.asarray(arr), tuple(2 - sig[2 - q] for q in range(3)))
            comp = self._dev_comp(comp)
            shift, self.axis_shift = self.axis_shift, 0
            try:
                return self.set_field(comp, arr)
            finally:
                self.axis_shift = shift
        if self.twin is not None:
            self.twin.set_field(comp, np.imag(arr))
            arr = np.real(arr)
        a = _f32(arr)
        if any(self.ghost):
            gx, gy = self.ghost[0], self.ghost[1]
            a = _f32(np.pad(a, ((0, 0), (gy, gy), (gx, gx))))
        if self.pad_x:
            a = _f32(np.pad(a, ((0, 0), (0, 0), (0, self.pad_x))))
        self._chk(self.lib.dll.fdtd_set_field(self.handle, comp, _ptr(a), a.nbytes),
                  "fdtd_set_field")

    def monitor_data(self) -> Dict[str, Tuple[np.ndarray, Tuple[int, int]]]:
        out = {}
        for m, mid, (lo2, hi2) in self.mon_ids:
            if mid < 0:
                continue
            bz, by, bx = hi2 - lo2, m.hi[1] - m.lo[1], m.hi[0] - m.lo[0]
            if m.kind == "dft":
                arr = np.empty((len(m.freqs), len(m.comps), bz, by, bx), dtype=np.complex64)
            else:
                arr = np.empty((len(m.steps), len(m.comps), bz, by, bx), dtype=np.float32)
            self._chk(self.lib.dll.fdtd_get_monitor(self.handle, mid, _ptr(arr), arr.nbytes),
                      "fdtd_get_monitor")
            out[m.name] = (arr, (lo2, hi2))
        if self.twin is not None:
            im = self.twin.monitor_data()
            for m, mid, _ in self.mon_ids:
                if mid >= 0:
                    out[m.name] = (out[m.name][0] + 1j * im[m.name][0], out[m.name][1])
        if self.axis_shift:
            out = {k: (unpermute_array(v[0], self.axis_shift), self.user_zrange[k]) for k, v in out.items()}
        return out

    def results(self) -> Dict[str, np.ndarray]:
        return {k: v[0] for k, v in self.monitor_data().items()}

    def close(self):
        if getattr(self, "twin", None) is not None:
            self.twin.close()
            self.twin = None
        if getattr(self, "handle", None) and self.handle.value:
            self.lib.dll.fdtd_destroy(self.handle)
            self.handle = C.c_void_p()
# ... 14 lines not shown
```

tidy3d_amd/lib.py:

```python
from __future__ import annotations

import ctypes as C
import os
from typing import Optional

from .exceptions import SolverLibraryError

_HERE = os.path.dirname(os.path.abspath(__file__))
DEFAULT_LIB = os.path.join(_HERE, "libfdtd_hip.so")



def _prefer_hw_queues() -> None:
    os.environ.setdefault("GPU_MAX_HW_QUEUES", "8")


SYMBOLS = (
    "fdtd_last_error", "fdtd_device_count", "fdtd_create", "fdtd_destroy", "fdtd_set_steps",
    "fdtd_set_media", "fdtd_set_material", "fdtd_set_material16", "fdtd_set_pml", "fdtd_set_absorber", "fdtd_add_ade",
    "fdtd_add_point_source", "fdtd_add_tfsf", "fdtd_add_monitor", "fdtd_get_monitor",
    "fdtd_set_field", "fdtd_get_field", "fdtd_set_shutoff", "fdtd_comm_unique_id",
    "fdtd_comm_init", "fdtd_run", "fdtd_run_bloch", "fdtd_get_stats", "fdtd_reset", "fdtd_set_option",
    "fdtd_far_field", "fdtd_set_mirror_plus", "fdtd_add_aniso", "fdtd_add_aniso_bloch",
)

BC_PEC, BC_PMC, BC_PERIODIC, BC_NEIGHBOR = 0, 1, 2, 3
MON_TIME, MON_DFT = 0, 1
VARIANT_AUTO, VARIANT_SIMPLE, VARIANT_ZMARCH, VARIANT_FUSED = 0, 1, 2, 3
FLAG_TIME_KERNELS = 1
OPT_FLAGS, OPT_VARIANT, OPT_ZCHUNK, OPT_ROWS, OPT_XCD_REMAP, OPT_FUSED_LB, OPT_PML_FUSED, OPT_BND_PLANES, OPT_AUTOTUNE, OPT_PML_SPLIT, OPT_LDS_PAD, OPT_MEM_HINTS, OPT_PLACEMENT_TRIES, OPT_TBLOCK, OPT_EDGE_ZCHUNK, OPT_GRAPH, OPT_TWOSTEP, OPT_SHELL_PAIRS, OPT_STRIP, OPT_SHELL2, OPT_SHELL2_SHAPE, OPT_DEBUG_SYNC, OPT_TILE_SPLIT, OPT_DISP, OPT_WHATIF, OPT_SRC_PAGED, OPT_SLAB_BOXES_FIRST = 0, 1, 2, 3, 4, 5, 6, 7, 8, 9, 10, 11, 12, 13, 14, 15, 16, 17, 18, 19, 20, 21, 22, 23, 24, 25, 26
F2_OFF_REASONS = {0: "", 1: "switched off", 2: "grid too small", 3: "z-slab rank", 4: "CPML (shell pairs not possible)",
                  5: "dispersive media not confined to a few planes along z", 6: "TFSF box while it injects", 7: "Bloch / PMC-plus faces (or rows not a multiple of 4 cells)", 8: "magnetic sources with absorber layers",
                  9: "magnetic source node on a tile seam", 10: "too many source nodes", 11: "two-pass kernels",
                  12: "CPML shell too large a part of the grid", 13: "no device memory for the third field set"}


class FdtdConfig(C.Structure):
    _fields_ = [("nx", C.c_int32), ("ny", C.c_int32), ("nz", C.c_int32),
                ("bc", C.c_int32 * 6), ("device", C.c_int32), ("variant", C.c_int32),
                ("flags", C.c_int32), ("z_chunk", C.c_int32), ("ch", C.c_float),
                ("reserved", C.c_int32 * 6)]


class FdtdStats(C.Structure):
    _fields_ = [("steps_done", C.c_int64), ("diverged", C.c_int32), ("stopped_early", C.c_int32),
                ("field_decay", C.c_double), ("run_ms", C.c_double), ("h_kernel_ms", C.c_double),
                ("e_kernel_ms", C.c_double), ("h_kernel_launches", C.c_int64),
                ("e_kernel_launches", C.c_int64), ("device_bytes", C.c_int64),
                ("fused_kernel_ms", C.c_double), ("fused_kernel_launches", C.c_int64),
                ("tile_rows", C.c_int32), ("tile_zchunk", C.c_int32),
                ("tile_order", C.c_int32), ("placement", C.c_int32),
                ("placement_ms_first", C.c_float), ("placement_ms_kept", C.c_float),
                ("stream_overlap", C.c_int32), ("stream_retries", C.c_int32),
                ("comm_ranks", C.c_int32), ("comm_rank", C.c_int32),
                ("two_step_pairs", C.c_int64), ("tblock_planes", C.c_int32), ("reserved0", C.c_int32),
                ("graph_pairs", C.c_int64), ("fused2_pairs", C.c_int64), ("fused2_shape", C.c_int64),
                ("shell_pairs", C.c_int64), ("shell_kernel_ms", C.c_double), ("shell_kernel_launches", C.c_int64),
                ("shell2_pairs", C.c_int64),
                ("fused2_off_reason", C.c_int32), ("struct_bytes", C.c_int32), ("disp_pairs", C.c_int64),
                ("single_step_reason", C.c_int32), ("src_paged_pairs", C.c_int32),
                ("seam_kernel_ms", C.c_double), ("seam_kernel_launches", C.c_int64)]


PROGRESS_FN = C.CFUNCTYPE(C.c_int, C.c_int64, C.c_double, C.c_double, C.c_void_p)


class FdtdLib:
    def __init__(self, path: str):
        self.path = path
        try:
            self.dll = C.CDLL(path)
        except OSError as e:
            raise SolverLibraryError(f"cannot load the HIP solver library '{path}': {e}") from e
        missing = [s for s in SYMBOLS if not hasattr(self.dll, s)]
        if missing:
            raise SolverLibraryError(f"'{path}' does not export: {', '.join(missing)}")
        d = self.dll
        vp, i32, i64, f32 = C.c_void_p, C.c_int32, C.c_int64, C.c_float
        d.fdtd_last_error.restype = C.c_char_p
        d.fdtd_last_error.argtypes = [vp]
        d.fdtd_device_count.restype = C.c_int
        d.fdtd_create.argtypes = [C.POINTER(FdtdConfig), C.POINTER(vp)]
        d.fdtd_destroy.argtypes = [vp]
        d.fdtd_destroy.restype = None
        d.fdtd_set_steps.argtypes = [vp, C.c_int, vp, vp, C.c_int]
        d.fdtd_set_media.argtypes = [vp, vp, vp, C.c_int]
        d.fdtd_set_material.argtypes = [vp, vp, C.c_size_t]
        d.fdtd_set_material16.argtypes = [vp, vp, C.c_size_t]
        d.fdtd_set_pml.argtypes = [vp, C.c_int, C.c_int, C.c_int, vp, vp, vp, vp, vp, vp, C.c_int]
        d.fdtd_set_absorber.argtypes = [vp, C.c_int, C.c_int, C.c_int, vp, vp, C.c_int]
        d.fdtd_set_mirror_plus.argtypes = [vp, C.c_int, C.c_int]
        d.fdtd_add_ade.argtypes = [vp, C.c_int, i64, vp, C.c_int, vp, vp, f32]
        d.fdtd_add_aniso.argtypes = [vp, C.c_int, i64, vp, vp, vp, vp]
        d.fdtd_add_aniso_bloch.argtypes = [vp, C.c_int, i64, vp, vp, vp, vp, vp]
        d.fdtd_add_point_source.argtypes = [vp, i64, vp, vp, vp, vp, i64, vp, vp]
        d.fdtd_add_tfsf.argtypes = [vp, C.c_int, vp, vp, vp, vp, C.c_int, i64, vp,
                                    i64, vp, vp, vp, vp, i64, vp, vp, vp, vp]
        d.fdtd_add_monitor.argtypes = [vp, C.c_int, C.c_int, vp, vp, vp, i64, vp, C.c_int, vp, vp]
        d.fdtd_get_monitor.argtypes = [vp, C.c_int, vp, C.c_size_t]
        d.fdtd_set_field.argtypes = [vp, C.c_int, vp, C.c_size_t]
        d.fdtd_get_field.argtypes = [vp, C.c_int, vp, C.c_size_t]
        d.fdtd_set_shutoff.argtypes = [vp, C.c_int, C.c_double, i64]
        d.fdtd_comm_unique_id.argtypes = [vp]
        d.fdtd_comm_init.argtypes = [vp, vp, C.c_int, C.c_int]
        d.fdtd_run.argtypes = [vp, i64, PROGRESS_FN, vp]
        d.fdtd_run_bloch.argtypes = [vp, vp, i64, vp, vp, PROGRESS_FN, vp]
        d.fdtd_get_stats.argtypes = [vp, C.POINTER(FdtdStats)]
        d.fdtd_reset.argtypes = [vp]
        d.fdtd_set_option.argtypes = [vp, C.c_int, C.c_int]
        f64 = C.c_double
        d.fdtd_far_field.argtypes = [C.c_int, C.c_int, C.c_int, vp, vp, vp, vp, vp, f64, f64, f64, C.c_int, vp, vp, vp, vp]

    def far_field(self, u, v, wu, wv, currents, w0: float, k: complex, r_u, r_v, r_w, device: int = 0):
        import numpy as np
        u, v, wu, wv = (np.ascontiguousarray(a, dtype=np.float64) for a in (u, v, wu, wv))
        cur = np.ascontiguousarray(currents, dtype=np.complex128)
        assert cur.shape == (4, u.size, v.size), cur.shape
        r_u, r_v, r_w = (np.ascontiguousarray(a, dtype=np.float64) for a in (r_u, r_v, r_w))
        out = np.empty((r_u.size, 4), dtype=np.complex128)
        p = lambda a: a.ctypes.data_as(C.c_void_p)
        self.check(self.dll.fdtd_far_field(int(device), int(u.size), int(v.size), p(u), p(v), p(wu), p(wv), p(cur), float(w0),
                                           float(np.real(k)), float(np.imag(k)), int(r_u.size), p(r_u), p(r_v), p(r_w), p(out)),
                   None, "fdtd_far_field")
        return out

    def error(self, handle) -> str:
        msg = self.dll.fdtd_last_error(handle)
        return msg.decode("utf-8", "replace") if msg else ""

    def check(self, status: int, handle=None, what: str = ""):
        if status < 0:
            raise SolverLibraryError(f"{what or 'libfdtd_hip'} failed: {self.error(handle)}")
        return status


_cached: Optional[FdtdLib] = None


def load_library(path: Optional[str] = None) -> FdtdLib:
    global _cached
    if path is None and os.environ.get("TIDY3D_AMD_LIBRARY"):
        path = os.environ["TIDY3D_AMD_LIBRARY"]
        if _cached is not None and getattr(_cached, "_path", None) == path:
            return _cached
        _prefer_hw_queues()
        _cached = FdtdLib(path)
        _cached._path = path
        import sys
        print(f"tidy3d_amd: solver library overridden by $TIDY3D_AMD_LIBRARY: {path}", file=sys.stderr)
        return _cached
    if path is None:
        if _cached is not None:
            return _cached
        if not os.path.exists(DEFAULT_LIB):
            raise SolverLibraryError(
                f"{DEFAULT_LIB} not found: build it with `python -m tidy3d_amd.build` "
                "(hipcc --offload-arch=gfx950); there is no CPU fallback.")
        _prefer_hw_queues()
        _cached = FdtdLib(DEFAULT_LIB)
        return _cached
    return FdtdLib(path)
```

Before: 200,800 Mcells/s.

## Defer seam write-back into next fused sweep via a replacement buffer

The seam kernel that fixes tile-boundary cells no longer writes its corrected values into the field arrays. It stores them in a compact replacement buffer, and the next fused two-step sweep reads them from that buffer instead of from the field arrays. A flush kernel writes the pending values back before monitors, decay checks, field reads, run end or any path that cannot consume them. The goal is to remove scattered field-array stores and reloads at seams on every pair. The cost is extra kernel instantiations, more seam buffer memory, and intricate bookkeeping of the pending state that could go stale if a path misses a flush.

```diff
diff --git a/include/fdtd_hip.h b/include/fdtd_hip.h
--- a/include/fdtd_hip.h
+++ b/include/fdtd_hip.h
@@ -67,6 +67,14 @@
   double  seam_kernel_ms;
   int64_t seam_kernel_launches;
 } FdtdStats;
+
+typedef struct FdtdSeamStats {
+  int64_t seam_deferred_pairs;
+  int64_t seam_flushes;
+  int32_t seam_pending;
+  int32_t reserved;
+  double  seam_flush_ms;
+} FdtdSeamStats;
 
 enum { FDTD_F2_OFF_NONE = 0,
        FDTD_F2_OFF_DISABLED = 1,
@@ -169,8 +177,10 @@
        FDTD_OPT_SRC_PAGED = 25,
        FDTD_OPT_WHATIF = 24,
        FDTD_OPT_SLAB_BOXES_FIRST = 26,
+       FDTD_OPT_SEAM_DEFER = 27,
        FDTD_OPT_LDS_PAD = 10  };
 int fdtd_set_option(FdtdSolver* h, int key, int value);
+int fdtd_get_seam_stats(FdtdSolver* h, FdtdSeamStats* out);
 int fdtd_reset(FdtdSolver* h);
 
 #ifdef __cplusplus
diff --git a/tidy3d_amd/csrc/fdtd_capi.hip b/tidy3d_amd/csrc/fdtd_capi.hip
--- a/tidy3d_amd/csrc/fdtd_capi.hip
+++ b/tidy3d_amd/csrc/fdtd_capi.hip
@@ -271,7 +271,11 @@
   int debug_sync = 0;
   hipEvent_t ev_shell_a = nullptr, ev_shell_b = nullptr;
   hipEvent_t ev_rec = nullptr;
+  long long seam_deferred_pairs = 0, seam_flushes = 0;
+  double seam_flush_ms = 0.0;
   float* seam_buf = nullptr;
+  int seam_defer = -1;
+  bool seam_pending = false;
   float* inj_val = nullptr;
   float* cap_val = nullptr;
   float* dump_buf = nullptr;
@@ -994,8 +998,9 @@
   return &h->tile_cls.back();
 }
 
+void flush_seams(FdtdSolver* h, hipStream_t st);
 int launch_fused2(FdtdSolver* h, long long n, hipStream_t st, const F2Table* tb, bool* sources2_done, bool* damp2_done = nullptr,
-                  const ClipP* clip = nullptr, bool use_disp = false, bool e2_clip = false, const SrcP& sr = SrcP{}) {
+                  const ClipP* clip = nullptr, bool use_disp = false, bool e2_clip = false, const SrcP& sr = SrcP{}, bool defer_ok = false) {
   const bool inject = tb->with_sources;
   const GridP& g = h->g;
   if (ensure_second_set(h)) return -1;
@@ -1010,7 +1015,7 @@
   const int nbz = (box.k1 - box.k0 + zc - 1) / zc;
   const int n_seams = nbx - 1 + ((clip && h->cfg.bc[0] == FDTD_BC_PERIODIC) ? 1 : 0);
   if (!h->seam_buf && (nbx > 1 || h->cfg.bc[0] == FDTD_BC_PERIODIC) &&
-      dev_alloc(h, &h->seam_buf, (size_t)nbx * kSeamArrays * (size_t)(g.nz + 2) * (size_t)g.ny)) return -1;
+      dev_alloc(h, &h->seam_buf, seam_scratch_floats(g, nbx) + seam_rep_floats(g, nbx))) return -1;
   if (!h->inj_val && dev_alloc(h, &h->inj_val, (size_t)kMaxInj)) return -1;
   if (!h->cap_val && dev_alloc(h, &h->cap_val, (size_t)kMaxCap)) return -1;
   InjP inj{};
@@ -1061,6 +1066,7 @@
   if (use_disp) dp = DispP{h->disp.dseg, h->disp.cs, h->disp.e1};
   int opt = (h->mem_hints ? 1 : 0) | (h->mat4 ? 2 : 0) | ((tb->mons.empty() && (!tb->with_sources || h->src_h_nodes == 0) && !tb->dstart) ? 0 : 4) |
             (clip ? 16 : (h->has_damp ? 8 : 0)) | (use_disp ? 32 | 1 : 0);
+  if (h->whatif == 19 && opt == 1 && W == 16) opt |= 9 << 8;
   if (h->whatif > 0 && h->whatif <= 15 && h->whatif != 9 && opt == 1 && (W == 16 || h->whatif == 13 || h->whatif == 14)) opt |= h->whatif << 8;
   SrcP sr_used = sr;
   if (h->whatif == 9 && !sr.sseg && !(opt & 8) && (!(opt & 32) || (opt & 16))) {
@@ -1074,20 +1080,41 @@
     if (S.sseg && S.state != 1) { sr_used.sseg = S.sseg; sr_used.t = S.tab; opt |= 64 | 4 | 1; }
   }
   if (sr.sseg) { opt |= 64 | 4 | 1; *sources2_done = true; h->spg.pairs++; }
+  const bool rep_capable = n_seams > 0 && !clip && (W == 16 || h->seam_defer == 2) && (opt & ~(1 | 2 | 8)) == 0;
+  float* const rep_arr = h->seam_buf ? h->seam_buf + seam_scratch_floats(g, nbx) : nullptr;
+  if (h->seam_pending && !rep_capable) flush_seams(h, st);
+  if (h->seam_pending || (h->whatif == 17 && rep_capable)) opt |= 8192;
+  h->seam_pending = false;
+  bool defer = defer_ok && rep_capable && h->seam_defer != 0 && h->whatif == 0;
+  if (defer) {
+    bool e_post = false;
+    for (const PointSrc& s : h->psrc) e_post = e_post || (s.n_e && n + 1 < s.n_steps);
+    if ((e_post && !*sources2_done) || (h->has_damp && !dmp.e2)) defer = false;
+  }
   const int blocks = remap ? ((total + 7) / 8) * 8 : total;
   const FdtdSolver::TileClasses* tc = tile_classes(h, W, zc, box, nbx, nby, nbz, use_disp, sr_used.sseg != nullptr);
   const bool split = tc && (use_disp || sr_used.sseg || (tc->n_bg > 0 && (h->tile_split == 1 || 8 * tc->n_bg >= tc->n_all)));
   launch_fused2_step(st, W, opt, blocks, g, h->f, h->f2, sp, mp, zc, nbx, nby, nbz, remap, inj, h->seam_buf, dmp, box,
                      TileClassP{split ? tc->dev : nullptr}, dp, sr_used);
   time_end(h, st);
-  if (n_seams > 0) {
+  if (n_seams > 0 && !(rep_capable && (h->whatif == 16 || h->whatif == 17))) {
     time_begin(h, 4, st);
-    launch_seams(st, g, h->f2, sp, mp, h->seam_buf, n_seams, dmp, box, inj, sr);
+    launch_seams(st, g, h->f2, sp, mp, h->seam_buf, n_seams, dmp, box, inj, sr, (defer || (h->whatif == 18 && rep_capable)) ? rep_arr : nullptr);
     time_end(h, st);
   }
   if (use_disp) h->disp.pairs++;
   if (!clip) swap_sets(h);
-  return 0;
+  if (defer) { h->seam_pending = true; h->seam_deferred_pairs++; }
+  return 0;
+}
+void flush_seams(FdtdSolver* h, hipStream_t st) {
+  if (!h->seam_pending) return;
+  const int nbx = (h->g.nx + 255) / 256;
+  time_begin(h, 5, st);
+  launch_seam_flush(st, h->g, h->f, h->seam_buf + seam_scratch_floats(h->g, nbx), nbx - 1);
+  time_end(h, st);
+  h->seam_pending = false;
+  h->seam_flushes++;
 }
 
 struct ShellGeom { int o0[3], o1[3]; };
@@ -2876,6 +2903,7 @@
   if (comp < 0 || comp > 5) return fail(h, "fdtd_set_field: bad component");
   if (bytes != (size_t)n_cells(h) * 4) return fail(h, "fdtd_set_field: expected %zu bytes", (size_t)n_cells(h) * 4);
   HIPCHK(h, hipSetDevice(h->cfg.device));
+  if (h->seam_pending) { flush_seams(h, h->stream); HIPCHK(h, hipStreamSynchronize(h->stream)); }
   HIPCHK(h, hipMemcpy(field_ptr(h, comp), host, bytes, hipMemcpyHostToDevice));
   for (AdeGroup& a : h->ade)
     if (a.comp == comp) {
@@ -2897,6 +2925,7 @@
   if (comp < 0 || comp > 5) return fail(h, "fdtd_get_field: bad component");
   if (bytes != (size_t)n_cells(h) * 4) return fail(h, "fdtd_get_field: expected %zu bytes", (size_t)n_cells(h) * 4);
   HIPCHK(h, hipSetDevice(h->cfg.device));
+  flush_seams(h, h->stream);
   HIPCHK(h, hipStreamSynchronize(h->stream));
   HIPCHK(h, hipMemcpy(host, field_ptr(h, comp), bytes, hipMemcpyDeviceToHost));
   return 0;
@@ -2934,6 +2963,7 @@
   if (!h) return -1;
   HIPCHK(h, hipSetDevice(h->cfg.device));
   HIPCHK(h, hipStreamSynchronize(h->stream));
+  h->seam_pending = false;
   for (int c = 0; c < 6; ++c) HIPCHK(h, hipMemset(h->fbase[c], 0, h->field_bytes));
   for (int c = 0; c < 6; ++c) if (h->fbase2[c]) HIPCHK(h, hipMemset(h->fbase2[c], 0, h->field_bytes));
   for (int c = 0; c < 6; ++c) if (h->fbase3[c]) HIPCHK(h, hipMemset(h->fbase3[c], 0, h->field_bytes));
@@ -3340,6 +3370,7 @@
       h->f2_off_reason = why;
     }
     h->fused2_pairs = 0;
+    h->seam_deferred_pairs = h->seam_flushes = 0;
     h->shell_pairs = 0;
     h->shell2_pairs = 0;
     done = 0;
@@ -3501,6 +3532,7 @@
   int begin_step() {
     n = h->step;
     rec = !fused_multi && rec_at(n);
+    if (rec) flush_seams(h, st);
     if (rec && multi) {
       HIPCHK(h, hipStreamWaitEvent(st, h->ev_e_bnd, 0));
       HIPCHK(h, hipStreamWaitEvent(st, h->ev_h_bnd, 0));
@@ -3694,7 +3726,11 @@
     bool sources2_done = false, damp2_done = true;
     launch_sources(h, false, n, 0, nz, st);
     if (pair_spg) spg_fill(h, n, st);
-    if (launch_fused2(h, n, st, tb, &sources2_done, &damp2_done, nullptr, pair_disp, false, pair_spg ? spg_params(h) : SrcP{})) return -1;
+    const auto decay_at = [&](long long m) { return h->decay_every > 0 && (m % h->decay_every) == 0; };
+    const bool defer_ok = done + 4 <= n_steps && !decay_at(n + 2) && !decay_at(n + 3) && !rec_at(n + 1) && !rec_at(n + 2) && !rec_at(n + 3) &&
+                          !pair_disp && !pair_spg && h->tfsf.empty() && h->src_h_nodes == 0 && h->cfg.bc[4] != FDTD_BC_PERIODIC && !multi &&
+                          !h->step_dev_mode && !h->debug_sync;
+    if (launch_fused2(h, n, st, tb, &sources2_done, &damp2_done, nullptr, pair_disp, false, pair_spg ? spg_params(h) : SrcP{}, defer_ok)) return -1;
     pair_record(h, tb, n, st);
     if (rec_at(n + 1)) record_monitors(h, n + 1, true, st);
     if (!sources2_done) launch_sources(h, true, n + 1, 0, nz, st);
@@ -3795,6 +3831,7 @@
     return 0;
   }
   int finish() {
+    flush_seams(h, st);
     if (multi) {
       HIPCHK(h, hipStreamWaitEvent(st, h->ev_e_bnd, 0));
       HIPCHK(h, hipStreamWaitEvent(st, h->ev_h_bnd, 0));
@@ -3809,7 +3846,7 @@
     HIPCHK(h, hipEventElapsedTime(&ms, h->ev0, h->ev1));
     h->stats.run_ms = ms;
     h->stats.steps_done = h->step;
-    h->stats.h_kernel_ms = h->stats.e_kernel_ms = h->stats.fused_kernel_ms = h->stats.shell_kernel_ms = h->stats.seam_kernel_ms = 0.0;
+    h->stats.h_kernel_ms = h->stats.e_kernel_ms = h->stats.fused_kernel_ms = h->stats.shell_kernel_ms = h->stats.seam_kernel_ms = h->seam_flush_ms = 0.0;
     h->stats.h_kernel_launches = h->stats.e_kernel_launches = h->stats.fused_kernel_launches = h->stats.shell_kernel_launches = h->stats.seam_kernel_launches = 0;
     for (size_t i = 0; i < h->kev_kind.size(); ++i) {
       float t = 0.f;
@@ -3818,6 +3855,7 @@
       else if (h->kev_kind[i] == 1) { h->stats.e_kernel_ms += t; h->stats.e_kernel_launches++; }
       else if (h->kev_kind[i] == 3) { h->stats.shell_kernel_ms += t; h->stats.shell_kernel_launches++; }
       else if (h->kev_kind[i] == 4) { h->stats.seam_kernel_ms += t; h->stats.seam_kernel_launches++; }
+      else if (h->kev_kind[i] == 5) h->seam_flush_ms += t;
       else { h->stats.fused_kernel_ms += t; h->stats.fused_kernel_launches++; }
     }
     return 0;
@@ -3825,6 +3863,7 @@
   int loop() {
     for (; done < n_steps; ++done) {
       if (begin_step()) return -1;
+      if (h->seam_pending && !(!fused_multi && pair && !use_s2 && !f2s_ok && f2_ok)) flush_seams(h, st);
       if (fused_multi) {
         const int rc = slab_rank_step();
         if (rc < 0) return -1;
@@ -3889,7 +3928,7 @@
   HIPCHK(h, hipSetDevice(h->cfg.device));
   Run r{h, n_steps, progress, user};
   if (r.setup() || r.setup_schedules() || r.setup_pairs()) return -1;
-  if (r.loop()) return -1;
+  if (r.loop()) { flush_seams(h, h->stream); return -1; }
   return r.finish();
 }
 int fdtd_run_bloch(FdtdSolver* hr, FdtdSolver* hi, int64_t n_steps, const double phase[3], const int n_real[3],
@@ -4137,7 +4176,8 @@
       if (h->spg.state == -1 && value != 0) h->spg.state = 0;
       return 0;
     case FDTD_OPT_SLAB_BOXES_FIRST: if (value < 0 || value > 3) break; h->slab_boxes_first = value; return 0;
-    case FDTD_OPT_WHATIF: if (value < 0 || value > 15) break; h->whatif = value; return 0;
+    case FDTD_OPT_WHATIF: if (value < 0 || value > 19) break; h->whatif = value; return 0;
+    case FDTD_OPT_SEAM_DEFER: if (value > 2) break; h->seam_defer = value < 0 ? -1 : value; return 0;
     case FDTD_OPT_DISP:
       if (h->disp.state == 1 && value == 0) break;
       h->disp_on = value < 0 ? -1 : (value != 0);
@@ -4185,4 +4225,14 @@
   return 0;
 }
 
-}
+int fdtd_get_seam_stats(FdtdSolver* h, FdtdSeamStats* out) {
+  if (!h || !out) return -1;
+  out->seam_deferred_pairs = h->seam_deferred_pairs;
+  out->seam_flushes = h->seam_flushes;
+  out->seam_pending = h->seam_pending ? 1 : 0;
+  out->reserved = 0;
+  out->seam_flush_ms = h->seam_flush_ms;
+  return 0;
+}
+
+}
diff --git a/tidy3d_amd/csrc/fdtd_fused2.hip b/tidy3d_amd/csrc/fdtd_fused2.hip
--- a/tidy3d_amd/csrc/fdtd_fused2.hip
+++ b/tidy3d_amd/csrc/fdtd_fused2.hip
@@ -1,4 +1,6 @@
 #include <hip/hip_runtime.h>
+#include <cstdio>
+#include <cstdlib>
 #undef __global__
 #if defined(__HIPCC__)
 #define __global__ static __attribute__((global))
@@ -21,7 +23,7 @@
     launch_fused2_step_src(st, waves, opt, grid_blocks, g, a, b, s, m, zchunk, nbx, nby, nbz, xcd_remap, inj, seam, dmp, clip, tcl, dp, sr);
     return;
   }
-  if (opt >> 8) {
+  if ((opt >> 8) & 15) {
     launch_fused2_step_whatif(st, waves, opt, grid_blocks, g, a, b, s, m, zchunk, nbx, nby, nbz, xcd_remap, inj, seam, dmp, clip);
     return;
   }
@@ -34,6 +36,15 @@
     return;
   }
   const dim3 grid(grid_blocks, 1, 1), block(64, waves, 1);
+  if (opt & 8192) {
+#define FDTD_F2_R(OV) \
+  case OV: hipLaunchKernelGGL((fused2_step_kernel<1024, OV | 8192>), grid, block, fused2_lds_bytes(1024, OV, waves), st, g, a, b, s, m, zchunk, nbx, \
+                              nby, nbz, xcd_remap, inj, seam, dmp, clip, tcl, dp, sr); break
+    switch (opt & 15) { FDTD_F2_R(0); FDTD_F2_R(1); FDTD_F2_R(2); FDTD_F2_R(3); FDTD_F2_R(8); FDTD_F2_R(9); FDTD_F2_R(10); FDTD_F2_R(11);
+      default: fprintf(stderr, "launch_fused2_step: no deferred-seam instantiation of the sweep for opt %d\n", opt); abort(); }
+#undef FDTD_F2_R
+    return;
+  }
 #define FDTD_F2_O(LBV, OV)                                                                                             \
   hipLaunchKernelGGL((fused2_step_kernel<LBV, OV>), grid, block, fused2_lds_bytes(LBV, OV, waves), st, g, a, b, s, m, zchunk, nbx, nby, nbz,     \
                      xcd_remap, inj, seam, dmp, clip, tcl, dp, sr)
@@ -74,11 +85,17 @@
 }
 
 void launch_seams(hipStream_t st, const GridP& g, const FieldP& b, const StepP& s, const MatP& m, const float* seam,
-                  int n_seams, const DampT& dmp, const ClipP& clip, const InjP& inj, const SrcP& sr) {
+                  int n_seams, const DampT& dmp, const ClipP& clip, const InjP& inj, const SrcP& sr, float* rep) {
   const long long nt = (long long)n_seams * (clip.j1 - clip.j0) * (clip.k1 - clip.k0);
   if (nt <= 0) return;
   const unsigned blocks = (unsigned)((nt + 255) / 256);
-  hipLaunchKernelGGL(seam_kernel, dim3(blocks), dim3(256), 0, st, g, b, s, m, seam, n_seams, dmp, clip, inj, sr);
+  hipLaunchKernelGGL(seam_kernel, dim3(blocks), dim3(256), 0, st, g, b, s, m, seam, n_seams, dmp, clip, inj, sr, rep);
+}
+
+void launch_seam_flush(hipStream_t st, const GridP& g, const FieldP& b, const float* rep, int n_seams) {
+  const long long nt = (long long)n_seams * g.ny * g.nz;
+  if (nt <= 0) return;
+  hipLaunchKernelGGL(seam_flush_kernel, dim3((unsigned)((nt + 255) / 256)), dim3(256), 0, st, g, b, rep, n_seams);
 }
 
 }
diff --git a/tidy3d_amd/csrc/fdtd_fused2.hpp b/tidy3d_amd/csrc/fdtd_fused2.hpp
--- a/tidy3d_amd/csrc/fdtd_fused2.hpp
+++ b/tidy3d_amd/csrc/fdtd_fused2.hpp
@@ -98,6 +98,10 @@
 void launch_dft_record_dump(hipStream_t st, const DftDumpP& r, const float* dump, float2* acc, long long cells, long long fstride,
                             const float2* phase, int nf);
 void launch_seams(hipStream_t st, const GridP& g, const FieldP& b, const StepP& s, const MatP& m, const float* seam,
-                  int n_seams, const DampT& dmp, const ClipP& clip, const InjP& inj, const SrcP& sr = SrcP{});
+                  int n_seams, const DampT& dmp, const ClipP& clip, const InjP& inj, const SrcP& sr = SrcP{}, float* rep = nullptr);
+constexpr int kRepArraysHost = 7;
+inline size_t seam_scratch_floats(const GridP& g, int n_tiles_x) { return (size_t)n_tiles_x * kSeamArrays * (size_t)(g.nz + 2) * (size_t)g.ny; }
+inline size_t seam_rep_floats(const GridP& g, int n_tiles_x) { return (size_t)n_tiles_x * kRepArraysHost * (size_t)g.nz * (size_t)g.ny; }
+void launch_seam_flush(hipStream_t st, const GridP& g, const FieldP& b, const float* rep, int n_seams);
 
 }
diff --git a/tidy3d_amd/csrc/fdtd_fused2w.hip b/tidy3d_amd/csrc/fdtd_fused2w.hip
--- a/tidy3d_amd/csrc/fdtd_fused2w.hip
+++ b/tidy3d_amd/csrc/fdtd_fused2w.hip
@@ -21,7 +21,7 @@
   case WV: hipLaunchKernelGGL((fused2_step_kernel<1024, 1 | (WV << 8)>), grid, block, shmem, st, g, a, b, s, m, zchunk, nbx, nby,  \
                               nbz, xcd_remap, inj, seam, dmp, clip, tcl, dp, SrcP{}); break
   switch (opt >> 8) {
-    FDTD_F2_W(1); FDTD_F2_W(2); FDTD_F2_W(3); FDTD_F2_W(4); FDTD_F2_W(5); FDTD_F2_W(6); FDTD_F2_W(7); FDTD_F2_W(8);
+    FDTD_F2_W(1); FDTD_F2_W(2); FDTD_F2_W(3); FDTD_F2_W(4); FDTD_F2_W(5); FDTD_F2_W(6); FDTD_F2_W(7); FDTD_F2_W(8); FDTD_F2_W(9);
     FDTD_F2_W(10); FDTD_F2_W(11); FDTD_F2_W(12); FDTD_F2_W(13); FDTD_F2_W(14); FDTD_F2_W(15);
     default: break;
   }
diff --git a/tidy3d_amd/csrc/fdtd_kernels2.hpp b/tidy3d_amd/csrc/fdtd_kernels2.hpp
--- a/tidy3d_amd/csrc/fdtd_kernels2.hpp
+++ b/tidy3d_amd/csrc/fdtd_kernels2.hpp
@@ -66,6 +66,14 @@
   return (((long long)seam * kSeamArrays + arr) * (g.nz + 2) + (k + 1)) * g.ny + j;
 }
 
+constexpr int kRepArrays = 7;
+__device__ __forceinline__ long long rep_base(const GridP& g, int n_tiles_x) {
+  return (long long)n_tiles_x * kSeamArrays * (g.nz + 2) * g.ny;
+}
+__device__ __forceinline__ long long rep_at(const GridP& g, int seam, int arr, int j, int k) {
+  return (((long long)seam * kRepArrays + arr) * g.nz + k) * g.ny + j;
+}
+
 __device__ __forceinline__ float lane_next(float v) {
 #if defined(__HIP_DEVICE_COMPILE__)
   const int x = __builtin_bit_cast(int, v);
@@ -139,6 +147,8 @@
   static_assert((!PF && !EZL) || (OPT & 0xfe) == 0, "prefetch instantiations: the vacuum sweep only");
   constexpr bool DAMP = (OPT & 8) != 0;
   constexpr bool CLIP = (OPT & 16) != 0;
+  constexpr bool REP = (OPT & 8192) != 0;
+  static_assert(!REP || (!CLIP && !PF && !EZL && !DISP && !SRC), "deferred seam repair: plain, materials and absorber sweeps of the whole grid");
   const bool per_x = CLIP && g.bcx0 == BC_PERIODIC;
   const int tile_y = t % nby;
   const int tile_x = (t / nby) % nbx;
@@ -211,6 +221,13 @@
   }
   const float ipy = s.ipy[j], idy = s.idy[j];
 
+  [[maybe_unused]] long long rep_arr = 0;
+  [[maybe_unused]] const float *rpl = nullptr, *rpr = nullptr;
+  if constexpr (REP) {
+    rep_arr = (long long)g.nz * g.ny;
+    rpl = seam + rep_base(g, nbx) + rep_at(g, tile_x, 0, j, 0);
+    rpr = seam + rep_base(g, nbx) + rep_at(g, tile_x > 0 ? tile_x - 1 : 0, 0, j, 0);
+  }
   float exk[V], eyk[V];
   float h1x[V], h1y[V], h1z[V];
   float e1x[V], e1y[V], e1z[V];
@@ -226,6 +243,10 @@
     ldf<V, true>(exk, uni(a.ex + p0), ubc);
     ldf<V, true>(eyk, uni(a.ey + p0), ubc);
     if (xh) exk_m = a.ex[p0 + im];
+    if constexpr (REP) {
+      if (act && tx == 63 && !last_x) { const float* r = rpl + (long long)kA * g.ny; exk[V - 1] = r[2 * rep_arr]; eyk[V - 1] = r[3 * rep_arr]; }
+      if (xh) { const float* r = rpr + (long long)kA * g.ny; eyk[0] = r[5 * rep_arr]; exk_m = r[2 * rep_arr]; }
+    }
   }
   if (kA > 0 && do_e1) {
     const long long pb = (long long)(kA - 1) * g.sxy + rowb;
@@ -240,6 +261,18 @@
     const float ipz = s.ipz[kA - 1];
     ldf<V, true>(ho, uni(a.hx + pb), ubc);
     ldf<V, true>(hoy, uni(a.hy + pb), ubc);
+    if constexpr (REP) {
+      if (act && tx == 63 && !last_x) {
+        const float* r = rpl + (long long)(kA - 1) * g.ny;
+        hoy[V - 1] = r[0]; exm[V - 1] = r[2 * rep_arr]; eym[V - 1] = r[3 * rep_arr]; ezm[V - 1] = r[4 * rep_arr]; ezx = r[6 * rep_arr];
+        if (use_jp) ezj[V - 1] = r[4 * rep_arr + 1];
+      }
+      if (xh) {
+        const float* r = rpr + (long long)(kA - 1) * g.ny;
+        eym[0] = r[5 * rep_arr]; ezm[0] = r[6 * rep_arr];
+        if (use_jp) ezj[0] = r[6 * rep_arr + 1];
+      }
+    }
     if constexpr (DAMP) {
       const float czp = dmp.fc[2][kA - 1];
       const float4 b4 = xdm[tx], c4 = xdm[64 + tx];
@@ -331,15 +364,43 @@
     else if constexpr (PF != 10 && PF != 11) ldf<V, true>(L.hyn, uni(a.hy + pb), ubc);
     if constexpr (PF != 10) ldf<V, true>(L.hzn, uni(a.hz + pb), ubc);
     L.eyx_g = 0.f; L.ezx_g = 0.f;
-    if (act && txo == 63 && !last_x) { L.eyx_g = a.ey[pb + ux + V]; L.ezx_g = a.ez[pb + ux + V]; }
+    const bool from_rep = REP && k < g.nz;
+    if (act && txo == 63 && !last_x && !from_rep) { L.eyx_g = a.ey[pb + ux + V]; L.ezx_g = a.ez[pb + ux + V]; }
     if (per_x && act && last_x) { L.eyx_g = a.ey[pb]; L.ezx_g = a.ez[pb]; }
     L.exn_m = 0.f; L.ez_mm = 0.f; L.ey_mm = 0.f; L.ex_jm = 0.f; L.hy_o = 0.f; L.hz_o = 0.f;
-    if (xh && do_e1) {
+    if (xh && do_e1 && !from_rep) {
       const long long pm = pb + im;
       L.exn_m = a.ex[pm + up];
       L.ez_mm = a.ez[pm]; L.ey_mm = a.ey[pm];
       L.ex_jm = use_jp ? a.ex[pjb + im] : 0.f;
       L.hy_o = a.hy[pm]; L.hz_o = a.hz[pm];
+    }
+    if constexpr (REP) {
+      if (k < g.nz) {
+        const bool up1 = k + 1 < g.nz;
+        if (act && txo == 63 && !last_x) {
+          const float* r = rpl + (long long)k * g.ny;
+          L.hyn[V - 1] = r[0]; L.hzn[V - 1] = r[rep_arr]; L.ezk[V - 1] = r[4 * rep_arr];
+          L.eyx_g = r[5 * rep_arr]; L.ezx_g = r[6 * rep_arr];
+          if (up1) { L.exn[V - 1] = r[2 * rep_arr + g.ny]; L.eyn[V - 1] = r[3 * rep_arr + g.ny]; }
+          if (use_jp) {
+            L.ezj[V - 1] = r[4 * rep_arr + 1];
+            if (!EXJ || ty == W - 1 || k == kA) L.exj[V - 1] = r[2 * rep_arr + 1];
+          }
+        }
+        if (xh) {
+          const float* r = rpr + (long long)k * g.ny;
+          L.ezk[0] = r[6 * rep_arr];
+          if (up1) L.eyn[0] = r[5 * rep_arr + g.ny];
+          if (use_jp) L.ezj[0] = r[6 * rep_arr + 1];
+          if (do_e1) {
+            L.exn_m = up1 ? r[2 * rep_arr + g.ny] : a.ex[pb + im + up];
+            L.ez_mm = r[4 * rep_arr]; L.ey_mm = r[3 * rep_arr];
+            if (use_jp) L.ex_jm = r[2 * rep_arr + 1];
+            L.hy_o = r[0]; L.hz_o = r[rep_arr];
+          }
+        }
+      }
     }
     if constexpr (PF != 0) {
       lds_dma_wait();
@@ -618,7 +679,7 @@
             }
           }
         }
-        if ((CLIP || (own && k >= k0 && k < k1)) && act) {
+        if (WHATIF != 9 && (CLIP || (own && k >= k0 && k < k1)) && act) {
           float* sp = seam + seam_row + (long long)k * g.ny;
           if (seam_l) {
             sp[0] = hyn[V - 1];
@@ -862,12 +923,12 @@
       }
       if (act && (!CLIP || (i0o >= clip.i0 && i0o < clip.i1))) {
         float* sq = seam + seam_row + (long long)(k - 1) * g.ny;
-        if (!CLIP && txo == 63 && !last_x) {
+        if (!CLIP && WHATIF != 9 && txo == 63 && !last_x) {
           sq[7 * seam_arr] = h2x[V - 1];
           sq[8 * seam_arr] = h2y[V - 2];
           sq[9 * seam_arr] = h2z[V - 2];
         }
-        if (!CLIP && txo == 0 && tile_x > 0) {
+        if (!CLIP && WHATIF != 9 && txo == 0 && tile_x > 0) {
           sq[10 * seam_arr - kSeamArrays * seam_arr] = h2x[0];
           sq[11 * seam_arr - kSeamArrays * seam_arr] = h2y[0];
           sq[12 * seam_arr - kSeamArrays * seam_arr] = h2z[0];
@@ -956,7 +1017,8 @@
 }
 
 __global__ __launch_bounds__(256) void seam_kernel(GridP g, FieldP b, StepP s, MatP m,
-                                                   const float* __restrict__ seam, int n_seams, DampT dmp, ClipP clip, InjP inj, SrcP sr) {
+                                                   const float* __restrict__ seam, int n_seams, DampT dmp, ClipP clip, InjP inj, SrcP sr,
+                                                   float* __restrict__ rep) {
   const long long t = (long long)blockIdx.x * blockDim.x + threadIdx.x;
   const int nj = clip.j1 - clip.j0;
   const long long per = (long long)nj * (clip.k1 - clip.k0);
@@ -999,7 +1061,7 @@
   const bool mir_y = (j == 0) && pmc_y0, mir_z = (k == 0) && pmc_z0;
   const long long pr = (long long)k * g.sxy + (long long)j * g.nx;
   const long long p = pr + cc, pl = pr + c - 1;
-  if (wl) { b.hy[pl] = hy_m; b.hz[pl] = hz_m; }
+  if (!rep && wl) { b.hy[pl] = hy_m; b.hz[pl] = hz_m; }
   const float idy = s.idy[j], idz = s.idz[k], idx_m = s.idx[c - 1], idx_c = s.idx[cc];
   const float hx_m = A(7, j, k), hy_mm = A(8, j, k), hz_mm = A(9, j, k);
   const float hx_c = A(10, j, k), hy_c = A(11, j, k), hz_c = A(12, j, k);
@@ -1053,8 +1115,26 @@
     ex_m *= cxm * byv * bzv; ey_m *= bxm * cyv * bzv; ez_m *= bxm * byv * czv;
     ey_c *= bxc * cyv * bzv; ez_c *= bxc * byv * czv;
   }
+  if (rep) {
+    float* r = rep + rep_at(g, sm, 0, j, k);
+    const long long ra = (long long)g.nz * g.ny;
+    r[0] = hy_m; r[ra] = hz_m; r[2 * ra] = ex_m; r[3 * ra] = ey_m; r[4 * ra] = ez_m; r[5 * ra] = ey_c; r[6 * ra] = ez_c;
+    return;
+  }
   if (wl) { b.ex[pl] = ex_m; b.ey[pl] = ey_m; b.ez[pl] = ez_m; }
   if (wr) { b.ey[p] = ey_c; b.ez[p] = ez_c; }
 }
 
-}
+__global__ __launch_bounds__(256) void seam_flush_kernel(GridP g, FieldP b, const float* __restrict__ rep, int n_seams) {
+  const long long t = (long long)blockIdx.x * blockDim.x + threadIdx.x;
+  const long long per = (long long)g.ny * g.nz;
+  if (t >= per * n_seams) return;
+  const int sm = (int)(t / per), k = (int)((t % per) / g.ny), j = (int)(t % g.ny);
+  const float* r = rep + rep_at(g, sm, 0, j, k);
+  const long long ra = per;
+  const long long p = (long long)k * g.sxy + (long long)j * g.nx + (sm + 1) * 256, pl = p - 1;
+  b.hy[pl] = r[0]; b.hz[pl] = r[ra]; b.ex[pl] = r[2 * ra]; b.ey[pl] = r[3 * ra]; b.ez[pl] = r[4 * ra];
+  b.ey[p] = r[5 * ra]; b.ez[p] = r[6 * ra];
+}
+
+}
diff --git a/tidy3d_amd/engine.py b/tidy3d_amd/engine.py
--- a/tidy3d_amd/engine.py
+++ b/tidy3d_amd/engine.py
@@ -569,6 +569,11 @@
                                      f"{C.sizeof(L.FdtdStats)}: rebuild the library (python -m tidy3d_amd.build)")
         return st
 
+    def seam_stats(self) -> L.FdtdSeamStats:
+        st = L.FdtdSeamStats()
+        self._chk(self.lib.dll.fdtd_get_seam_stats(self.handle, C.byref(st)), "fdtd_get_seam_stats")
+        return st
+
     def set_option(self, key: int, value: int):
         self._chk(self.lib.dll.fdtd_set_option(self.handle, key, value), "fdtd_set_option")
 
diff --git a/tidy3d_amd/lib.py b/tidy3d_amd/lib.py
--- a/tidy3d_amd/lib.py
+++ b/tidy3d_amd/lib.py
@@ -21,14 +21,14 @@
     "fdtd_add_point_source", "fdtd_add_tfsf", "fdtd_add_monitor", "fdtd_get_monitor",
     "fdtd_set_field", "fdtd_get_field", "fdtd_set_shutoff", "fdtd_comm_unique_id",
     "fdtd_comm_init", "fdtd_run", "fdtd_run_bloch", "fdtd_get_stats", "fdtd_reset", "fdtd_set_option",
-    "fdtd_far_field", "fdtd_set_mirror_plus", "fdtd_add_aniso", "fdtd_add_aniso_bloch",
+    "fdtd_far_field", "fdtd_set_mirror_plus", "fdtd_add_aniso", "fdtd_add_aniso_bloch", "fdtd_get_seam_stats",
 )
 
 BC_PEC, BC_PMC, BC_PERIODIC, BC_NEIGHBOR = 0, 1, 2, 3
 MON_TIME, MON_DFT = 0, 1
 VARIANT_AUTO, VARIANT_SIMPLE, VARIANT_ZMARCH, VARIANT_FUSED = 0, 1, 2, 3
 FLAG_TIME_KERNELS = 1
-OPT_FLAGS, OPT_VARIANT, OPT_ZCHUNK, OPT_ROWS, OPT_XCD_REMAP, OPT_FUSED_LB, OPT_PML_FUSED, OPT_BND_PLANES, OPT_AUTOTUNE, OPT_PML_SPLIT, OPT_LDS_PAD, OPT_MEM_HINTS, OPT_PLACEMENT_TRIES, OPT_TBLOCK, OPT_EDGE_ZCHUNK, OPT_GRAPH, OPT_TWOSTEP, OPT_SHELL_PAIRS, OPT_STRIP, OPT_SHELL2, OPT_SHELL2_SHAPE, OPT_DEBUG_SYNC, OPT_TILE_SPLIT, OPT_DISP, OPT_WHATIF, OPT_SRC_PAGED, OPT_SLAB_BOXES_FIRST = 0, 1, 2, 3, 4, 5, 6, 7, 8, 9, 10, 11, 12, 13, 14, 15, 16, 17, 18, 19, 20, 21, 22, 23, 24, 25, 26
+OPT_FLAGS, OPT_VARIANT, OPT_ZCHUNK, OPT_ROWS, OPT_XCD_REMAP, OPT_FUSED_LB, OPT_PML_FUSED, OPT_BND_PLANES, OPT_AUTOTUNE, OPT_PML_SPLIT, OPT_LDS_PAD, OPT_MEM_HINTS, OPT_PLACEMENT_TRIES, OPT_TBLOCK, OPT_EDGE_ZCHUNK, OPT_GRAPH, OPT_TWOSTEP, OPT_SHELL_PAIRS, OPT_STRIP, OPT_SHELL2, OPT_SHELL2_SHAPE, OPT_DEBUG_SYNC, OPT_TILE_SPLIT, OPT_DISP, OPT_WHATIF, OPT_SRC_PAGED, OPT_SLAB_BOXES_FIRST, OPT_SEAM_DEFER = 0, 1, 2, 3, 4, 5, 6, 7, 8, 9, 10, 11, 12, 13, 14, 15, 16, 17, 18, 19, 20, 21, 22, 23, 24, 25, 26, 27
 F2_OFF_REASONS = {0: "", 1: "switched off", 2: "grid too small", 3: "z-slab rank", 4: "CPML (shell pairs not possible)",
                   5: "dispersive media not confined to a few planes along z", 6: "TFSF box while it injects", 7: "Bloch / PMC-plus faces (or rows not a multiple of 4 cells)", 8: "magnetic sources with absorber layers",
                   9: "magnetic source node on a tile seam", 10: "too many source nodes", 11: "two-pass kernels",
@@ -62,6 +62,11 @@
                 ("seam_kernel_ms", C.c_double), ("seam_kernel_launches", C.c_int64)]
 
 
+class FdtdSeamStats(C.Structure):
+    _fields_ = [("seam_deferred_pairs", C.c_int64), ("seam_flushes", C.c_int64), ("seam_pending", C.c_int32),
+                ("reserved", C.c_int32), ("seam_flush_ms", C.c_double)]
+
+
 PROGRESS_FN = C.CFUNCTYPE(C.c_int, C.c_int64, C.c_double, C.c_double, C.c_void_p)
 
 
@@ -83,6 +88,7 @@
         d.fdtd_create.argtypes = [C.POINTER(FdtdConfig), C.POINTER(vp)]
         d.fdtd_destroy.argtypes = [vp]
         d.fdtd_destroy.restype = None
+        d.fdtd_get_seam_stats.argtypes = [vp, C.POINTER(FdtdSeamStats)]
         d.fdtd_set_steps.argtypes = [vp, C.c_int, vp, vp, C.c_int]
         d.fdtd_set_media.argtypes = [vp, vp, vp, C.c_int]
         d.fdtd_set_material.argtypes = [vp, vp, C.c_size_t]
```

Measured after the change: 206,900 Mcells/s, median of 6. 3.0% higher.
